# pangenome/seqrush

Hardware: AMD Instinct MI355X
Metric: aligned pairs/sec all-vs-all 64x5kb (higher is better)
Workload: dtype i16

## Files before the change

__graft_entry__.py:

```python
import os
import subprocess
import sys

ROOT = os.path.dirname(os.path.abspath(__file__))
if ROOT not in sys.path:
    sys.path.insert(0, ROOT)


def _newer(target, deps):
    if not os.path.exists(target):
        return False
    t = os.path.getmtime(target)
    return all(os.path.getmtime(d) <= t for d in deps if os.path.exists(d))


def _lib_is_current(lib):
    sys.path.insert(0, os.path.join(ROOT, "scripts"))
    import src_digest
    try:
        have, want = open(lib + ".digest").read().strip(), src_digest.digest(ROOT)
    except OSError as e:
        print(f"[build] no digest beside {os.path.basename(lib)} ({e}): building", file=sys.stderr)
        return False
    if not os.path.exists(lib) or have != want:
        print(f"[build] library digest {have} != source digest {want}: building", file=sys.stderr)
        return False
    return True


def build() -> None:
    csrc = os.path.join(ROOT, "seqrush_amd", "csrc")
    lib = os.path.join(ROOT, "seqrush_amd", "libseqrush_amd.so")
    bounds_lib = os.path.join(ROOT, "seqrush_amd", "libseqrush_amd_bounds.so")
    if not _lib_is_current(lib) or not os.path.exists(bounds_lib):
        subprocess.check_call(["make", "-C", csrc, "-s", "-j8"], stdout=subprocess.DEVNULL)
    odir = os.path.join(ROOT, "oracle")
    olib = os.path.join(odir, "liboracle.so")
    odeps = [os.path.join(odir, f) for f in ("uf.c", "wfa.c", "seqrush.c", "compact.c", "sr_oracle.h")]
    if not _newer(olib, odeps):
        subprocess.check_call(["make", "-C", odir, "-s", "-B"])
    ref_script = os.path.join(odir, "build_ref.sh")
    if os.path.isdir("/root/reference") and os.path.exists(ref_script):
        subprocess.call(["bash", ref_script])
    cli = os.path.join(ROOT, "seqrush_amd", "seqrush_mi355x")
    if not os.path.exists(cli):
        subprocess.check_call(["make", "-C", csrc, "-s"])
    import seqrush_amd
    from seqrush_amd import _lib
    L = _lib.load()
    missing = [s for s in _lib.EXPORTS if not hasattr(L, s)]
    if missing:
        raise RuntimeError(f"libseqrush_amd.so lacks symbols: {missing}")


def smoke() -> None:
    build()
    sys.path.insert(0, os.path.join(ROOT, "tests"))
    import numpy as np
    import oracle_binding as ob
    from seqrush_amd import synth
    from seqrush_amd.seqrush import SeqSet, Params, Context, build_gfa

    recs = synth.config_c1()
    ss = SeqSet(recs)
    ctx = Context(0)
    ctx.load(ss, Params())
    ctx.align(); ctx.unite(); ctx.sync()
    al = ctx.alignments()
    labels = ctx.download_labels()
    ctx.sync()
    o = ob.OracleSeqRush(records=recs)
    op = ob.default_params(); op.threads = 4
    for i in range(al.n):
        oa = o.align_pair(op, int(al.query_idx[i]), int(al.target_idx[i]))
        assert al.raw_cigar_bytes(i) == oa["cigar"], f"CIGAR mismatch on pair {i}"
        assert bool(al.is_reverse[i]) == oa["is_reverse"]
        assert int(al.score[i]) == oa["score"]
    o.align_and_unite(op)
    assert np.array_equal(o.canonical_labels(), labels), "UF partition differs from oracle"
    g_gpu, n_gpu, e_gpu = build_gfa(ss, labels)
    g_cpu, n_cpu, e_cpu = o.gfa(canonical=True)

    def canon(g):
        lines = g.strip().split("\n")
        return [x for x in lines if x[0] != "L"], sorted(x for x in lines if x[0] == "L")
    assert canon(g_gpu) == canon(g_cpu), "GFA differs from oracle"
    print(f"smoke ok: {al.n} pairs, {n_gpu} nodes, {e_gpu} edges, "
          f"align {ctx.kernel_ms(0):.2f} ms, unite {ctx.kernel_ms(1):.2f} ms")
    al.close(); ctx.close()


if __name__ == "__main__":
    build()
    if len(sys.argv) > 1 and sys.argv[1] == "smoke":
        smoke()
```

include/seqrush_amd.h:

```cpp
#ifndef SEQRUSH_AMD_H
#define SEQRUSH_AMD_H
#include <stddef.h>
#include <stdint.h>

#ifdef __cplusplus
extern "C" {
#endif

#define SR_ABI_VERSION 2

typedef enum {
    SR_OK = 0,
    SR_ERR_INVALID = -1,
    SR_ERR_NO_DEVICE = -2,
    SR_ERR_HIP = -3,
    SR_ERR_ALPHABET = -4,
    SR_ERR_EMPTY_SEQ = -5,
    SR_ERR_UNSUPPORTED = -6,
    SR_ERR_DEVICE_FAULT = -7,
    SR_ERR_IO = -8,
    SR_ERR_NOMEM = -9
} sr_status;

typedef struct {
// ... 30 lines not shown
    uint32_t shard_rank, shard_count;
    uint32_t tree_k_nearest, tree_k_farthest;
    double tree_rand_frac;
    uint32_t tree_kmer;
} sr_params;

void sr_default_params(sr_params *p);
int sr_parse_scores(const char *s, sr_params *p);
int sr_parse_orientation_scores(const char *s, sr_params *p);
int sr_parse_sparsification(const char *s, sr_params *p);

int sr_pair_list(uint32_t n, const sr_params *p, uint32_t **q_out, uint32_t **t_out,
                 uint64_t *count);

typedef struct {
    uint64_t n;
    uint32_t *query_idx, *target_idx;
    uint8_t *is_reverse;
    int32_t *score;
    uint64_t *query_start, *query_end, *target_start, *target_end;
    uint64_t *cigar_off;
    uint32_t *cigar_ops;
} sr_alignments;

int sr_align_all(const sr_seqset *seqs, const sr_params *p, sr_alignments **out);
void sr_alignments_free(sr_alignments *a);
size_t sr_alignment_cigar(const sr_alignments *a, uint64_t i, char *buf, size_t cap);

int sr_align_and_unite(const sr_seqset *seqs, const sr_params *p, uint64_t *parent_out);

uint64_t sr_uf_find(const uint64_t *nodes, uint64_t n, uint64_t x);
int sr_uf_same(const uint64_t *nodes, uint64_t n, uint64_t x, uint64_t y);
int sr_uf_init_host(uint64_t *nodes, uint64_t n, uint64_t total_len);
int sr_uf_unite_host(uint64_t *nodes, uint64_t n, uint64_t x, uint64_t y);
int sr_uf_merge_labels_host(uint64_t *nodes, uint64_t n, const uint64_t *labels, uint32_t count);
int sr_uf_canonical_labels_host(const uint64_t *nodes, uint64_t n, uint64_t *labels_out);

int sr_write_paf(const sr_alignments *a, const sr_seqset *seqs, const char *path);

typedef struct sr_ctx sr_ctx;
int sr_ctx_create(int device, sr_ctx **out);
void sr_ctx_destroy(sr_ctx *c);
int sr_ctx_set_stream(sr_ctx *c, void *hip_stream);
int sr_ctx_load(sr_ctx *c, const sr_seqset *seqs, const sr_params *p);
int sr_ctx_load_pairs(sr_ctx *c, const sr_seqset *seqs, const sr_params *p, const uint32_t *query_idx,
                      const uint32_t *target_idx, uint64_t count);
int sr_ctx_pairs(const sr_ctx *c, uint32_t **q_out, uint32_t **t_out, uint64_t *count);
uint32_t sr_ctx_num_batches(const sr_ctx *c);
const char *sr_ctx_workspace_report(const sr_ctx *c);
int sr_ctx_reset_uf(sr_ctx *c);
int sr_ctx_align(sr_ctx *c);
int sr_ctx_unite(sr_ctx *c);
int sr_ctx_run(sr_ctx *c);
int sr_ctx_align_all(sr_ctx *c, int unite, sr_alignments **out);
int sr_ctx_pair_results(sr_ctx *c, int32_t *score, uint8_t *is_reverse, uint32_t *cigar_ops);
int sr_ctx_sync(sr_ctx *c);
int sr_ctx_alignments(sr_ctx *c, sr_alignments **out);
int sr_ctx_download_uf(sr_ctx *c, uint64_t *parent_out);
uint64_t sr_ctx_uf_size(const sr_ctx *c);
uint64_t sr_ctx_num_pairs(const sr_ctx *c);
uint64_t sr_ctx_dp_cells(const sr_ctx *c);
int sr_ctx_labels_device(sr_ctx *c, uint64_t *dev_labels);
int sr_ctx_merge_labels(sr_ctx *c, const uint64_t *dev_labels, uint32_t count);
int sr_ctx_labels_device_u32(sr_ctx *c, uint32_t *dev_labels);
int sr_ctx_merge_labels_u32(sr_ctx *c, const uint32_t *dev_labels, uint32_t count);
int sr_ctx_download_labels(sr_ctx *c, uint64_t *labels_out);
int sr_ctx_merge_labels_host(sr_ctx *c, const uint64_t *labels, uint32_t count);
int sr_ctx_load_paf(sr_ctx *c, const sr_seqset *seqs, const sr_params *p, const char *paf_path);
int sr_unite_paf(const sr_seqset *seqs, const sr_params *p, const char *paf_path, uint64_t *parent_out);
int sr_ctx_build_gfa(sr_ctx *c, const sr_seqset *seqs, char **gfa, uint64_t *n_nodes, uint64_t *n_edges);
int sr_ctx_kernel_ms(sr_ctx *c, int which, float *ms);
const char *sr_ctx_align_kernel(const sr_ctx *c);
int sr_ctx_counters(sr_ctx *c, uint64_t out[16]);
int sr_ctx_counters_ext(sr_ctx *c, uint64_t out[32]);
int sr_ctx_counters_all(sr_ctx *c, uint64_t *out, uint32_t cap);
const char *sr_knobs_doc(void);
int sr_ctx_tail_deferred(sr_ctx *c, uint64_t *out);
int sr_ctx_tail_timeline(sr_ctx *c, uint64_t *out, uint32_t cap_wg);
int sr_ctx_prio_timeline(sr_ctx *c, uint64_t *out, uint32_t cap_wg);
int sr_tile_prio_role_host(uint32_t rank, uint32_t epoch, uint32_t wg_per_cu);
int sr_tile_prio_epoch_shift(void);
int sr_tail_shape(int impl, int block_levels, int wave_build, int off16, int ring_u16, int symbol_bits, int two_piece,
                  int main_threads, uint32_t max_words, int forced);

typedef struct {
    uint64_t tree_entries;
    uint64_t random_entries;
    uint64_t random_processed;
    uint64_t random_aligned;
    uint64_t checks;
    uint64_t windows;
    uint64_t post_tree;
    uint64_t final_components;
    int32_t stabilized;
    int32_t tree_defaulted;
    uint32_t tree_k_nearest, tree_k_farthest;
    double tree_rand_frac;
    uint32_t tree_kmer;
    uint32_t reserved;
} sr_iter_stats;
int sr_ctx_load_iterative(sr_ctx *c, const sr_seqset *seqs, const sr_params *p, int keep_alignments);
int sr_ctx_run_iterative(sr_ctx *c);
int sr_ctx_iterative_stats(sr_ctx *c, sr_iter_stats *out, uint64_t *check_counts, uint64_t cap);
int sr_ctx_iterative_alignments(sr_ctx *c, sr_alignments **out);
int sr_uf_count_components_host(const uint64_t *nodes, uint64_t n, uint64_t total_len, uint64_t *count);
int sr_iterative_stop_host(const uint64_t *counts, uint64_t nchecks, uint64_t post_tree, uint64_t *stop_check);
int sr_iterative_pair_lists(uint32_t n, const uint8_t *sel, const sr_params *p, uint32_t **tree_i, uint32_t **tree_j,
                            uint64_t *tree_count, uint32_t **rand_i, uint32_t **rand_j, uint64_t *rand_count);
int sr_base_cone_reach(int e1, int e2, int two, int levels_left);
int sr_mirror_map(const uint32_t *query_idx, const uint32_t *target_idx, uint64_t count, const uint32_t *batch_first,
                  uint32_t nbatch, uint32_t workgroups, uint32_t *mirror_out, uint64_t *partners_out);
int sr_ctx_orientation_scores(sr_ctx *c, int32_t *fwd, int32_t *rev);
int sr_mirror_bt_pick(const int *off, int transposed);
int sr_mirror_bt_rank_transposed(int tag);
int sr_mirror_bt_tie_host(const int *off);
int sr_mirror_bp_pick_host(const int *val, const int *dist, const int *comp, const int *diag, int n, int value_bias,
                           int *pick_out, int *pick_t_out);
int sr_replay_record_ints(void);
void sr_replay_transpose_host(const int *rec, int *out);
int sr_replay_match_host(const int *recs, int nrec, const int *segs, int nseg, int level, int *match_out);

typedef struct {
    uint64_t min_size;
    int32_t keep_alignments;
    uint32_t join_below;
} sr_inv_params;
typedef struct {
    uint64_t scanned;
    uint64_t sites;
    uint64_t candidates;
    uint64_t accepted;
    uint64_t rejected_score;
    uint64_t rejected_divergence;
    uint64_t united_bases;
    uint64_t patch_batches;
    double scan_ms, patch_align_ms;
} sr_inv_stats;
typedef struct {
    uint64_t pair;
    uint32_t query_idx, target_idx;
    uint64_t query_start, query_end;
    uint64_t target_start, target_end;
    int32_t main_score, patch_score;
    uint8_t is_reverse;
    uint8_t accepted;
    uint8_t reserved[2];
    int32_t site_cost;
} sr_inv_job;
int sr_ctx_enable_inversions(sr_ctx *c, const sr_inv_params *p);
int sr_ctx_inversion_stats(sr_ctx *c, sr_inv_stats *out);
int sr_ctx_inversion_join_stats(sr_ctx *c, uint64_t out[4]);
int sr_ctx_inversion_jobs(sr_ctx *c, sr_inv_job **jobs, uint64_t *count);
int sr_ctx_inversion_alignments(sr_ctx *c, sr_alignments **out);
int sr_append_paf_tagged(const sr_alignments *a, const sr_seqset *seqs, const char *path, const char *tag);
#define SR_INV_SITE_DIVERGENT 1
#define SR_INV_SITE_QUERY_ONLY 2
#define SR_INV_SITE_TARGET_ONLY 3
typedef struct {
    uint64_t query_start, query_end, target_start, target_end;
    int32_t kind;
    int32_t candidate;
} sr_inv_site;
int sr_inversion_sites_host(const uint32_t *ops, uint64_t n_ops, uint64_t min_size, sr_inv_site **sites, uint64_t *count);
int sr_inversion_candidate(uint64_t qgap, uint64_t tgap, uint64_t min_size);
int sr_inversion_accept(int32_t patch_score, int32_t main_score);
int sr_inversion_sites_host_join(const uint32_t *ops, uint64_t n_ops, uint64_t min_size, uint32_t join_below, const sr_params *pen,
// ... 183 lines not shown
```

seqrush_amd/_lib.py:

```python
import ctypes as C
import os

_HERE = os.path.dirname(os.path.abspath(__file__))
LIB_PATH = os.environ.get("SEQRUSH_AMD_LIB") or os.path.join(_HERE, "libseqrush_amd.so")

EXPORTS = [
    "sr_default_params", "sr_parse_scores", "sr_parse_orientation_scores",
    "sr_parse_sparsification", "sr_align_all", "sr_alignments_free", "sr_alignment_cigar",
    "sr_align_and_unite", "sr_uf_find", "sr_uf_same", "sr_write_paf", "sr_ctx_create",
    "sr_ctx_destroy", "sr_ctx_set_stream", "sr_ctx_load", "sr_ctx_reset_uf", "sr_ctx_align",
    "sr_ctx_unite", "sr_ctx_sync", "sr_ctx_alignments", "sr_ctx_download_uf", "sr_ctx_uf_size",
    "sr_ctx_num_pairs", "sr_ctx_dp_cells", "sr_ctx_labels_device", "sr_ctx_merge_labels",
    "sr_ctx_download_labels", "sr_ctx_kernel_ms", "sr_ctx_counters", "sr_build_gfa", "sr_free",
    "sr_last_error", "sr_abi_version", "sr_device_count", "sr_pair_list", "sr_ctx_align_kernel",
    "sr_ctx_load_paf", "sr_unite_paf", "sr_ctx_build_gfa", "sr_ctx_load_pairs", "sr_ctx_pairs",
    "sr_ctx_num_batches", "sr_ctx_workspace_report", "sr_ctx_run", "sr_ctx_align_all", "sr_ctx_pair_results",
    "sr_ctx_labels_device_u32", "sr_ctx_merge_labels_u32", "sr_ctx_counters_ext",
    "sr_build_gfa_opts", "sr_ctx_build_gfa_opts", "sr_ctx_merge_labels_host",
    "sr_uf_init_host", "sr_uf_unite_host", "sr_uf_merge_labels_host", "sr_uf_canonical_labels_host",
    "sr_build_gfa_from_nodes", "sr_ctx_counters_all", "sr_knobs_doc",
    "sr_sort_params_default", "sr_ctx_build_gfa_sorted", "sr_sort_gfa", "sr_sgd_layout", "sr_sgd_tables", "sr_sort_stats",
    "sr_ctx_load_iterative", "sr_ctx_run_iterative", "sr_ctx_iterative_stats", "sr_ctx_iterative_alignments",
    "sr_uf_count_components_host", "sr_iterative_stop_host", "sr_iterative_pair_lists", "sr_base_cone_reach",
    "sr_ctx_enable_inversions", "sr_ctx_inversion_stats", "sr_ctx_inversion_jobs", "sr_ctx_inversion_alignments",
    "sr_append_paf_tagged", "sr_inversion_sites_host", "sr_inversion_candidate", "sr_inversion_accept",
    "sr_inversion_scan_device",
    "sr_ctx_inversion_join_stats", "sr_inversion_sites_host_join", "sr_inversion_accept_site", "sr_inversion_scan_device_join",
    "sr_compact_gfa", "sr_compact_stats",
    "sr_sketch_device", "sr_knn_select_device",
    "sr_graph_stats_gfa", "sr_graph_stats_free", "sr_graph_stats_report", "sr_stats_sq_sums_host",
    "sr_mirror_map", "sr_mirror_bt_pick", "sr_mirror_bt_rank_transposed", "sr_mirror_bt_tie_host", "sr_mirror_bp_pick_host",
    "sr_ctx_orientation_scores",
    "sr_layout_params_default", "sr_layout_gfa", "sr_layout_tsv", "sr_layout_svg", "sr_layout_quality", "sr_layout_stats",
    "sr_layout_resolve", "sr_layout_select_host",
    "sr_path_bins_gfa", "sr_path_bins_free", "sr_path_bins_tsv", "sr_viz_params_default", "sr_path_bins_rgb", "sr_path_bins_png",
    "sr_growth_params_default", "sr_growth_gfa", "sr_growth_free", "sr_growth_groups", "sr_growth_expected", "sr_growth_fit",
    "sr_growth_report",
    "sr_variant_params_default", "sr_variants_gfa", "sr_variants_free", "sr_variants_vcf",
    "sr_ctx_tail_deferred", "sr_ctx_tail_timeline", "sr_tail_shape",
    "sr_replay_record_ints", "sr_replay_transpose_host", "sr_replay_match_host",
    "sr_ctx_prio_timeline", "sr_tile_prio_role_host", "sr_tile_prio_epoch_shift",
]


class SeqSetC(C.Structure):
    _fields_ = [("n", C.c_uint32), ("bases", C.c_char_p), ("offsets", C.POINTER(C.c_uint64)),
                ("names", C.POINTER(C.c_char_p))]


class ParamsC(C.Structure):
    _fields_ = [
        ("match_score", C.c_int32), ("mismatch_penalty", C.c_int32),
        ("gap_open1", C.c_int32), ("gap_ext1", C.c_int32),
        ("gap_open2", C.c_int32), ("gap_ext2", C.c_int32),
        ("ori_match", C.c_int32), ("ori_mismatch", C.c_int32),
        ("ori_gap_open", C.c_int32), ("ori_gap_ext", C.c_int32),
        ("min_match_len", C.c_uint64), ("max_divergence", C.c_double),
        ("exclude_self", C.c_int32), ("memory_mode", C.c_int32),
        ("sparsify_kind", C.c_int32), ("sparsify_factor", C.c_double),
        ("sparsify_seed", C.c_uint64), ("canonical_labels", C.c_int32), ("device", C.c_int32),
        ("shard_rank", C.c_uint32), ("shard_count", C.c_uint32),
        ("tree_k_nearest", C.c_uint32), ("tree_k_farthest", C.c_uint32), ("tree_rand_frac", C.c_double),
        ("tree_kmer", C.c_uint32),
    ]


class SortParamsC(C.Structure):
    _fields_ = [
        ("seed", C.c_uint64), ("iter_max", C.c_uint64), ("theta", C.c_double), ("eps", C.c_double),
        ("eta_max", C.c_double), ("cooling_start", C.c_double), ("space", C.c_uint64), ("space_max", C.c_uint64),
        ("space_quant", C.c_uint64), ("min_term_updates", C.c_uint64), ("terms_per_round", C.c_uint64),
        ("skip_sgd", C.c_int32), ("skip_groom", C.c_int32), ("skip_topo", C.c_int32), ("device", C.c_int32),
    ]


class LayoutParamsC(C.Structure):
    _fields_ = [
        ("seed", C.c_uint64), ("iter_max", C.c_uint64), ("theta", C.c_double), ("eps", C.c_double),
        ("eta_max", C.c_double), ("cooling_start", C.c_double), ("space", C.c_uint64), ("space_max", C.c_uint64),
        ("space_quant", C.c_uint64), ("min_term_updates", C.c_uint64), ("terms_per_round", C.c_uint64),
        ("device", C.c_int32), ("reserved", C.c_int32),
    ]


class IterStatsC(C.Structure):
    _fields_ = [
        ("tree_entries", C.c_uint64), ("random_entries", C.c_uint64), ("random_processed", C.c_uint64),
        ("random_aligned", C.c_uint64), ("checks", C.c_uint64), ("windows", C.c_uint64), ("post_tree", C.c_uint64),
        ("final_components", C.c_uint64), ("stabilized", C.c_int32), ("tree_defaulted", C.c_int32),
        ("tree_k_nearest", C.c_uint32), ("tree_k_farthest", C.c_uint32), ("tree_rand_frac", C.c_double),
        ("tree_kmer", C.c_uint32), ("reserved", C.c_uint32),
    ]


class InvParamsC(C.Structure):
    _fields_ = [("min_size", C.c_uint64), ("keep_alignments", C.c_int32), ("join_below", C.c_uint32)]


class InvStatsC(C.Structure):
    _fields_ = [("scanned", C.c_uint64), ("sites", C.c_uint64), ("candidates", C.c_uint64), ("accepted", C.c_uint64),
                ("rejected_score", C.c_uint64), ("rejected_divergence", C.c_uint64), ("united_bases", C.c_uint64),
                ("patch_batches", C.c_uint64), ("scan_ms", C.c_double), ("patch_align_ms", C.c_double)]


class InvJobC(C.Structure):
    _fields_ = [("pair", C.c_uint64), ("query_idx", C.c_uint32), ("target_idx", C.c_uint32),
                ("query_start", C.c_uint64), ("query_end", C.c_uint64), ("target_start", C.c_uint64),
                ("target_end", C.c_uint64), ("main_score", C.c_int32), ("patch_score", C.c_int32),
                ("is_reverse", C.c_uint8), ("accepted", C.c_uint8), ("reserved", C.c_uint8 * 2), ("site_cost", C.c_int32)]


class InvSiteC(C.Structure):
    _fields_ = [("query_start", C.c_uint64), ("query_end", C.c_uint64), ("target_start", C.c_uint64),
                ("target_end", C.c_uint64), ("kind", C.c_int32), ("candidate", C.c_int32)]


class GraphStatsC(C.Structure):
    _fields_ = [("length", C.c_uint64), ("nodes", C.c_uint64), ("edges", C.c_uint64), ("paths", C.c_uint64), ("steps", C.c_uint64),
                ("rev_steps", C.c_uint64), ("depth_bp", C.c_uint64),
                ("self_loops", C.c_uint64), ("tips", C.c_uint64), ("components", C.c_uint64),
                ("depth", C.POINTER(C.c_uint32)), ("paths_on", C.POINTER(C.c_uint32)),
                ("bp_by_paths", C.POINTER(C.c_uint64)), ("nodes_by_paths", C.POINTER(C.c_uint64)),
                ("shared", C.POINTER(C.c_uint64)),
                ("path_pairs", C.POINTER(C.c_uint64)), ("path_abs", C.POINTER(C.c_uint64)), ("path_len", C.POINTER(C.c_uint64)),
# ... 233 lines not shown
```

seqrush_amd/csrc/sr_align_blk.hip:

```cpp
#include "sr_dev_common.h"
#include "sr_uf_dev.h"
#define SR_BLK_TU 1
#undef SR_BFS_MAXACT
#ifdef SR_BLK_WAVE
#define SR_BFS_MAXACT 4
#define K_P2 4
#define SR_BLK_SUB wave1
#else
#define SR_BFS_MAXACT 16
#define K_P2 16
#define SR_BLK_SUB wg4
#endif
#define BFS_MAK_SLOTS SR_BLK_MAK_SLOTS
#define SR_BT_ATTR __forceinline__
namespace SR_NS { namespace SR_BLK_SUB {
#include "sr_align_bfs.inc"
#include "sr_align_blk.inc"
} }
using namespace SR_NS::SR_BLK_SUB;

template <typename OT, int NT, bool TWO, bool PROF = false>
static int launch_blk3(const SrAlignArgs *a, int nwg, size_t lds_bytes, hipStream_t st) {
    if (lds_bytes > 16 * 1024) {
        hipError_t e = hipFuncSetAttribute((const void *)sr_align_blk_kernel<OT, NT, TWO, 5, 2, 1, PROF>,
                                           hipFuncAttributeMaxDynamicSharedMemorySize, (int)lds_bytes);
        if (e != hipSuccess) return (int)e;
    }
    hipLaunchKernelGGL((sr_align_blk_kernel<OT, NT, TWO, 5, 2, 1, PROF>), dim3(nwg), dim3(NT), lds_bytes, st, *a);
    return (int)hipGetLastError();
}
template <typename OT, int NT, bool TWO, bool PROF = false, typename RT = OT>
static int launch_blk10(const SrAlignArgs *a, int nwg, size_t lds_bytes, hipStream_t st) {
    if (lds_bytes > 16 * 1024) {
        hipError_t e = hipFuncSetAttribute((const void *)sr_align_blk_kernel<OT, NT, TWO, 10, 2, 1, PROF, 5, 10, RT>,
                                           hipFuncAttributeMaxDynamicSharedMemorySize, (int)lds_bytes);
        if (e != hipSuccess) return (int)e;
    }
    hipLaunchKernelGGL((sr_align_blk_kernel<OT, NT, TWO, 10, 2, 1, PROF, 5, 10, RT>), dim3(nwg), dim3(NT), lds_bytes, st, *a);
    return (int)hipGetLastError();
}
#if SR_SYMBITS == 2 && !defined(SR_BLK_WAVE)
extern "C" int srk_align_blk_max_levels(void) { return KB_MAX; }
#ifndef SR_BUILD_TAG
#define SR_BUILD_TAG "default"
#endif
extern "C" const char *srk_align_blk_build_tag(void) { return SR_BUILD_TAG; }
extern "C" int srk_align_blk_supports(const SrPen *pen, const SrPen *ori) {
    if (ori->two || ori->e1 != 1 || ori->scope + 2 > BFS_MAK_SLOTS) return 0;
    if (pen->e1 != 2 || (pen->two && pen->e2 != 1)) return 0;
    if (pen->x == 5 && pen->o1 + pen->e1 == 10 && (!pen->two || (pen->o2 + pen->e2 >= 10 && (pen->o2 + pen->e2) % 5 == 0)) &&
        (2 * pen->scope + 2 * 10 + 2 + 9) / 10 * 10 <= BFS_MAK_SLOTS) return 10;
    const int B = 5;
    if (pen->x < B || pen->o1 + pen->e1 < B) return 0;
    if (pen->two && pen->o2 + pen->e2 < B) return 0;
    if (pen->scope + B + 1 > BFS_MAK_SLOTS) return 0;
    return B;
}
#endif
#ifdef SR_BLK_WAVE
extern "C" int SRK_NAME(srk_align_blkw)(const SrAlignArgs *a, int nwg, size_t lds_bytes, int off16, int nthreads, void *stream) {
    hipStream_t st = (hipStream_t)stream;
    const bool two = a->pen.two != 0;
    if (a->kblock == 10 && nthreads == 128 && off16)
        return two ? launch_blk10<int16_t, 128, true>(a, nwg, lds_bytes, st) : launch_blk10<int16_t, 128, false>(a, nwg, lds_bytes, st);
    if (a->kblock == 10) {
        if (off16) return two ? launch_blk10<int16_t, 64, true>(a, nwg, lds_bytes, st) : launch_blk10<int16_t, 64, false>(a, nwg, lds_bytes, st);
        return two ? launch_blk10<int32_t, 64, true>(a, nwg, lds_bytes, st) : launch_blk10<int32_t, 64, false>(a, nwg, lds_bytes, st);
    }
    if (off16) return two ? launch_blk3<int16_t, 64, true>(a, nwg, lds_bytes, st) : launch_blk3<int16_t, 64, false>(a, nwg, lds_bytes, st);
    return two ? launch_blk3<int32_t, 64, true>(a, nwg, lds_bytes, st) : launch_blk3<int32_t, 64, false>(a, nwg, lds_bytes, st);
}
#else
extern "C" int SRK_NAME(srk_align_blk)(const SrAlignArgs *a, int nwg, size_t lds_bytes, int off16, int nthreads, void *stream) {
    hipStream_t st = (hipStream_t)stream;
    const bool two = a->pen.two != 0;
    if (a->kblock == 10) {
        if (off16) {
#if SR_SYMBITS == 2
            if (nthreads == 1024 && two) return launch_blk10<int16_t, 1024, true>(a, nwg, lds_bytes, st);
#endif
            if (nthreads >= 512) return two ? launch_blk10<int16_t, 512, true>(a, nwg, lds_bytes, st) : launch_blk10<int16_t, 512, false>(a, nwg, lds_bytes, st);
#if SR_SYMBITS == 2
            if (a->profile_ticks && two) return launch_blk10<int16_t, 256, true, true>(a, nwg, lds_bytes, st);
#endif
            return two ? launch_blk10<int16_t, 256, true>(a, nwg, lds_bytes, st) : launch_blk10<int16_t, 256, false>(a, nwg, lds_bytes, st);
        }
        if (a->ring_u16 && nthreads == 512) return two ? launch_blk10<int32_t, 512, true, false, uint16_t>(a, nwg, lds_bytes, st)
                                                       : launch_blk10<int32_t, 512, false, false, uint16_t>(a, nwg, lds_bytes, st);
        if (a->ring_u16) return two ? launch_blk10<int32_t, 256, true, false, uint16_t>(a, nwg, lds_bytes, st)
                                    : launch_blk10<int32_t, 256, false, false, uint16_t>(a, nwg, lds_bytes, st);
        return two ? launch_blk10<int32_t, 256, true>(a, nwg, lds_bytes, st) : launch_blk10<int32_t, 256, false>(a, nwg, lds_bytes, st);
    }
    if (off16) {
        if (nthreads == 128) return two ? launch_blk3<int16_t, 128, true>(a, nwg, lds_bytes, st) : launch_blk3<int16_t, 128, false>(a, nwg, lds_bytes, st);
        if (nthreads == 512) return two ? launch_blk3<int16_t, 512, true>(a, nwg, lds_bytes, st) : launch_blk3<int16_t, 512, false>(a, nwg, lds_bytes, st);
        return two ? launch_blk3<int16_t, 256, true>(a, nwg, lds_bytes, st) : launch_blk3<int16_t, 256, false>(a, nwg, lds_bytes, st);
    }
    return two ? launch_blk3<int32_t, 256, true>(a, nwg, lds_bytes, st) : launch_blk3<int32_t, 256, false>(a, nwg, lds_bytes, st);
}
#endif
```

seqrush_amd/csrc/sr_align_blk.inc:

```
#include "sr_blk_rows.inc"
#include "sr_blk_tile.inc"
#include "sr_blk_pass.inc"
#include "sr_blk_phase2.inc"
#include "sr_blk_orient.inc"

#define K_SHIFT0 29
#define K_WIDTH0 64
struct KSeqs { int poff_f, poff_r, toff_f, toff_r, plen_all, tlen_all; };
__device__ __forceinline__ void kjob_set(int jid, int base, int pb, int pe, int tb, int te, int rev, int begin, int chk,
                                         int seg, const KSeqs &q) {
    bjob_set(jid, base, pb, pe, tb, te, 0, begin, chk, seg, rev ? q.poff_r : q.poff_f);
    BJob &b = b_sh.job[jid];
    b.shift = (pe - pb) + K_SHIFT0;
    b.pad0 = rev ? q.toff_r : q.toff_f;
    b.pad2 = 1;
    if (rev) { b.p0 = q.plen_all - pe; b.t0 = q.tlen_all - te; }
}
__device__ __forceinline__ int kjob_width(int plen, int tlen) { return (plen + tlen + K_WIDTH0) & ~3; }

#define SR_BLK_MIN_WAVES 4
template <typename OT, int NT, bool TWO, int B, int E1, int E2, bool PROF = false, int X = 0, int OE1 = 0, typename RT = OT>
__global__ void __launch_bounds__(NT, SR_BLK_MIN_WAVES) sr_align_blk_kernel(SrAlignArgs a) {
    const int tid = threadIdx.x;
    if (a.tail_mode == SR_TAIL_RUN && *a.tail_count == 0u) return;
    GP<RT> bring = (GP<RT>)(RT *)a.bring + (size_t)blockIdx.x * a.bring_wg_stride;
    GP<OT> bhist = (GP<OT>)(OT *)a.bhist + (size_t)blockIdx.x * a.bhist_wg_stride;
    GP<int> lists = (GP<int>)a.bseg + (size_t)blockIdx.x * 2 * SR_BFS_MAXSEG * SR_BFS_SEGREC;
    GP<uint32_t> btbuf = (GP<uint32_t>)a.bbt + (size_t)blockIdx.x * a.bbase_jobs * SR_BFS_BTCAP;
    GP<uint32_t> clist = (GP<uint32_t>)a.bcl + (size_t)blockIdx.x * a.bcl_wg_stride;
    GP<int> gmak = (GP<int>)a.bmak + (size_t)blockIdx.x * (BJ_MAX * BFS_MAK_SLOTS);
    unsigned long long t_ori = 0, t_bp = 0, t_base = 0, t_all = 0, tb_bt = 0, tb_emit = 0;
    unsigned long long tq_pass = 0, tq_bar = 0, tq_ctl = 0, tq_ph2 = 0, tq_tail = 0, tq_rec = 0;
    unsigned row_ld = 0, row_st = 0;
    unsigned long long tl_first = 0, tl_last = 0, tl_n = 0, tl_mir = 0, tl_end1 = 0;
    const int depth = a.kdepth;
    const int depth2 = a.kdepth2;
    const unsigned nrows = (unsigned)depth + 4u * (unsigned)depth2 + (unsigned)SR_NULL_ROWS + 2u;
    KRows<OT, RT> RR;
    KRows<OT, OT> RH;
    RR.base = bring; RR.cM = (unsigned)depth * 256u; RR.cst2 = (unsigned)depth2 * 256u; RR.sstr = 256u; RR.chs = nrows * 256u;
    RR.depth = depth; RR.depth2 = depth2; RR.perjob = false; RR.extent = (unsigned)a.bring_wg_stride;
    RR.nuloff = ((unsigned)depth + 4u * (unsigned)depth2) * 256u; RR.urow = RR.nuloff + (unsigned)SR_NULL_ROWS * 256u; RR.trash = RR.urow + 256u;
    const unsigned urow = RR.urow;
    const unsigned hw = a.hist_nul_w;
    RH.base = bhist; RH.cM = 0; RH.cst2 = 0; RH.sstr = 0; RH.chs = 256u; RH.depth = 0x3fff; RH.depth2 = 0x3fff; RH.urow = 0; RH.perjob = true; RH.extent = (unsigned)a.bhist_wg_stride;
    RH.nuloff = (unsigned)a.hist_cap; RH.trash = RH.nuloff + hw;
    if (tid < 64) k_sh.cells_l[tid] = 0ull;
    if (tid < 64) k_sh.row_w[tid >> 4][tid & 15] = 0ull;
    {
        for (int r = 0; r < SR_NULL_ROWS; r++)
            for (int i = tid; i < a.brow; i += NT) rput(RR, RR.nuloff + (unsigned)r * 256u, (unsigned)i, NULLV);
        for (int i = tid; i < (int)hw; i += NT) RH.base[RH.nuloff + (unsigned)i] = (OT)NULLV;
        if (tid == 0) {
            b_sh.pen[0] = a.pen; b_sh.pen[1] = a.ori; b_sh.cells = 0; k_sh.t_setup = 0; k_sh.t_p2a = k_sh.t_p2f = k_sh.t_p2e = k_sh.t_p2w = 0; k_sh.t_c1 = k_sh.t_c2 = 0;
            k_sh.dg_f = k_sh.dg_c = k_sh.dg_e = k_sh.dg_r = 0; k_sh.dg_redo = 0;
#ifdef SR_BOUNDS
            k_sh.bnd_flag = 0; k_sh.bnd_off = k_sh.bnd_ext = k_sh.bnd_what = 0; k_sh.lds_seq_bytes = 16u * a.max_words + 16u;
#endif
            k_sh.dg_steps = k_sh.dg_nbase = k_sh.dg_nbp = k_sh.dg_npass = 0; k_sh.base_tiles = k_sh.base_cells = 0;
            k_sh.mir_next = -1; k_sh.mir_pairs = k_sh.mir_ties = 0;
            k_sh.rp_record = k_sh.rp_on = k_sh.rp_ready = 0; k_sh.rp_nrec = 0;
            k_sh.rp_replays = k_sh.rp_cached = k_sh.rp_tie_top = k_sh.rp_tie_base = 0;
            b_sh.geom.brow = a.brow; b_sh.geom.ring_scope = a.ring_scope; b_sh.geom.ring_hot = a.ring_hot;
            b_sh.geom.bbase_jobs = a.bbase_jobs; b_sh.geom.hist_w = a.hist_w; b_sh.geom.hist_levels = a.hist_levels;
            b_sh.geom.urow = urow;
            unsigned p_rank = 0, p_idx = 0, p_arr = 0;
            if (a.cu_arrivals) {
                const unsigned xcc = (unsigned)__builtin_amdgcn_s_getreg(20 | (0 << 6) | (3 << 11));
                const unsigned cu = (unsigned)__builtin_amdgcn_s_getreg(4 | (8 << 6) | (7 << 11));
                p_idx = sr_prio_table_index(xcc, cu);
                p_arr = atomicAdd(&a.cu_arrivals[p_idx], 1u);
                p_rank = p_arr % (unsigned)max(a.prio_wg, 1);
                atomicAdd(&a.counters[52], 1ull);
                atomicMax(&a.counters[53], (unsigned long long)p_arr + 1ull);
            }
            k_sh.prio_rank = (int)p_rank; k_sh.prio_role = 0;
            k_sh.prio_wg = (a.tile_prio && a.cu_arrivals && a.prio_wg > 1) ? a.prio_wg : 0;
            if (PROF && a.prio_timeline) {
                unsigned long long *tp = a.prio_timeline + 4ull * blockIdx.x;
                tp[0] = 0ull; tp[1] = p_rank; tp[2] = p_idx; tp[3] = p_arr;
            }
        }
        __syncthreads();
    }
    const SrPen pen = a.pen;
    const SrPen ori = a.ori;
    constexpr bool KTIGHT = KTIGHT_OF(OT, RT, B, X);
    const int scope = pen.scope;
    const int gap_opening = TWO ? max(pen.o1, pen.o2) : pen.o1;
    for (;;) {
        if (tid < 64) {
            unsigned long long cl = k_sh.cells_l[tid];
            k_sh.cells_l[tid] = 0ull;
            for (int o = 32; o > 0; o >>= 1) cl += __shfl_xor(cl, o, 64);
            if (tid == 0) b_sh.cells += cl;
        }
        if (tid == 0) {
            int pr = k_sh.mir_next;
            k_sh.mir_next = -1;
            const bool from_mir = pr >= 0;
            if (a.tail_mode == SR_TAIL_RUN) {
                const uint32_t i = atomicAdd(a.tail_head, 1u);
                pr = i < *a.tail_count ? (int)a.tail_list[i] : (int)a.npairs;
            } else while (pr < 0) {
                pr = (int)atomicAdd(a.queue_head, 1u);
                if (pr >= (int)a.npairs) { pr = (int)a.npairs; break; }
                if (a.order) pr = (int)a.order[pr];
                if (a.mirror && a.mirror[pr] != SR_MIRROR_NONE && (a.mirror[pr] & SR_MIRROR_SECONDARY)) pr = -1;
            }
            if (PROF) {
                const unsigned long long now = KTICK();
                if (tl_n == 0) tl_first = now;
                if (tl_n == 1 && tl_end1 == 0) tl_end1 = now;
                if (pr < (int)a.npairs) { tl_last = now; tl_n++; tl_mir = from_mir ? 1ull : 0ull; }
            }
            k_sh.rp_on = (from_mir && k_sh.rp_ready) ? 1 : 0;
            k_sh.rp_ready = 0; k_sh.rp_record = 0;
            if (a.brec && !from_mir && a.tail_mode != SR_TAIL_RUN && a.mirror && pr < (int)a.npairs) {
                const uint32_t m = a.mirror[pr];
                if (m != SR_MIRROR_NONE && !(m & SR_MIRROR_SECONDARY)) { k_sh.rp_record = 1; k_sh.rp_nrec = 0; }
            }
            k_sh.rp_level = 0; k_sh.rp_rd = 0; k_sh.rp_top_tie = 0; k_sh.rp_seg_tie = 0;
            b_sh.pair = pr;
            b_sh.err = 0; b_sh.cig_cnt = 0; b_sh.score_acc = 0; k_sh.pend_op = -1; k_sh.pend_len = 0;
            k_sh.mir_tie = 0;
            k_sh.mir_snap[0] = b_sh.cells; k_sh.mir_snap[1] = k_sh.dg_steps; k_sh.mir_snap[2] = k_sh.dg_nbase; k_sh.mir_snap[3] = k_sh.dg_nbp;
        }
        __syncthreads();
        const int pair = RFL(b_sh.pair);
        if (pair >= (int)a.npairs) break;
        const uint32_t q = a.pair_q[pair], t = a.pair_t[pair];
        const int plen = (int)a.seqlen[q], tlen = (int)a.seqlen[t];
        const int pw = SR_SEQ_WORDS(plen), tw = SR_SEQ_WORDS(tlen);
        load_seq_lds<NT>(lds_seq, (GP<const uint32_t>)a.seqwords + a.word_off_fwd[q] - 1, pw);
        load_seq_lds<NT>(lds_seq + a.max_words, (GP<const uint32_t>)a.seqwords + a.word_off_rc[q] - 1, pw);
        load_seq_lds<NT>(lds_seq + 2 * (size_t)a.max_words, (GP<const uint32_t>)a.seqwords + a.word_off_fwd[t] - 1, tw);
        load_seq_lds<NT>(lds_seq + 3 * (size_t)a.max_words, (GP<const uint32_t>)a.seqwords + a.word_off_rev[t] - 1, tw);
        const int oPf = 1, oPr = (int)a.max_words + 1, oTf = 2 * (int)a.max_words + 1, oTr = 3 * (int)a.max_words + 1;
        GP<uint32_t> ops = (GP<uint32_t>)a.cigar_ops + a.cigar_base[pair];
        const uint32_t cap = (uint32_t)(a.cigar_base[pair + 1] - a.cigar_base[pair]);
        const unsigned long long tk0 = KTICK();
        int fwd = -1, rev = INT_MAX, is_rev = 0;
        if (a.pre_oriented) {
// ... 52 lines not shown
                if (s > smax) { if (tid == 0) b_sh.err |= SR_DEV_ERR_SCORE_BOUND; break; }
            }
        }
        }
        if (a.word_off_rev != a.word_off_rc) {
            __syncthreads();
            load_seq_lds<NT>(lds_seq + (is_rev ? 0 : (size_t)a.max_words),
                             (GP<const uint32_t>)a.seqwords + (is_rev ? a.word_off_cmp[q] : a.word_off_rev[q]) - 1, pw);
            __syncthreads();
        }
        const KSeqs ks = {is_rev ? oPr : oPf, is_rev ? oPf : oPr, oTf, oTr, plen, tlen};
        const unsigned long long tk1 = KTICK();
        t_ori += tk1 - tk0;
        GP<int> cur = lists, nxt = lists + (size_t)SR_BFS_MAXSEG * SR_BFS_SEGREC;
        if (tid == 0) {
            cur[SL_PB] = 0; cur[SL_PE] = plen; cur[SL_TB] = 0; cur[SL_TE] = tlen; cur[SL_CB] = SR_C_M; cur[SL_CE] = SR_C_M;
            const int rem = (a.mem_mode == 3) ? INT_MAX : -1;
            cur[SL_REM] = rem; cur[SL_KIND] = seg_kind(plen, tlen, rem);
            b_sh.list_n = 1;
            if (is_rev) k_sh.rp_on = 0;
            if (k_sh.rp_on) k_sh.rp_replays += 1ull;
        }
        __syncthreads();
        for (;;) {
            const int n_cur = RFL(b_sh.list_n);
            bool any_bp = false;
            int pos = 0;
            if (RFL(k_sh.rp_on) != 0 && tid == 0) {
                GP<int> recs = (GP<int>)a.brec + (size_t)blockIdx.x * (SR_BPREC_MAX * SR_BPREC_INTS);
                const int nrec = min(k_sh.rp_nrec, SR_BPREC_MAX), lvl = k_sh.rp_level;
                int rd = k_sh.rp_rd;
                unsigned long long cells = 0ull, cached = 0ull;
                while (rd < nrec && recs[rd * SR_BPREC_INTS + SR_BR_LEVEL] < lvl) rd++;
                for (int p = 0; p < n_cur; p++) {
                    GP<int> e = cur + (size_t)p * SR_BFS_SEGREC;
                    if (e[SL_KIND] != SK_BP) continue;
                    int solved = 0;
                    while (rd < nrec) {
                        GP<int> r = recs + rd * SR_BPREC_INTS;
                        if (r[SR_BR_LEVEL] != lvl) break;
                        const int c = sr_replay_cmp(r, e);
                        if (c > 0) break;
                        rd++;
                        if (c < 0) continue;
                        if (r[SR_BR_TIE] == 0 && sr_replay_same(r, e)) {
                            e[SL_BV] = sr_bprec_t(r, SR_BR_BV); e[SL_BH] = sr_bprec_t(r, SR_BR_BH); e[SL_BCOMP] = sr_bprec_t(r, SR_BR_BCOMP);
                            e[SL_BSF] = r[SR_BR_BSF]; e[SL_BSR] = r[SR_BR_BSR]; e[SL_PASSES] = r[SR_BR_PASSES];
                            cells += ((unsigned long long)(unsigned)r[SR_BR_CELLS_HI] << 32) | (unsigned long long)(unsigned)r[SR_BR_CELLS_LO];
                            cached += 1ull; solved = 1;
                        }
                        break;
                    }
                    e[SL_SOLVED] = solved;
                }
                k_sh.rp_rd = rd; b_sh.cells += cells; k_sh.rp_cached += cached;
            }
            while (pos < n_cur && RFL(b_sh.err) == 0) {
                __syncthreads();
                if (tid == 0) {
                    int na = 0, p = pos, base = 0, ntot = 0, maxp = 0;
                    const bool rp_on = k_sh.rp_on != 0, rp_rec = k_sh.rp_record != 0;
                    for (; p < n_cur && ntot < SR_BFS_MAXACT; p++) {
                        GP<int> e = cur + (size_t)p * SR_BFS_SEGREC;
                        if (e[SL_KIND] != SK_BP) continue;
                        ntot++;
                        if (rp_on && e[SL_SOLVED] != 0) { maxp = max(maxp, e[SL_PASSES]); continue; }
                        k_sh.sg_tie[na] = 0; k_sh.sg_sur[na] = 0; k_sh.sg_done[na] = 0;
                        if (rp_rec) {
                            b_sh.cells += k_sh.cells_l[2 * na] + k_sh.cells_l[2 * na + 1];
                            k_sh.cells_l[2 * na] = 0ull; k_sh.cells_l[2 * na + 1] = 0ull;
                        }
                        BSeg &sg = b_sh.seg[na];
                        sg.pb = e[SL_PB]; sg.pe = e[SL_PE]; sg.tb = e[SL_TB]; sg.te = e[SL_TE]; sg.cb = e[SL_CB]; sg.ce = e[SL_CE];
                        sg.score_f = sg.score_r = 0; sg.last_fwd = 0; sg.f_ak = sg.r_ak = 0; sg.phase = 1;
                        const int sp = sg.pe - sg.pb, st = sg.te - sg.tb;
                        sg.max_ad = sp + st - 1; sg.bp_score = INT_MAX; sg.list_pos = p;
                        const int w = kjob_width(sp, st);
                        kjob_set(2 * na, base, sg.pb, sg.pe, sg.tb, sg.te, 0, sg.cb, -1, na, ks); base += w;
                        kjob_set(2 * na + 1, base, sg.pb, sg.pe, sg.tb, sg.te, 1, sg.ce, -1, na, ks); base += w;
                        if (a.lazy_id) { b_sh.job[2 * na].pad2 = 0; b_sh.job[2 * na + 1].pad2 = 0; }
                        na++;
                    }
                    b_sh.nact = na; b_sh.next_pos = p; b_sh.njobs = 2 * na; b_sh.nrunning = na;
                    k_sh.rp_ntot = ntot; k_sh.rp_maxp = maxp; k_sh.rp_npass0 = k_sh.dg_npass;
                }
                __syncthreads();
                const int nact = RFL(b_sh.nact);
                pos = RFL(b_sh.next_pos);
                if (RFL(k_sh.rp_ntot) == 0) break;
                any_bp = true;
                if (tid == 0) k_sh.dg_nbp += (unsigned long long)k_sh.rp_ntot;
                if (nact == 0) {
                    if (tid == 0) k_sh.dg_steps += 2ull * (unsigned long long)k_sh.rp_ntot * B * (unsigned long long)k_sh.rp_maxp;
                    continue;
                }
                const unsigned long long tb0 = KTICK();
                const int njobs = 2 * nact;
                for (int s0i = 0; RFL(b_sh.nrunning) > 0; s0i += B) {
                    const int s0 = kopaque_s(s0i);
                    const unsigned long long q0 = KTICK();
                    blk_pass<OT, TWO, NT, B, E1, E2, PROF, X, OE1, RT, true>(RR, s0, pen, njobs, row_ld, row_st, s0 == 0);
                    const unsigned long long q1 = KTICK();
                    __syncthreads();
                    const unsigned long long q2 = KTICK();
                    tq_pass += q1 - q0; tq_bar += q2 - q1;
                    if (tid == 0) k_sh.dg_steps += (unsigned long long)njobs * B;
                    const int avail = s0 + B - 1;
                    const int tid_o = tid;
                    if (tid < 64) {
                        const int tid = (int)kopaque_v((unsigned)tid_o);
                        KPRIO_HI();
                        if (tid < njobs) {
#pragma unroll
                            for (int j = 0; j < B; j++) gmak[tid * BFS_MAK_SLOTS + (s0 + j) % depth] = k_sh.jak[j][tid];
                        }
                        const unsigned long long qc1 = KTICK();
                        int ph = 0, ph0 = 0;
                        if (tid < nact) {
                            BSeg &sg = b_sh.seg[tid];
                            ph = sg.phase; ph0 = ph;
                            const long long smax = 2LL * ((long long)pen.o1 * 2 + (long long)pen.e1 * (sg.max_ad + 1)) + 1024;
                            if (ph == 1) {
                                int score_f = sg.score_f, score_r = sg.score_r, last_fwd = sg.last_fwd, f_ak = sg.f_ak, r_ak = sg.r_ak;
                                const int max_ad = sg.max_ad;
                                for (int j = 0; j < B && ph == 1; j++) {
                                    const int s = s0 + j;
                                    const int akf = k_sh.jak[j][2 * tid], akr = k_sh.jak[j][2 * tid + 1];
                                    if (s == 0) {
                                        f_ak = akf; r_ak = akr;
                                        if (f_ak + r_ak >= max_ad) ph = 2;
                                    } else {
                                        score_f = s; f_ak = akf; last_fwd = 1;
                                        if (f_ak + r_ak >= max_ad) ph = 2;
                                        else {
                                            score_r = s; r_ak = akr; last_fwd = 0;
                                            if ((long long)score_f + score_r > smax) ph = 4;
                                            else if (f_ak + r_ak >= max_ad) ph = 2;
                                        }
                                    }
                                }
                                sg.score_f = score_f; sg.score_r = score_r; sg.last_fwd = last_fwd; sg.f_ak = f_ak; sg.r_ak = r_ak;
                                sg.phase = ph;
                            }
                        }
                        const unsigned long long qc2 = KTICK();
                        if (PROF && tid == 0) { k_sh.t_c1 += qc1 - q2; k_sh.t_c2 += qc2 - qc1; }
                        const unsigned long long m2 = __ballot(ph == 2);
                        const unsigned long long mnew = __ballot(ph == 2 && ph0 == 1);
                        if (tid == 0) k_sh.newmask = (unsigned)mnew;
                        if (tid == 0) { k_sh.p2mask_lo = (unsigned)m2; k_sh.p2mask_hi = (unsigned)(m2 >> 32); }
                        if (m2 == 0ull) {
                            const unsigned long long run = __ballot(ph == 1);
                            if (tid < nact && ph != 1) { b_sh.job[2 * tid].active = 0; b_sh.job[2 * tid + 1].active = 0; }
                            if (tid == 0) b_sh.nrunning = __popcll(run);
                            if (run != 0ull) blk_setup<TWO, NT, B, E1, E2, KTIGHT>(s0 + B, pen, njobs);
                        }
                        KPRIO_LO();
                    }
                    __syncthreads();
                    const unsigned long long q3 = KTICK();
                    tq_ctl += q3 - q2;
                    bool p2_or_rec = (RFL(k_sh.p2mask_lo) | RFL(k_sh.p2mask_hi)) != 0u;
                    if (a.lazy_id) {
                        if (RFL(k_sh.newmask) != 0u) p2_or_rec = true;
                        for (unsigned nm = RFL(k_sh.newmask); nm != 0u; nm &= nm - 1u) {
                            const int sa = __ffs((int)nm) - 1;
                            blk_recompute<OT, TWO, NT, B, E1, E2, X, OE1>(RR, pen, sa, RFL(b_sh.seg[sa].score_f), s0, row_ld, row_st);
                        }
                    }
                    tq_rec += KTICK() - q3;
                    if ((RFL(k_sh.p2mask_lo) | RFL(k_sh.p2mask_hi)) != 0u) {
                        blk_phase2<OT, TWO, NT, B, E1, E2, RT, PROF>(RR, clist, gmak, pen, s0, nact, gap_opening);
                        if (tid < 64) {
                            KPRIO_HI();
                            const int ph = (tid < nact) ? b_sh.seg[tid].phase : 0;
                            const unsigned long long run = __ballot(ph == 1 || ph == 2);
                            if (tid < nact && ph != 1 && ph != 2) { b_sh.job[2 * tid].active = 0; b_sh.job[2 * tid + 1].active = 0; }
                            if (tid == 0) b_sh.nrunning = __popcll(run);
                            if (run != 0ull) blk_setup<TWO, NT, B, E1, E2, KTIGHT>(s0 + B, pen, njobs);
                            KPRIO_LO();
                        }
                    }
                    const unsigned long long q4 = KTICK();
                    if (p2_or_rec) __syncthreads();
                    tq_ph2 += q4 - q3; tq_tail += KTICK() - q4;
                    if (tid == 0) k_sh.dg_npass += 1ull;
                }
                if (tid < nact) {
                    BSeg &sg = b_sh.seg[tid];
                    GP<int> e = cur + (size_t)sg.list_pos * SR_BFS_SEGREC;
                    const int sp = sg.pe - sg.pb, st = sg.te - sg.tb;
                    const int bh = sg.bp_off_f, bv = sg.bp_off_f - sg.bp_k_f;
                    if (sg.phase != 3 || sg.bp_score == INT_MAX) atomicOr(&b_sh.err, SR_DEV_ERR_SCORE_BOUND);
                    else if (bv < 0 || bv > sp || bh < 0 || bh > st) atomicOr(&b_sh.err, SR_DEV_ERR_BREAKPOINT);
                    else {
                        e[SL_BV] = bv; e[SL_BH] = bh; e[SL_BCOMP] = sg.bp_comp; e[SL_BSF] = sg.bp_score_f; e[SL_BSR] = sg.bp_score_r;
                        const int ri = k_sh.rp_nrec + tid;
// ... 228 lines not shown
                if (atomicCAS(&a.counters[40], 0ull, (unsigned long long)pair + 1ull) == 0ull) {
                    a.counters[41] = k_sh.bnd_what; a.counters[42] = k_sh.bnd_off; a.counters[43] = k_sh.bnd_ext;
                }
            }
#endif
        }
        __syncthreads();
        const uint32_t mir = a.mirror ? a.mirror[pair] : SR_MIRROR_NONE;
        bool mir_emit = false;
        if (mir != SR_MIRROR_NONE && !(mir & SR_MIRROR_SECONDARY)) {
            mir_emit = p_err == 0 && !is_rev && p_tie == 0 && !(a.pre_oriented && a.is_reverse[mir] != 0);
            if (mir_emit) {
                GP<uint32_t> ops2 = (GP<uint32_t>)a.cigar_ops + a.cigar_base[mir];
                for (uint32_t i = tid; i < cnt; i += NT) { const uint32_t v = ops[i]; ops2[i] = v ^ ((v & 2u) >> 1); }
                if (tid < 64) {
                    unsigned long long cl = k_sh.cells_l[tid];
                    k_sh.cells_l[tid] = 0ull;
                    for (int o = 32; o > 0; o >>= 1) cl += __shfl_xor(cl, o, 64);
                    if (tid == 0) {
                        b_sh.cells += cl;
                        b_sh.cells += b_sh.cells - k_sh.mir_snap[0]; k_sh.dg_steps += k_sh.dg_steps - k_sh.mir_snap[1];
                        k_sh.dg_nbase += k_sh.dg_nbase - k_sh.mir_snap[2]; k_sh.dg_nbp += k_sh.dg_nbp - k_sh.mir_snap[3];
                        k_sh.mir_pairs += 1ull;
                        a.score[mir] = p_score; a.cigar_cnt[mir] = cnt;
                        if (!a.pre_oriented) { a.is_reverse[mir] = 0; a.ori_fwd[mir] = fwd; a.ori_rev[mir] = rev; }
                    }
                }
            } else if (tid == 0) {
                k_sh.mir_ties += 1ull;
                if (p_tie != 0) {
                    if (k_sh.rp_top_tie != 0) k_sh.rp_tie_top += 1ull;
                    else if (k_sh.rp_seg_tie == 0) k_sh.rp_tie_base += 1ull;
                }
                const bool replay = k_sh.rp_record != 0 && p_err == 0 && !is_rev && k_sh.rp_top_tie == 0 &&
                                    !(a.pre_oriented && a.is_reverse[mir] != 0) && a.tail_mode != SR_TAIL_DEFER_ALL;
                bool defer = false;
                if (!replay && a.tail_list && a.tail_mode != SR_TAIL_RUN)
                    defer = a.tail_mode == SR_TAIL_DEFER_ALL ||
                            __hip_atomic_load(a.queue_head, __ATOMIC_RELAXED, __HIP_MEMORY_SCOPE_AGENT) >= a.npairs;
                if (defer) { a.tail_list[atomicAdd(a.tail_count, 1u)] = mir; atomicAdd(a.tail_deferred, 1u); }
                else { k_sh.mir_next = (int)mir; k_sh.rp_ready = replay ? 1 : 0; }
            }
        }
        if (a.fuse_unite) {
            const int sc = p_err ? -1 : p_score;
            if (sc >= 0 && sc <= a.max_score[pair]) {
                unsigned long long united = 0, runs = 0;
                int uerr = 0;
                uf_unite_cigar<NT>((const uint32_t *)a.cigar_ops + a.cigar_base[pair], cnt, a.seq_goff[q], a.seq_goff[t],
                                   (unsigned long long)plen, is_rev != 0, 0ull, 0ull, a.min_match_len, a.uf_nodes, united, runs, uerr);
                for (int o = 32; o > 0; o >>= 1) { united += __shfl_xor(united, o, 64); runs += __shfl_xor(runs, o, 64); }
                if ((tid & 63) == 0) {
                    if (united) atomicAdd(&a.counters[4], mir_emit ? 2ull * united : united);
                    if (runs) atomicAdd(&a.counters[5], mir_emit ? 2ull * runs : runs);
                }
                if (uerr) atomicOr(a.error_flag, uerr);
            }
        }
        t_all += KTICK() - tk0;
        if ((tid & 63) == 0) {
            k_sh.row_w[0][(tid >> 6) & 15] += row_ld; k_sh.row_w[1][(tid >> 6) & 15] += row_st;
            k_sh.row_w[2][(tid >> 6) & 15] += row_ld; k_sh.row_w[3][(tid >> 6) & 15] += row_st;
        }
        row_ld = 0; row_st = 0;
    }
    if (tid < 64 && k_sh.cells_l[tid]) atomicAdd(&a.counters[0], k_sh.cells_l[tid]);
    if ((tid & 63) == 0) {
        const unsigned long long lane_bytes = 8ull;
        const unsigned long long row_ld_acc = k_sh.row_w[0][(tid >> 6) & 15], row_st_acc = k_sh.row_w[1][(tid >> 6) & 15];
        if (row_ld_acc) atomicAdd(&a.counters[16], row_ld_acc * lane_bytes);
        if (row_st_acc) atomicAdd(&a.counters[17], row_st_acc * lane_bytes);
        const unsigned long long hist_ld_acc = k_sh.row_w[2][(tid >> 6) & 15], hist_st_acc = k_sh.row_w[3][(tid >> 6) & 15];
        if (hist_ld_acc) atomicAdd(&a.counters[44], hist_ld_acc * lane_bytes);
        if (hist_st_acc) atomicAdd(&a.counters[45], hist_st_acc * lane_bytes);
    }
    if (tid == 0) {
        atomicAdd(&a.counters[0], b_sh.cells);
        atomicAdd(&a.counters[1], k_sh.dg_steps);
        atomicAdd(&a.counters[2], k_sh.dg_nbase);
        atomicAdd(&a.counters[3], k_sh.dg_nbp);
        atomicAdd(&a.counters[9], k_sh.dg_npass);
        atomicAdd(&a.counters[19], k_sh.dg_f); atomicAdd(&a.counters[20], k_sh.dg_c);
        atomicAdd(&a.counters[21], k_sh.dg_e); atomicAdd(&a.counters[22], k_sh.dg_r);
        if (k_sh.dg_redo) atomicAdd(&a.counters[37], k_sh.dg_redo);
        if (k_sh.mir_pairs) atomicAdd(&a.counters[38], k_sh.mir_pairs);
        if (k_sh.mir_ties) atomicAdd(&a.counters[39], k_sh.mir_ties);
        if (k_sh.rp_tie_top) atomicAdd(&a.counters[48], k_sh.rp_tie_top);
        if (k_sh.rp_tie_base) atomicAdd(&a.counters[49], k_sh.rp_tie_base);
        if (k_sh.rp_replays) atomicAdd(&a.counters[50], k_sh.rp_replays);
        if (k_sh.rp_cached) atomicAdd(&a.counters[51], k_sh.rp_cached);
        atomicAdd(&a.counters[46], k_sh.base_tiles); atomicAdd(&a.counters[47], k_sh.base_cells);
        if (PROF && a.timeline) {
            unsigned long long *tl = a.timeline + 4ull * blockIdx.x;
            tl[0] = tl_first; tl[1] = tl_last; tl[2] = KTICK(); tl[3] = tl_n | (tl_mir << 32);
        }
        if (PROF && a.prio_timeline) a.prio_timeline[4ull * blockIdx.x] = tl_end1;
        if (PROF) {
            if (!a.pre_oriented) atomicAdd(&a.counters[6], t_ori);
            atomicAdd(&a.counters[7], t_bp);
            atomicAdd(&a.counters[8], t_base);
            atomicAdd(&a.counters[10], t_all);
            atomicAdd(&a.counters[11], tq_pass);
            atomicAdd(&a.counters[12], tq_bar);
            atomicAdd(&a.counters[13], k_sh.t_setup);
            atomicAdd(&a.counters[25], tq_ctl); atomicAdd(&a.counters[26], k_sh.t_c1); atomicAdd(&a.counters[27], k_sh.t_c2);
            atomicAdd(&a.counters[28], k_sh.t_p2a); atomicAdd(&a.counters[29], k_sh.t_p2f); atomicAdd(&a.counters[30], k_sh.t_p2e); atomicAdd(&a.counters[31], k_sh.t_p2w);
            atomicAdd(&a.counters[14], tq_ph2);
            atomicAdd(&a.counters[18], tq_rec);
            atomicAdd(&a.counters[23], tb_bt); atomicAdd(&a.counters[24], tb_emit);
            atomicAdd(&a.counters[15], tq_tail);
        }
    }
#undef KTICK
}
```

seqrush_amd/csrc/sr_blk_pass.inc:

```
#include "sr_base_cone.h"
#include "sr_prio_rule.h"
template <bool TWO, int E1, int E2>
__device__ __forceinline__ int kreach(const SrPen &p, int s, int begin) {
    int r;
    if (begin == SR_C_M) {
        r = (s >= p.o1 + E1) ? (s - p.o1) / E1 : 0;
        if (TWO && s >= p.o2 + E2) r = max(r, (s - p.o2) / E2);
    } else {
        r = s / E1;
        if (TWO) r = max(r, s / E2);
    }
    return r;
}

template <bool TWO, int B, int E1, int E2, bool TIGHT>
__device__ __forceinline__ void kwindow(const SrPen &pen, const BJob &b, int s0, int &glo, int &ghi) {
    const int Rw = kreach<TWO, E1, E2>(pen, s0 + B - 1, b.begin);
    const int mg = TIGHT ? 1 : pen.scope + 1;
    const int wlo = max(-b.plen - 1, -Rw - mg), whi = min(b.tlen + 1, Rw + mg);
    glo = (wlo + b.shift) >> 2; ghi = (whi + b.shift) >> 2;
}

#define KTICK() (PROF ? __builtin_amdgcn_s_memrealtime() : 0ull)
__device__ __forceinline__ void kprio_role() {
    switch (RFL(k_sh.prio_role)) {
    case 1: __builtin_amdgcn_s_setprio(1); break;
    case 2: __builtin_amdgcn_s_setprio(2); break;
    case 3: __builtin_amdgcn_s_setprio(3); break;
    default: __builtin_amdgcn_s_setprio(0); break;
    }
}
__device__ __forceinline__ void kprio_epoch() {
    const int wg = RFL(k_sh.prio_wg);
    if (wg > 1) {
        const unsigned epoch = (unsigned)(__builtin_amdgcn_s_memrealtime() >> SR_PRIO_EPOCH_SHIFT);
        if (threadIdx.x == 0) k_sh.prio_role = sr_tile_prio_role((unsigned)k_sh.prio_rank, epoch, (unsigned)wg);
    }
}
#define KPRIO_HI() __builtin_amdgcn_s_setprio(3)
#define KPRIO_LO() kprio_role()
#ifndef SR_BASE_CONE
#define SR_BASE_CONE 1
#endif
template <bool TWO, int NT, int B, int E1, int E2, bool TIGHT = false, bool BASE = false>
__device__ __forceinline__ void blk_setup(int s0, const SrPen &pen, int njobs) {
    const int tid = threadIdx.x;
    constexpr bool CONE = BASE && SR_BASE_CONE;
    int nt = 0, glo = 0, ghi = -1, cells = 0, ccells = 0;
    const bool act = tid < njobs && b_sh.job[tid].active;
    const int pglo = (tid < BJ_MAX) ? k_sh.jglo[tid] : 0, pghi = (tid < BJ_MAX) ? k_sh.jghi[tid] : -1;
    if (act) {
        const BJob &b = b_sh.job[tid];
        int Rw = 0, clo0 = 0, chi0 = 0;
#pragma unroll
        for (int j = 0; j < B; j++) {
            Rw = kreach<TWO, E1, E2>(pen, s0 + j, b.begin);
            int klo = max(-b.plen, -Rw), khi = min(b.tlen, Rw);
            cells += (khi >= klo) ? khi - klo + 1 : 0;
            if (CONE) {
                const int rb = sr_cone_reach(E1, E2, TWO, b.pad1 - 1 - (s0 + j));
                klo = max(klo, b.kend - rb); khi = min(khi, b.kend + rb);
                if (j == 0) { clo0 = b.kend - rb; chi0 = b.kend + rb; }
            }
            k_sh.jklo[j][tid] = klo; k_sh.jkhi[j][tid] = khi;
            ccells += (khi >= klo) ? khi - klo + 1 : 0;
        }
        (void)Rw;
        kwindow<TWO, B, E1, E2, TIGHT>(pen, b, s0, glo, ghi);
        if (CONE) {
            const int mg = TIGHT ? 1 : pen.scope + 1;
            const int wlo = max(max(-b.plen - 1, -Rw - mg), clo0 - 1), whi = min(min(b.tlen + 1, Rw + mg), chi0 + 1);
            glo = (wlo + b.shift) >> 2; ghi = (whi >= wlo) ? (whi + b.shift) >> 2 : glo - 1;
        }
        nt = max(0, (ghi - glo + KGeo<B>::OWN) / KGeo<B>::OWN);
        if (BASE && ccells) atomicAdd(&k_sh.base_cells, (unsigned long long)ccells);
    }
    int incl = nt, hincl = 0;
#pragma unroll
    for (int o = 1; o < 64; o <<= 1) {
        const int v = __shfl_up(incl, o, 64), h = __shfl_up(hincl, o, 64);
        if (tid >= o) { incl += v; hincl += h; }
    }
    if (tid < BJ_MAX) {
        k_sh.jglo[tid] = glo; k_sh.jghi[tid] = ghi;
        k_sh.jgplo[tid] = pglo; k_sh.jgphi[tid] = pghi;
        k_sh.jtstart[tid + 1] = incl;
        k_sh.jmerge[tid] = 0;
        k_sh.jband[tid] = INT_MAX / 2;
#pragma unroll
        for (int j = 0; j < B; j++) { k_sh.jak[j][tid] = 0; k_sh.jreach[j][tid] = 0; }
    }
    if (tid == 0) k_sh.jtstart[0] = 0;
    if (tid == 63) { k_sh.nband = hincl; k_sh.total_tiles = incl + hincl; k_sh.next_tile = NT / 64; if (BASE) k_sh.base_tiles += (unsigned long long)incl; }
    k_sh.cells_l[tid] += (unsigned long long)cells;
    kprio_epoch();
}

template <typename OT, bool TWO, int NT, int B, int E1, int E2, bool PROF, int X = 0, int OE1 = 0, typename ST = OT, bool RING = false, bool BASE = false>
__device__ __forceinline__ void blk_pass(const KRows<OT, ST> &R, int s0, const SrPen &pen, int njobs,
                                         unsigned &row_ld, unsigned &row_st, const bool setup = true) {
    const int tid = threadIdx.x;
    if (setup) {
        const unsigned long long tsu0 = KTICK();
        if (tid < 64) blk_setup<TWO, NT, B, E1, E2, RING && KTIGHT_OF(OT, ST, B, X), BASE>(s0, pen, njobs);
        __syncthreads();
        if (PROF && threadIdx.x == 0) k_sh.t_setup += KTICK() - tsu0;
    }
    kprio_role();
    const int total = RFL(k_sh.total_tiles);
    const int slot0 = kslots(R, s0);
    const int nband = RFL(k_sh.nband);
    for (int t = (tid >> 6); t < total;) {
        int lo, ti;
        if (t < nband) { lo = RFL(k_sh.jbandown[t]); ti = RFL(k_sh.jband[lo]); }
        else {
            const int r = t - nband;
            int hi = njobs; lo = 0;
            while (hi - lo > 1) { const int mid = (lo + hi) >> 1; if (RFL(k_sh.jtstart[mid]) <= r) lo = mid; else hi = mid; }
            ti = r - RFL(k_sh.jtstart[lo]);
            ti += (ti >= RFL(k_sh.jband[lo])) ? 1 : 0;
        }
        blk_tile_any<OT, TWO, B, E1, E2, false, X, OE1, ST, RING>(R, s0, slot0, pen, lo, ti, lo, row_ld, row_st);
        int nx = 0;
        if ((tid & 63) == 0) nx = atomicAdd(&k_sh.next_tile, 1);
        t = RFL(nx);
    }
}

template <typename OT, bool TWO, int NT, int B, int E1, int E2, int X = 0, int OE1 = 0, typename ST = OT>
__device__ __forceinline__ void blk_recompute(const KRows<OT, ST> &R, const SrPen &pen, int sa, int entry_level, int s0_now,
                                              unsigned &row_ld, unsigned &row_st) {
    const int tid = threadIdx.x;
    const int wlo = max(0, entry_level - pen.scope);
    for (int blk = (wlo / B) * B; blk <= s0_now; blk += B) {
        __syncthreads();
        if (tid < 2) {
            const BJob &b = b_sh.job[2 * sa + tid];
            int Rw = 0;
#pragma unroll
            for (int j = 0; j < B; j++) {
                Rw = kreach<TWO, E1, E2>(pen, blk + j, b.begin);
                k_sh.jklo[j][BJ_MAX + tid] = max(-b.plen, -Rw); k_sh.jkhi[j][BJ_MAX + tid] = min(b.tlen, Rw);
            }
            (void)Rw;
            int glo, ghi;
            kwindow<TWO, B, E1, E2, KTIGHT_OF(OT, ST, B, X)>(pen, b, blk, glo, ghi);
            const bool first = blk == (wlo / B) * B;
            k_sh.jgplo[BJ_MAX + tid] = first ? 1 : k_sh.jglo[BJ_MAX + tid];
            k_sh.jgphi[BJ_MAX + tid] = first ? 0 : k_sh.jghi[BJ_MAX + tid];
            k_sh.jglo[BJ_MAX + tid] = glo; k_sh.jghi[BJ_MAX + tid] = ghi;
            const int nt = (ghi - glo + KGeo<B>::OWN) / KGeo<B>::OWN;
            const int n0 = __shfl(nt, 0, 64), n1 = __shfl(nt, 1, 64);
            if (tid == 0) { k_sh.rt_n0 = n0; k_sh.rt_total = n0 + n1; }
        }
        __syncthreads();
        const int n0 = RFL(k_sh.rt_n0), total = RFL(k_sh.rt_total);
        const int slot0 = kslots(R, blk);
        for (int t = (tid >> 6); t < total; t += NT / 64) {
            const int side = (t >= n0) ? 1 : 0;
            blk_tile_any<OT, TWO, B, E1, E2, true, X, OE1, ST, true>(R, blk, slot0, pen, 2 * sa + side, t - (side ? n0 : 0), BJ_MAX + side, row_ld, row_st);
        }
    }
    __syncthreads();
    if (tid < 2) b_sh.job[2 * sa + tid].pad2 = 1;
}

__device__ __forceinline__ long long blk_surplus(const SrPen &pen, int jid, int l0, int l1) {
    const BJob &b = b_sh.job[jid];
    long long c = 0;
    for (int l = l0 + 1; l <= l1; l++) {
        const int Rw = reach(pen, l, b.begin);
        const int klo = max(-b.plen, -Rw), khi = min(b.tlen, Rw);
        c += (khi >= klo) ? khi - klo + 1 : 0;
    }
    return c;
}
```

seqrush_amd/csrc/sr_blk_rows.inc:

```
#define SR_ORI_B 16
#define SR_KB_MAX 10
#define KB_LV (SR_ORI_B > SR_KB_MAX ? SR_ORI_B : SR_KB_MAX)
#define KB_MAX SR_KB_MAX
#define KPK_U16_OF(OT, ST, B, X) (sizeof(OT) == 4 && sizeof(ST) == 2 && (X) > 0 && (B) % 10 == 0)
#define KTIGHT_OF(OT, ST, B, X) ((X) > 0 && (B) % 10 == 0 && (sizeof(OT) == 2 || KPK_U16_OF(OT, ST, B, X)))

struct KShared {
    int jklo[KB_LV][BJ_MAX + 2], jkhi[KB_LV][BJ_MAX + 2];
    int jak[KB_MAX][BJ_MAX], jreach[KB_LV][BJ_MAX];
    int jtstart[BJ_MAX + 1], jglo[BJ_MAX + 2], jghi[BJ_MAX + 2];
    int jmerge[BJ_MAX];
    int jband[BJ_MAX], jbandown[BJ_MAX], nband;
    unsigned newmask;
    int rt_n0, rt_total;
    int jgplo[BJ_MAX + 2], jgphi[BJ_MAX + 2];
    int total_tiles;
    int next_tile;
    int prio_role, prio_rank, prio_wg;
    int p2n, p2seg[K_P2];
    unsigned p2mask_lo, p2mask_hi;
    int pc_n[K_P2], pc_s1[K_P2][2 * KB_MAX];
    unsigned char pc_side[K_P2][2 * KB_MAX];
    signed char pc_idx[K_P2][2][KB_MAX];
    unsigned long long pc_best[K_P2][2 * KB_MAX];
    unsigned long long pc_best_t[K_P2][2 * KB_MAX];
    int pu_start[2 * K_P2 + 1], pu_glo[2 * K_P2];
    int pu_kmin[2 * K_P2], pu_kmax[2 * K_P2];
    int cl_n;
#ifdef SR_BOUNDS
    unsigned lds_seq_bytes;
    int bnd_flag; unsigned bnd_off, bnd_ext, bnd_what;
#endif
    int mir_tie, mir_next;
    unsigned long long mir_snap[4];
    unsigned long long mir_pairs, mir_ties;
    int sg_tie[SR_BFS_MAXACT], sg_sur[SR_BFS_MAXACT], sg_done[SR_BFS_MAXACT];
    int rp_record, rp_on, rp_ready;
    int rp_level, rp_nrec, rp_rd;
    int rp_top_tie, rp_seg_tie;
    int rp_ntot, rp_maxp;
    unsigned long long rp_npass0;
    unsigned long long rp_replays, rp_cached, rp_tie_top, rp_tie_base;
    int redo_from;
    int pend_op, pend_len;
    unsigned long long row_w[4][16];
    unsigned long long base_tiles, base_cells;
    unsigned long long cells_l[64];
    unsigned long long t_c1, t_c2;
    unsigned long long t_setup, t_p2a, t_p2f, t_p2e, t_p2w;
    unsigned long long dg_steps, dg_nbase, dg_nbp, dg_npass;
    unsigned long long dg_f, dg_c, dg_e, dg_r;
    unsigned long long dg_redo;
};
__shared__ KShared k_sh;

template <typename OT, typename ST = OT>
struct KRows {
    GP<ST> base;
    unsigned cM, cst2, sstr, chs;
    unsigned urow, nuloff, trash;
    int depth, depth2;
    bool perjob;
    unsigned extent;
};
#ifdef SR_BOUNDS
__device__ __forceinline__ void kbnd_fail(unsigned what, unsigned off, unsigned ext) {
    atomicOr(&b_sh.err, SR_DEV_ERR_ADDRESS);
    if (atomicCAS(&k_sh.bnd_flag, 0, 1) == 0) { k_sh.bnd_off = off; k_sh.bnd_ext = ext; k_sh.bnd_what = what; }
}
#define SR_BND_OK(R, CELL, WHAT) (((CELL) + 3u < (R).extent) ? true : (kbnd_fail((WHAT), (CELL), (R).extent), false))
#else
#define SR_BND_OK(R, CELL, WHAT) true
#endif
struct KAdr { unsigned hb, cM, cst2, sst; int slotM, slotD, depth, depth2; };
template <typename OT, typename ST>
__device__ __forceinline__ KAdr kadr(const KRows<OT, ST> &R, const BJob &jb, int slots) {
    KAdr A;
    if (R.perjob) { const unsigned hw = RFL(jb.hw); A.hb = RFL(jb.hbase); A.cM = hw; A.cst2 = hw; A.sst = 5u * hw; }
    else { A.hb = 0u; A.cM = R.cM; A.cst2 = R.cst2; A.sst = R.sstr; }
    A.slotM = slots & 0xffff; A.slotD = (int)((unsigned)slots >> 16); A.depth = R.depth; A.depth2 = R.depth2;
    return A;
}
template <typename OT, typename ST>
__device__ __forceinline__ int kslots(const KRows<OT, ST> &R, int s) { return (s % R.depth) | ((s % R.depth2) << 16); }
#define SR_RING_BIAS 24576
typedef short __attribute__((ext_vector_type(4))) S4;
template <typename OT, typename ST> __device__ __forceinline__ V4<OT> kcvt_in(V4<ST> v) {
    if constexpr (sizeof(ST) == sizeof(OT)) return v;
    else { const V4<OT> b = {SR_RING_BIAS, SR_RING_BIAS, SR_RING_BIAS, SR_RING_BIAS}; return __builtin_convertvector((S4)v, V4<OT>) + b; }
}
template <typename OT, typename ST> __device__ __forceinline__ V4<ST> kcvt_out(V4<OT> v) {
    if constexpr (sizeof(ST) == sizeof(OT)) return v;
    else { const V4<OT> b = {SR_RING_BIAS, SR_RING_BIAS, SR_RING_BIAS, SR_RING_BIAS}; return (V4<ST>)__builtin_convertvector(v - b, S4); }
}
// ... 111 lines not shown
```

seqrush_amd/csrc/sr_blk_tile.inc:

```
template <typename OT, bool TWO, int B, int E1, int E2, bool IDONLY = false, int X = 0, int OE1 = 0, typename ST = OT>
__device__ __forceinline__ void blk_tile(const KRows<OT, ST> &R, const int s0, const int slot0, const SrPen &pen,
                                         const int jid, const int ti, const int tix, unsigned &row_ld, unsigned &row_st) {
    constexpr int N1 = E1 < B ? E1 : B, N2 = E2 < B ? E2 : B;
    constexpr bool XK = X > 0;
    static_assert(!XK || (B == OE1 && X <= B), "exact-penalty instance: block depth == o1 + e1 >= x");
    constexpr int HL = KGeo<B>::HL, OWN = KGeo<B>::OWN;
    constexpr int PF = XK ? 3 : B;
    const int lane = threadIdx.x & 63;
    const BJob &jb = b_sh.job[jid];
    const int base = RFL(jb.base), shift = RFL(jb.shift), plen = RFL(jb.plen), tlen = RFL(jb.tlen);
    const int p0 = RFL(jb.p0), t0 = RFL(jb.t0), begin = RFL(jb.begin);
    const int chk = RFL(jb.chk), kend = RFL(jb.kend), poff = RFL(jb.poff), toff = RFL(jb.pad0);
    const bool rec = IDONLY || RFL(jb.pad2) != 0;
    const int glo = RFL(k_sh.jglo[tix]), ghi = RFL(k_sh.jghi[tix]);
    const int g = glo + ti * OWN + lane - HL;
    const bool owned = (lane >= HL) && (lane < 64 - HL) && (g <= ghi);
    const int k0 = (g << 2) - shift;
    const unsigned idx0 = klane(R, (unsigned)(base + (g << 2)));
    const LP P = (LP)(lds_seq + poff), T = (LP)(lds_seq + toff);
    const int cp0 = p0 - k0 + (int)(((uint32_t)(uintptr_t)P >> 2) << SR_WIN_LOG);
    const int ct0 = t0 + (int)(((uint32_t)(uintptr_t)T >> 2) << SR_WIN_LOG);
    const KAdr A = kadr(R, jb, slot0);
#define KROW(LVL, C) krow_rel(R, A, s0, (LVL), (C))
    V4<OT> Lmx[XK ? 1 : B], Lmo1[B], Lmo2[B], Li1[N1], Ld1[N1], Li2[N2], Ld2[N2];
// ... 272 lines not shown
            "v_pk_ashrrev_i16 %1, 15, %5 op_sel_hi:[0,1]\n\t"
            "v_bfi_b32 %2, %0, %6, %4\n\t"
            "v_bfi_b32 %3, %1, %6, %5"
            : "=&v"(ta), "=&v"(tb), "=&v"(ra), "=&v"(rb)
            : "v"(h2_u(v.a)), "v"(h2_u(v.b)), "s"(nul));
    } else {
        const uint32_t bias2 = ((uint32_t)BIAS & 0xffffu) | ((uint32_t)BIAS << 16);
        asm("v_pk_add_i16 %0, %4, %7 clamp\n\t"
            "v_pk_add_i16 %1, %5, %7 clamp\n\t"
            "v_pk_ashrrev_i16 %0, 15, %0 op_sel_hi:[0,1]\n\t"
            "v_pk_ashrrev_i16 %1, 15, %1 op_sel_hi:[0,1]\n\t"
            "v_bfi_b32 %2, %0, %6, %4\n\t"
            "v_bfi_b32 %3, %1, %6, %5"
            : "=&v"(ta), "=&v"(tb), "=&v"(ra), "=&v"(rb)
            : "v"(h2_u(v.a)), "v"(h2_u(v.b)), "s"(nul), "v"(bias2));
    }
    Q4 r; r.a = h2_bits(ra); r.b = h2_bits(rb);
    return r;
}
#define SR_DEEP_INT16 3000
#define SR_DEEP_RING16 1500
__device__ __forceinline__ int q4_get(Q4 x, int q) {
    return (q == 0) ? (int)x.a.x : (q == 1) ? (int)x.a.y : (q == 2) ? (int)x.b.x : (int)x.b.y;
}

template <bool TWO, int B, int E1, int E2, bool IDONLY = false, int X = 0, int OE1 = 0, bool RING = false, typename KR = KRows<short>, int BIAS = 0>
__device__ __forceinline__ void blk_tile16(const KR &R, const int s0, const int slot0, const SrPen &pen,
                                           const int jid, const int ti, const int tix, unsigned &row_ld, unsigned &row_st) {
    typedef short OT;
    typedef short ST;
    static_assert(BIAS == 0 || (RING && X > 0 && B % 10 == 0), "the biased tile exists for ring rows with immediate addressing only");
    constexpr uint32_t NUL = BIAS ? 0x80008000u : NULL16;
    constexpr int NULC = BIAS ? -32768 : -16384;
    const Q4 nulq = {h2_bits(NUL), h2_bits(NUL)};
    constexpr int N1 = E1 < B ? E1 : B, N2 = E2 < B ? E2 : B;
    constexpr bool XK = X > 0;
    static_assert(!XK || (B == OE1 && X <= B), "exact-penalty instance: block depth == o1 + e1 >= x");
    constexpr int HL = KGeo<B>::HL, OWN = KGeo<B>::OWN;
    constexpr int PF = XK ? 3 : B;
    const int lane = threadIdx.x & 63;
    const BJob &jb = b_sh.job[jid];
    const int base = RFL(jb.base), p0 = RFL(jb.p0), t0 = RFL(jb.t0), poff = RFL(jb.poff), toff = RFL(jb.pad0);
    const int shift = RFL(jb.shift), plen = RFL(jb.plen), tlen = RFL(jb.tlen), begin = RFL(jb.begin);
    const int chk = RFL(jb.chk), kend = RFL(jb.kend);
    const bool rec = IDONLY || RFL(jb.pad2) != 0;
    const int glo = RFL(k_sh.jglo[tix]), ghi = RFL(k_sh.jghi[tix]);
    const int g = glo + ti * OWN + lane - HL;
    const bool owned = (lane >= HL) && (lane < 64 - HL) && (g <= ghi);
    const int k0 = (g << 2) - shift;
    const unsigned idx0 = klane(R, (unsigned)(base + (g << 2)));
    const LP P = (LP)(lds_seq + poff), T = (LP)(lds_seq + toff);
    const KAdr A = kadr(R, jb, slot0);
#define KROW(LVL, C) krow_rel(R, A, s0, (LVL), (C))
#define LDQ(LVL, C) q4_from(rld<OT>(R, KROW((LVL), (C)), idx0))
#define LDQ_NT(LVL, C) q4_from(rld_nt<OT>(R, KROW((LVL), (C)), idx0))
    constexpr bool IMMR = RING && XK && (B % 10 == 0);
    const unsigned lane_b = idx0 * (unsigned)sizeof(ST);
    GPB bM1 = nullptr, bM2a = nullptr, bM2b = nullptr, bI1 = nullptr, bD1 = nullptr, bI2 = nullptr, bD2 = nullptr;
    GPB sM = nullptr, sI1 = nullptr, sD1 = nullptr, sI2 = nullptr, sD2 = nullptr;
    if constexpr (IMMR) {
        const int oe2 = pen.o2 + E2;
        bM1 = kbase(R, s0 - B < 0 ? R.nuloff + KBLK_C * 256u : KROW(s0 - B + KBLK_C, SR_C_M));
        bM2a = kbase(R, KROW(s0 - oe2, SR_C_M)); bM2b = kbase(R, KROW(s0 - oe2 + 5, SR_C_M));
        bI1 = kbase(R, KROW(s0 - E1, SR_C_I1)); bD1 = kbase(R, KROW(s0 - E1, SR_C_D1));
        bI2 = kbase(R, KROW(s0 - E2, SR_C_I2)); bD2 = kbase(R, KROW(s0 - E2, SR_C_D2));
        sM = kbase(R, KROW(s0 + KBLK_C, SR_C_M));
        sI1 = kbase(R, KROW(s0 + KBLK_C, SR_C_I1)); sD1 = kbase(R, KROW(s0 + KBLK_C, SR_C_D1));
        sI2 = kbase(R, KROW(s0 + KBLK_C, SR_C_I2)); sD2 = kbase(R, KROW(s0 + KBLK_C, SR_C_D2));
    }
    constexpr bool TIGHT = IMMR && (BIAS ? true : (bool)KTIGHT_OF(short, short, B, X));
    bool msk = false, in10 = true, in2a = true, in2b = true;
    if constexpr (TIGHT) {
        const int oe2 = TWO ? pen.o2 + E2 : B;
        const int l2a = s0 - oe2, l2b = s0 - oe2 + 5;
        const int b2a = l2a >= 0 ? (l2a / B) * B : -1, b2b = l2b >= 0 ? (l2b / B) * B : -1;
        int lo10 = INT_MIN / 2, hi10 = INT_MAX / 2, lo2a = lo10, hi2a = hi10, lo2b = lo10, hi2b = hi10;
        if (s0 - B >= 0) kwindow<TWO, B, E1, E2, true>(pen, jb, s0 - B, lo10, hi10);
        if (TWO && b2a >= 0) kwindow<TWO, B, E1, E2, true>(pen, jb, b2a, lo2a, hi2a);
        if (TWO && b2b >= 0) kwindow<TWO, B, E1, E2, true>(pen, jb, b2b, lo2b, hi2b);
        lo10 = RFL(lo10); hi10 = RFL(hi10); lo2a = RFL(lo2a); hi2a = RFL(hi2a); lo2b = RFL(lo2b); hi2b = RFL(hi2b);
        in10 = g >= lo10 && g <= hi10; in2a = g >= lo2a && g <= hi2a; in2b = g >= lo2b && g <= hi2b;
        msk = __builtin_amdgcn_ballot_w64(!(in10 && in2a && in2b)) != 0ull;
    }
    Q4 Lmx[XK ? 1 : B], Lmo1[B], Lmo2[B], Li1[N1], Ld1[N1], Li2[N2], Ld2[N2];
    unsigned ld_lanes10 = 64u, ld_lanes2 = 64u;
    if (TIGHT && msk) {
#pragma unroll
        for (int j = 0; j < B; j++) { Lmo1[j] = nulq; Lmo2[j] = nulq; }
#pragma unroll
        for (int j = 0; j < N1; j++) { Li1[j] = nulq; Ld1[j] = nulq; }
#pragma unroll
        for (int j = 0; j < N2; j++) { Li2[j] = nulq; Ld2[j] = nulq; }
        if constexpr (IMMR) {
            if (in10) {
#pragma unroll
                for (int j = 0; j < B; j++) Lmo1[j] = q4_from(ild<OT, ST>(R, bM1, lane_b, j - KBLK_C));
#pragma unroll
                for (int j = 0; j < N1; j++) { Li1[j] = q4_from(ild_nt<OT, ST>(R, bI1, lane_b, j)); Ld1[j] = q4_from(ild_nt<OT, ST>(R, bD1, lane_b, j)); }
                if (TWO) {
#pragma unroll
                    for (int j = 0; j < N2; j++) { Li2[j] = q4_from(ild_nt<OT, ST>(R, bI2, lane_b, j)); Ld2[j] = q4_from(ild_nt<OT, ST>(R, bD2, lane_b, j)); }
                }
            }
            if (TWO && in2a) {
#pragma unroll
                for (int j = 0; j < PF && j < 5; j++) Lmo2[j] = q4_from(ild_nt<OT, ST>(R, bM2a, lane_b, j));
            }
        }
        ld_lanes10 = (unsigned)__popcll(__builtin_amdgcn_ballot_w64(in10)); ld_lanes2 = (unsigned)__popcll(__builtin_amdgcn_ballot_w64(in2a));
    } else {
#pragma unroll
    for (int j = 0; j < B; j++) {
        if constexpr (!IDONLY && !XK) Lmx[XK ? 0 : j] = LDQ(s0 + j - pen.x, SR_C_M);
        if constexpr (IMMR) {
            Lmo1[j] = q4_from(ild<OT, ST>(R, bM1, lane_b, j - KBLK_C));
            if (TWO && j < PF) Lmo2[j] = q4_from(ild_nt<OT, ST>(R, j < 5 ? bM2a : bM2b, lane_b, j < 5 ? j : j - 5));
        } else {
            Lmo1[j] = LDQ(s0 + j - pen.o1 - E1, SR_C_M);
            if (TWO && j < PF) Lmo2[j] = LDQ_NT(s0 + j - pen.o2 - E2, SR_C_M);
        }
    }
#pragma unroll
    for (int j = 0; j < N1; j++) {
        if constexpr (IMMR) {
            Li1[j] = q4_from(ild_nt<OT, ST>(R, bI1, lane_b, j)); Ld1[j] = q4_from(ild_nt<OT, ST>(R, bD1, lane_b, j));
        } else {
            Li1[j] = LDQ_NT(s0 + j - E1, SR_C_I1);
            Ld1[j] = LDQ_NT(s0 + j - E1, SR_C_D1);
        }
    }
    if (TWO) {
#pragma unroll
        for (int j = 0; j < N2; j++) {
            if constexpr (IMMR) {
                Li2[j] = q4_from(ild_nt<OT, ST>(R, bI2, lane_b, j)); Ld2[j] = q4_from(ild_nt<OT, ST>(R, bD2, lane_b, j));
            } else {
                Li2[j] = LDQ_NT(s0 + j - E2, SR_C_I2);
                Ld2[j] = LDQ_NT(s0 + j - E2, SR_C_D2);
            }
        }
    }
    }
    const bool with_u = (chk < 0) && (R.urow != 0u) && rec;
    {
        const int nown = min(OWN, max(0, ghi - (glo + ti * OWN) + 1));
        const int n10 = ((!IDONLY && !XK) ? B : 0) + B + 2 * N1 + (TWO ? 2 * N2 : 0);
        const int n2f = TWO ? (PF < B ? PF : B) : 0, n2p = TWO ? B - n2f : 0;
        int nst = (IDONLY ? 0 : B) + (with_u ? 1 : 0);
#pragma unroll
        for (int j = 0; j < B; j++) {
            nst += (j + E1 >= B || rec) ? 2 : 0;
            if (TWO) nst += (j + E2 >= B || rec) ? 2 : 0;
        }
        row_ld += ld_lanes10 * (unsigned)n10 + ld_lanes2 * (unsigned)n2f + 64u * (unsigned)(n2p + (IDONLY ? B : 0) + ((with_u && s0 > 0) ? 1 : 0));
        row_st += (unsigned)nown * (unsigned)nst;
    }
    Q4 uacc = nulq;
    Q4 Lown[IDONLY ? B : 1];
    if (IDONLY) {
#pragma unroll
        for (int j = 0; j < B; j++) {
            if constexpr (IMMR) Lown[IDONLY ? j : 0] = q4_from(ild<OT, ST>(R, sM, lane_b, j - KBLK_C));
            else Lown[IDONLY ? j : 0] = LDQ(s0 + j, SR_C_M);
        }
    }
    if (with_u) {
        const int gplo = RFL(k_sh.jgplo[tix]), gphi = RFL(k_sh.jgphi[tix]);
        if (s0 > 0 && g >= gplo && g <= gphi) uacc = q4_from(rld_raw16(R, R.urow, idx0));
    }
    const bool deep = s0 >= (BIAS ? SR_DEEP_RING16 : SR_DEEP_INT16);
    if (deep) {
#pragma unroll
        for (int j = 0; j < B; j++) {
            if (XK) { if (j + OE1 - X < B && j + OE1 - X >= 0 && j < X) Lmo1[(XK && j + OE1 - X < B) ? j + OE1 - X : 0] = q4_renull<NUL, BIAS>(Lmo1[(XK && j + OE1 - X < B) ? j + OE1 - X : 0]); }
            else if (!IDONLY) Lmx[XK ? 0 : j] = q4_renull<NUL, BIAS>(Lmx[XK ? 0 : j]);
        }
#pragma unroll
        for (int j = 0; j < N1; j++) { Li1[j] = q4_renull<NUL, BIAS>(Li1[j]); Ld1[j] = q4_renull<NUL, BIAS>(Ld1[j]); }
        if (TWO) {
#pragma unroll
            for (int j = 0; j < N2; j++) { Li2[j] = q4_renull<NUL, BIAS>(Li2[j]); Ld2[j] = q4_renull<NUL, BIAS>(Ld2[j]); }
        }
    }
    Q4 Lb;
    {
        int l[4];
#pragma unroll
        for (int q = 0; q < 4; q++) l[q] = max(min(tlen, plen + k0 + q), -1) - BIAS;
        Lb.a = h2_pack(l[0], l[1]); Lb.b = h2_pack(l[2], l[3]);
    }
    const int cp0 = p0 - k0 + BIAS + (int)(((uint32_t)(uintptr_t)P >> 2) << SR_WIN_LOG);
    const int ct0 = t0 + BIAS + (int)(((uint32_t)(uintptr_t)T >> 2) << SR_WIN_LOG);
    const int cpb0 = cp0 << SR_SYM_LOG, cpb1 = (cp0 - 1) << SR_SYM_LOG, cpb2 = (cp0 - 2) << SR_SYM_LOG, cpb3 = (cp0 - 3) << SR_SYM_LOG;
    const int ctb = ct0 << SR_SYM_LOG;
    const unsigned long long ownb = __builtin_amdgcn_ballot_w64(owned);
    Q4 kk;
    kk.a = h2_pack(k0, k0 + 1); kk.b = h2_pack(k0 + 2, k0 + 3);
    int klo0 = RFL(k_sh.jklo[0][tix]), khi0 = RFL(k_sh.jkhi[0][tix]);
    if constexpr (!RING) { klo0 = max(klo0, RFL(k_sh.jklo[B - 1][tix])); khi0 = min(khi0, RFL(k_sh.jkhi[B - 1][tix])); }
    const bool inside = __builtin_amdgcn_ballot_w64(!(k0 >= klo0 && k0 + 3 <= khi0)) == 0ull;
    Q4 hI1[B], hD1[B], hI2[B], hD2[B], mvh[XK ? B : 1];
#pragma unroll
    for (int j = 0; j < B; j++) {
        const int s = s0 + j;
        int klo = 0, khi = 0;
        if (!inside || chk >= 0 || (j == 0 && s0 == 0)) { klo = RFL(k_sh.jklo[j][tix]); khi = RFL(k_sh.jkhi[j][tix]); }
        if (TWO && XK && j + PF < B) {
            if constexpr (IMMR) Lmo2[j + PF < B ? j + PF : 0] = q4_from(ild_nt<OT, ST>(R, j + PF < 5 ? bM2a : bM2b, kopaque_v(lane_b), j + PF < 5 ? j + PF : j + PF - 5));
            else Lmo2[j + PF < B ? j + PF : 0] = LDQ_NT(s0 + j + PF - pen.o2 - E2, SR_C_M);
        }
        if (TIGHT && TWO && msk && j >= PF) {
            const bool in_ = j < 5 ? in2a : in2b;
            const Q4 nq = nulq;
            Lmo2[j].a = in_ ? Lmo2[j].a : nq.a; Lmo2[j].b = in_ ? Lmo2[j].b : nq.b;
        }
        const unsigned lane_j = IMMR ? kopaque_v(lane_b) : 0u;
        Q4 Lj = Lb;
        if (!inside) {
            int l[4];
#pragma unroll
            for (int q = 0; q < 4; q++) { const int k = k0 + q; l[q] = (k >= klo && k <= khi) ? q4_get(Lb, q) : -32768; }
            Lj.a = h2_pack(l[0], l[1]); Lj.b = h2_pack(l[2], l[3]);
        }
        Q4 mx, mo1 = Lmo1[j], si1, sd1, mo2 = nulq, si2 = nulq, sd2 = nulq;
        if (IDONLY) mx = nulq;
        else if (!XK) mx = Lmx[XK ? 0 : j];
        else if (j >= X) mx = mvh[(XK && j >= X) ? j - X : 0];
        else mx = Lmo1[(XK && j + OE1 - X < B) ? j + OE1 - X : 0];
        if (j < N1) { si1 = Li1[j < N1 ? j : 0]; sd1 = Ld1[j < N1 ? j : 0]; }
        else { si1 = hI1[j >= E1 ? j - E1 : 0]; sd1 = hD1[j >= E1 ? j - E1 : 0]; }
        if (TWO) {
            mo2 = Lmo2[j];
            if (j < N2) { si2 = Li2[j < N2 ? j : 0]; sd2 = Ld2[j < N2 ? j : 0]; }
            else { si2 = hI2[j >= E2 ? j - E2 : 0]; sd2 = hD2[j >= E2 ? j - E2 : 0]; }
        }
        Q4 i1 = q4_bound<NUL>(q4_inc(q4_from_left(q4_max(mo1, si1))), Lj);
        Q4 d1 = q4_bound<NUL>(q4_from_right(q4_max(mo1, sd1)), Lj);
// ... 28 lines not shown
                bp[0] = bit_index<0>(mwa, cpb0); bp[1] = bit_index<1>(mwa, cpb1); bp[2] = bit_index<0>(mwb, cpb2); bp[3] = bit_index<1>(mwb, cpb3);
                bt[0] = bit_index_u<0>(mwa, ctb); bt[1] = bit_index_u<1>(mwa, ctb); bt[2] = bit_index_u<0>(mwb, ctb); bt[3] = bit_index_u<1>(mwb, ctb);
#ifdef SR_BOUNDS
                {
                    const unsigned lo_ = (unsigned)(uintptr_t)lds_seq;
                    const unsigned seq_hi = lo_ + RFL(k_sh.lds_seq_bytes);
#pragma unroll
                    for (int q = 0; q < 4; q++) {
                        const int mvq = q4_get(m, q);
                        if (owned && mvq >= -BIAS && mvq <= q4_get(Lb, q)) {
                            const unsigned ap = ((unsigned)bp[q] >> 3) & ~3u, at = ((unsigned)bt[q] >> 3) & ~3u;
                            if (ap < lo_ || ap + 8u > seq_hi) kbnd_fail(3u, ap, seq_hi);
                            if (at < lo_ || at + 8u > seq_hi) kbnd_fail(3u, at, seq_hi);
                        }
                    }
                }
#endif
#pragma unroll
                for (int q = 0; q < 4; q++) { win_words_bit(bp[q], pl[q], ph[q]); win_words_bit(bt[q], tl[q], th[q]); }
                asm volatile("; 8 windows in flight" : "+v"(pl[0]), "+v"(ph[0]), "+v"(pl[1]), "+v"(ph[1]), "+v"(pl[2]), "+v"(ph[2]), "+v"(pl[3]), "+v"(ph[3]),
                                                        "+v"(tl[0]), "+v"(th[0]), "+v"(tl[1]), "+v"(th[1]), "+v"(tl[2]), "+v"(th[2]), "+v"(tl[3]), "+v"(th[3]));
#pragma unroll
                for (int q = 0; q < 4; q++) {
                    const int nn = q4_get(Lb, q) - mv[q];
                    const uint32_t xw = __builtin_amdgcn_alignbit(ph[q], pl[q], (uint32_t)bp[q]) ^
                                        __builtin_amdgcn_alignbit(th[q], tl[q], (uint32_t)bt[q]);
                    const int ext_ = (int)min3u(ffs_sym(xw), (unsigned)SR_WIN, (unsigned)nn);
                    mv[q] += ext_;
                    pend[q] = __builtin_amdgcn_ballot_w64(ext_ == SR_WIN) & __builtin_amdgcn_ballot_w64(mv[q] >= -BIAS) & ownb;
                }
            }
            while ((pend[0] | pend[1] | pend[2] | pend[3]) != 0ull) {
#pragma unroll
                for (int q = 0; q < 4; q++) {
                    if (pend[q] == 0ull) continue;
                    const int nn = lanes_or_zero(pend[q], q4_get(Lb, q) - mv[q]);
                    const uint32_t xw = win_sym(mv[q] + cp0 - q) ^ win_sym(mv[q] + ct0);
                    mv[q] += (int)min3u(ffs_sym(xw), (unsigned)SR_WIN, (unsigned)nn);
                    pend[q] = __builtin_amdgcn_ballot_w64(xw == 0u && nn > SR_WIN);
                }
            }
            m.a = h2_pack_perm(mv[0], mv[1]); m.b = h2_pack_perm(mv[2], mv[3]);
            if (XK) mvh[XK ? j : 0] = m;
            int ak;
            if constexpr (BIAS == 0) {
                typedef unsigned short __attribute__((ext_vector_type(2))) U2;
                const uint32_t va = ~h2_u(m.a >> (H2){15, 15}), vb = ~h2_u(m.b >> (H2){15, 15});
                const uint32_t aa = h2_u(m.a + m.a - kk.a) & va, ab = h2_u(m.b + m.b - kk.b) & vb;
                const uint32_t mx2 = __builtin_bit_cast(uint32_t, __builtin_elementwise_max(__builtin_bit_cast(U2, aa), __builtin_bit_cast(U2, ab)));
                ak = owned ? (int)max(mx2 >> 16, mx2 & 0xffffu) : 0;
            } else {
                ak = 0;
#pragma unroll
                for (int q = 0; q < 4; q++) ak = max(ak, mv[q] >= -BIAS ? 2 * (mv[q] + BIAS) - (k0 + q) : 0);
                ak = owned ? ak : 0;
            }
            uacc = q4_max(uacc, m);
            if (j == 0 && s0 == 0) uacc = TWO ? q4_max(uacc, q4_max(q4_max(i1, i2), q4_max(d1, d2))) : q4_max(uacc, q4_max(i1, d1));
            if (chk >= 0) {
                const int qe = kend - k0;
                if (owned && qe >= 0 && qe < 4 && kend >= klo && kend <= khi) {
                    const uint32_t wa = (chk == SR_C_I1) ? h2_u(i1.a) : (chk == SR_C_I2) ? h2_u(i2.a) : (chk == SR_C_D1) ? h2_u(d1.a)
                                      : (chk == SR_C_D2) ? h2_u(d2.a) : h2_u(m.a);
                    const uint32_t wb = (chk == SR_C_I1) ? h2_u(i1.b) : (chk == SR_C_I2) ? h2_u(i2.b) : (chk == SR_C_D1) ? h2_u(d1.b)
                                      : (chk == SR_C_D2) ? h2_u(d2.b) : h2_u(m.b);
                    const uint32_t w = (qe & 2) ? wb : wa;
                    const int val = (int)(short)((qe & 1) ? (w >> 16) : (w & 0xffffu));
                    if (val + BIAS >= tlen) k_sh.jreach[j][jid] = 1;
                }
            }
            ak = row16_max_nn(ak);
            if ((lane & 15) == 15 && ak > 0) atomicMax(&k_sh.jak[j][jid], ak);
        } else {
            uacc = q4_max(uacc, Lown[IDONLY ? j : 0]);
            if (j == 0 && s0 == 0) uacc = TWO ? q4_max(uacc, q4_max(q4_max(i1, i2), q4_max(d1, d2))) : q4_max(uacc, q4_max(i1, d1));
        }
        if (owned) {
            if constexpr (IMMR) {
                const int im = j - KBLK_C;
                const bool l1 = j + E1 >= B, l2 = j + E2 >= B;
                if (!IDONLY) ist<OT, ST>(R, sM, lane_j, im, q4_vec(m));
                if (l1) { ist<OT, ST>(R, sI1, lane_j, im, q4_vec(i1)); ist<OT, ST>(R, sD1, lane_j, im, q4_vec(d1)); }
                if (TWO && l2) { ist<OT, ST>(R, sI2, lane_j, im, q4_vec(i2)); ist<OT, ST>(R, sD2, lane_j, im, q4_vec(d2)); }
                if (rec && (!l1 || (TWO && !l2))) {
                    const unsigned lane_r = kopaque_v(lane_b);
                    if (!l1) { ist_nt<OT, ST>(R, sI1, lane_r, im, q4_vec(i1)); ist_nt<OT, ST>(R, sD1, lane_r, im, q4_vec(d1)); }
                    if (TWO && !l2) { ist_nt<OT, ST>(R, sI2, lane_r, im, q4_vec(i2)); ist_nt<OT, ST>(R, sD2, lane_r, im, q4_vec(d2)); }
                }
            } else {
            if (!IDONLY) rst<OT>(R, KROW(s, SR_C_M), idx0, q4_vec(m));
            if (j + E1 < B) { if (rec) { rst_nt<OT>(R, KROW(s, SR_C_I1), idx0, q4_vec(i1)); rst_nt<OT>(R, KROW(s, SR_C_D1), idx0, q4_vec(d1)); } }
            else { rst<OT>(R, KROW(s, SR_C_I1), idx0, q4_vec(i1)); rst<OT>(R, KROW(s, SR_C_D1), idx0, q4_vec(d1)); }
            if (TWO) {
                if (j + E2 < B) { if (rec) { rst_nt<OT>(R, KROW(s, SR_C_I2), idx0, q4_vec(i2)); rst_nt<OT>(R, KROW(s, SR_C_D2), idx0, q4_vec(d2)); } }
                else { rst<OT>(R, KROW(s, SR_C_I2), idx0, q4_vec(i2)); rst<OT>(R, KROW(s, SR_C_D2), idx0, q4_vec(d2)); }
            }
            }
        }
    }
    if (with_u && owned) rst_raw16(R, R.urow, idx0, q4_vec(uacc));
#undef KROW
#undef LDQ
#undef LDQ_NT
}

template <typename OT, bool TWO, int B, int E1, int E2, bool IDONLY, int X, int OE1, typename ST = OT, bool RING = false>
__device__ __forceinline__ void blk_tile_any(const KRows<OT, ST> &R, const int s0, const int slot0, const SrPen &pen,
                                             const int jid, const int ti, const int tix, unsigned &row_ld, unsigned &row_st) {
    if constexpr (sizeof(OT) == 2 && (X > 0 || B >= 5)) blk_tile16<TWO, B, E1, E2, IDONLY, X, OE1, RING>(R, s0, slot0, pen, jid, ti, tix, row_ld, row_st);
    else if constexpr (KPK_U16_OF(OT, ST, B, X) && RING) blk_tile16<TWO, B, E1, E2, IDONLY, X, OE1, true, KRows<OT, ST>, SR_RING_BIAS>(R, s0, slot0, pen, jid, ti, tix, row_ld, row_st);
    else blk_tile<OT, TWO, B, E1, E2, IDONLY, X, OE1>(R, s0, slot0, pen, jid, ti, tix, row_ld, row_st);
}
```

seqrush_amd/csrc/sr_host.cpp:

```cpp
#include <hip/hip_runtime_api.h>
#include <algorithm>
#include <chrono>
#include <climits>
#include <functional>
#include <queue>
#include <cmath>
#include <cstdio>
#include <cstdlib>
#include <cstring>
#include <string>
#include <unordered_map>
#include <unordered_set>
#include <vector>
#include "../../include/seqrush_amd.h"
#include "sr_internal.h"
#include "sr_graph.h"
#include "sr_sort.h"
#include "sr_compact.h"
#include "sr_iter_rule.h"
#include "sr_inv_rule.h"
#include "sr_base_cone.h"
#include "sr_mirror_rule.h"
#include "sr_prio_rule.h"

static thread_local std::string g_err;
static int fail(int code, const std::string &msg) { g_err = msg; return code; }
int sr_fail(int code, const std::string &msg) { return fail(code, msg); }
extern "C" const char *sr_last_error(void) { return g_err.c_str(); }

struct SrKnob { const char *name, *unset, *doc; };
static const SrKnob SR_KNOBS[] = {
    {"SR_ALIGN_IMPL", "2 when the penalties have a blocked instance", "1 = level-per-pass kernel (sr_align_bfs_kernel), 2 = score-blocked kernel"},
    {"SR_BLK_LEVELS", "10 for x=5, o1+e1=10", "5 = generic 5-level blocked instance instead of the exact 10-level one"},
    {"SR_ALIGN_THREADS", "by pairs per CU", "threads per workgroup: 64 | 128 | 256 | 512 | 1024"},
    {"SR_WG_PER_CU", "4", "workgroups per CU the launch is sized for"},
    {"SR_NWG", "CUs x workgroups per CU", "cap on workgroups (several pairs per workgroup on small inputs)"},
    {"SR_RING_U16", "1 below 57 k", "0 = 32-bit searches keep 32-bit ring rows"},
    {"SR_LAZY_ID", "1", "0 = searches store their I/D rows from the first level (no recompute pass)"},
    {"SR_HIST_JOBS", "4", "worst-case base cases the per-workgroup history holds (1..16)"},
    {"SR_BFS_BASE_JOBS", "16 (lean builds 4 / 8)", "base cases per batch"},
    {"SR_CIGAR_ARENA_OPS", "25 % of free memory", "CIGAR arena in ops (tests: force batches)"},
    {"SR_POISON_ROWS", "off", "fill the row workspaces with this offset before the run (stale-row tests)"},
    {"SR_PREORIENT", "by pairs per CU and LDS", "1 / 0 = orientation as its own kernel / inside the alignment kernel"},
    {"SR_NO_REORDER", "off", "keep list order instead of the cost-sorted dequeue order"},
    {"SR_ORIENT_LEVELS", "off", "orientation level by level even for the default penalties"},
    {"SR_NO_KBITS", "off", "no q-gram bound in the orientation kernel"},
    {"SR_NO_MIRROR", "off", "1 = no pair has a mirror partner: (q, t) and (t, q) are both aligned (A/B runs, tests)"},
    {"SR_MIRROR_REPLAY", "on", "0 = a tied secondary is aligned in full: its primary keeps no breakpoint records and none is matched (A/B runs, tests)"},
    {"SR_NO_FUSED_UNITE", "off", "sr_ctx_run launches sr_unite_kernel per batch instead of uniting inside the blocked alignment kernel"},
    {"SR_PROFILE_TICKS", "0", "1 = launch the instrumented instance (100 MHz tick counters, per-workgroup timeline)"},
    {"SR_TAIL", "on", "0 = no tail launch: a tied secondary is always aligned by its primary's workgroup (A/B runs); all = every such secondary is deferred to the tail launch (tests)"},
    {"SR_TAIL_THREADS", "widest instance wider than the main launch", "threads per workgroup of the tail launch among the existing instances: 256 | 512 | 1024 (tests)"},
    {"SR_TILE_PRIO", "1", "0 = no rotating tile priority among the workgroups of a CU: all tile code at priority 0, no clock read (A/B runs, tests)"},
    {"SR_TAIL_ROUNDS", "8", "a batch defers only when its alignments are at most this many times the launch's workgroups"},
    {"SR_FORCE_INT32", "off", "tests: 32-bit offsets (and the 16-bit ring of 32-bit searches) whatever the sequence length"},
    {"SR_TEST_BASE_LEVELS", "off", "tests: cap on the levels a base case is given at first (forces the re-queue path)"},
    {"SR_BOUNDS_DETAIL", "off", "1 = (bounds-checked build) keep the first offending access in counters[40..43]"},
};
static const char *knob(const char *name) {
    for (const SrKnob &k : SR_KNOBS)
        if (!strcmp(k.name, name)) return getenv(name);
    fprintf(stderr, "seqrush_amd: internal error: environment knob %s is not in SR_KNOBS\n", name);
    abort();
}
static std::string knobs_json() {
    std::string out = "{";
    for (const SrKnob &k : SR_KNOBS)
        if (const char *v = getenv(k.name)) {
            if (out.size() > 1) out += ", ";
            out += std::string("\"") + k.name + "\": \"";
            for (const char *q = v; *q; q++) if (*q != '"' && *q != '\\' && (unsigned char)*q >= 32) out += *q;
            out += "\"";
        }
    return out + "}";
}
extern "C" const char *sr_knobs_doc(void) {
    static std::string doc;
    if (doc.empty())
        for (const SrKnob &k : SR_KNOBS) doc += std::string(k.name) + "\t" + k.unset + "\t" + k.doc + "\n";
    return doc.c_str();
}
extern "C" int sr_abi_version(void) { return SR_ABI_VERSION; }
extern "C" void sr_free(void *p) { free(p); }
extern "C" int sr_device_count(void) {
    int n = 0;
    if (hipGetDeviceCount(&n) != hipSuccess) return 0;
    return n;
}

#define HIPCHK(expr)                                                                     \
    do {                                                                                 \
        hipError_t _e = (expr);                                                          \
        if (_e != hipSuccess)                                                            \
            return fail(SR_ERR_HIP, std::string(#expr) + ": " + hipGetErrorString(_e));  \
    } while (0)

extern "C" void sr_default_params(sr_params *p) {
    memset(p, 0, sizeof(*p));
    p->match_score = 0; p->mismatch_penalty = 5; p->gap_open1 = 8; p->gap_ext1 = 2;
    p->gap_open2 = 24; p->gap_ext2 = 1;
    p->ori_match = 0; p->ori_mismatch = 1; p->ori_gap_open = 1; p->ori_gap_ext = 1;
    p->min_match_len = 0; p->max_divergence = -1.0; p->exclude_self = 0;
    p->memory_mode = SR_MEM_ULTRALOW; p->sparsify_kind = SR_SPARSE_NONE; p->sparsify_factor = 1.0;
    p->sparsify_seed = 42; p->canonical_labels = 0; p->device = 0;
    p->shard_rank = 0; p->shard_count = 1;
    p->tree_k_nearest = 0; p->tree_k_farthest = 0; p->tree_rand_frac = 0.0; p->tree_kmer = 16;
}

static bool parse_i32(const std::string &s, int32_t *out) {
    if (s.empty() || s.size() > 15) return false;
    size_t i = (s[0] == '+' || s[0] == '-') ? 1 : 0;
    if (i == s.size()) return false;
    for (size_t j = i; j < s.size(); j++) if (s[j] < '0' || s[j] > '9') return false;
    long long v = atoll(s.c_str());
    if (v > INT32_MAX || v < INT32_MIN) return false;
    *out = (int32_t)v;
    return true;
}
static std::vector<std::string> split(const std::string &s, char c) {
    std::vector<std::string> out;
    size_t st = 0;
    for (;;) {
        size_t p = s.find(c, st);
        if (p == std::string::npos) { out.push_back(s.substr(st)); break; }
        out.push_back(s.substr(st, p - st));
        st = p + 1;
    }
    return out;
}

extern "C" int sr_parse_scores(const char *s, sr_params *p) {
    auto parts = split(s, ',');
    if (parts.size() < 4)
        return fail(SR_ERR_INVALID, "Scores must have at least 4 values: match,mismatch,gap1_open,gap1_extend");
    if (parts.size() > 6) return fail(SR_ERR_INVALID, "Too many score values provided (max 6)");
    int32_t v[6] = {0, 0, 0, 0, -1, -1};
// ... 29 lines not shown
    *out = v;
    return true;
}

extern "C" int sr_parse_sparsification(const char *cs, sr_params *p) {
    std::string s(cs);
    if (s == "none" || s == "1.0") { p->sparsify_kind = SR_SPARSE_NONE; return SR_OK; }
    if (s == "auto") { p->sparsify_kind = SR_SPARSE_AUTO; return SR_OK; }
    double f;
    if (s.rfind("random:", 0) == 0) {
        if (!parse_f64(s.substr(7), &f)) return fail(SR_ERR_INVALID, "Invalid random factor: " + s);
        if (f > 0.0 && f <= 1.0) { p->sparsify_kind = SR_SPARSE_RANDOM; p->sparsify_factor = f; return SR_OK; }
        return fail(SR_ERR_INVALID, "Random factor must be in (0.0, 1.0]");
    }
    if (s.rfind("connectivity:", 0) == 0) {
        if (!parse_f64(s.substr(13), &f)) return fail(SR_ERR_INVALID, "Invalid connectivity probability: " + s);
        if (f > 0.0 && f <= 1.0) { p->sparsify_kind = SR_SPARSE_CONNECTIVITY; p->sparsify_factor = f; return SR_OK; }
        return fail(SR_ERR_INVALID, "Connectivity probability must be in (0.0, 1.0]");
    }
    if (s.rfind("tree:", 0) == 0) {
        auto parts = split(s.substr(5), ',');
        if (parts.empty() || parts.size() > 4)
            return fail(SR_ERR_INVALID, "Tree sampling requires 1-4 values: tree:neighbor[,stranger[,random[,k-mer]]], got " + s);
        auto parse_usize = [](const std::string &t, uint64_t *v) {
            size_t i = (!t.empty() && t[0] == '+') ? 1 : 0;
            if (i >= t.size()) return false;
            *v = 0;
            for (; i < t.size(); i++) {
                if (t[i] < '0' || t[i] > '9') return false;
                const uint64_t dgt = (uint64_t)(t[i] - '0');
                if (*v > (0xffffffffffffffffULL - dgt) / 10) return false;
                *v = *v * 10 + dgt;
            }
            return true;
        };
        uint64_t kn = 0, kf = 0, km = 16;
        double rf = 0.0;
        if (!parse_usize(parts[0], &kn)) return fail(SR_ERR_INVALID, "Invalid neighbor count: " + parts[0]);
        if (parts.size() >= 2 && !parse_usize(parts[1], &kf)) return fail(SR_ERR_INVALID, "Invalid stranger count: " + parts[1]);
        if (parts.size() >= 3) {
            if (!parse_f64(parts[2], &rf)) return fail(SR_ERR_INVALID, "Invalid random fraction: " + parts[2]);
            if (rf < 0.0 || rf > 1.0) return fail(SR_ERR_INVALID, "Random fraction must be in [0.0, 1.0], got " + parts[2]);
        }
        if (parts.size() >= 4) {
            if (!parse_usize(parts[3], &km)) return fail(SR_ERR_INVALID, "Invalid k-mer size: " + parts[3]);
            if (km == 0) return fail(SR_ERR_INVALID, "K-mer size must be > 0");
        }
        p->sparsify_kind = SR_SPARSE_TREE;
        p->tree_k_nearest = (uint32_t)std::min<uint64_t>(kn, 0xffffffffULL);
        p->tree_k_farthest = (uint32_t)std::min<uint64_t>(kf, 0xffffffffULL);
        p->tree_rand_frac = rf; p->tree_kmer = (uint32_t)std::min<uint64_t>(km, 0xffffffffULL);
        return SR_OK;
    }
    if (parse_f64(s, &f) && f > 0.0 && f <= 1.0) { p->sparsify_kind = SR_SPARSE_RANDOM; p->sparsify_factor = f; return SR_OK; }
    return fail(SR_ERR_INVALID, "Invalid sparsification: '" + s + "'");
}

static int32_t max_score_for_divergence(const sr_params &p, uint64_t seq_len, double d) {
    int32_t max_mismatches = (int32_t)std::ceil((double)seq_len * d);
    int32_t max_gaps = (int32_t)std::ceil((double)seq_len * d * 0.5);
    int32_t mismatch_score = max_mismatches * p.mismatch_penalty;
    int32_t gap_score = max_gaps > 0 ? p.gap_open1 + (max_gaps - 1) * p.gap_ext1 : 0;
    return std::max(mismatch_score + gap_score, p.mismatch_penalty * 2);
}

#define SR_TAIL_ROUNDS_DEFAULT 8

struct sr_ctx {
    int device = 0;
    hipStream_t stream = nullptr;
    bool own_stream = false;
    sr_params prm;
    uint32_t n = 0;
    std::vector<uint32_t> len;
    std::vector<uint64_t> goff;
    uint64_t total_len = 0, uf_size = 0;
    std::vector<uint32_t> pair_q, pair_t;
    std::vector<uint64_t> cigar_base;
    std::vector<uint32_t> batch_first;
    uint64_t total_pairs_all_ranks = 0;
    uint64_t dp_cells = 0;
    int off16 = 1, nwg = 0, nthreads = 256, symbits = 2;
    size_t lds_bytes = 0;
    SrAlignArgs aa{};
    SrUniteArgs ua{};
    std::vector<void *> dev_allocs;
    unsigned long long *d_nodes = nullptr, *d_minarr = nullptr, *d_labels = nullptr;
    unsigned long long *d_counters = nullptr;
    int *d_error = nullptr;
    uint32_t *d_queue = nullptr, *d_oqueue = nullptr, *d_order = nullptr;
    uint64_t *d_okeys = nullptr, *d_okeys2 = nullptr;
    uint32_t *d_ovals = nullptr; void *d_otemp = nullptr; size_t otemp_bytes = 0;
    uint64_t *d_cbase = nullptr;
    uint8_t *d_bases = nullptr;
    int onwg = 0;
    size_t olds_bytes = 0;
    int32_t *d_max_score = nullptr;
    uint32_t *d_mirror = nullptr;
    uint64_t mirror_partners = 0;
    int tail_threads = 0, tail_wg_per_cu = 1, tail_rounds = SR_TAIL_ROUNDS_DEFAULT, tail_cus = 0;
    bool tail_all = false;
    std::vector<uint32_t> batch_partners;
    uint32_t *d_tail_list = nullptr, *d_tail_deferred = nullptr;
    unsigned long long *d_timeline = nullptr;
    int prio_rounds = SR_TAIL_ROUNDS_DEFAULT;
    uint32_t *d_cu_arrivals = nullptr;
    unsigned long long *d_prio_timeline = nullptr;
    std::vector<std::pair<hipEvent_t, hipEvent_t>> ev[5];
    int ev_used[5] = {0, 0, 0, 0, 0};
    bool loaded = false;
    bool fuse_unite = false;
    bool from_paf = false;
    bool aligned_batch_valid = false;
    std::string workspace_report;
    bool iter_loaded = false, iter_keep = false, iter_ran = false;
    uint64_t iter_tree_pairs = 0;
    uint32_t iter_tree_batches = 0, iter_max_chunks = 0;
    sr_iter_stats iter_stats{};
    std::vector<uint64_t> iter_counts;
    SrIterState *d_iter_state = nullptr;
    unsigned long long *d_iter_counts = nullptr;
    sr_alignments *iter_al = nullptr;
    bool inv_on = false, inv_keep = false;
    uint64_t inv_m = 0;
    uint32_t *d_inv_count = nullptr, *d_inv_off = nullptr;
    unsigned long long *d_inv_stats = nullptr;
    SrInvJob *d_inv_jobs = nullptr;
    uint64_t inv_job_cap = 0;
    std::vector<SrInvJob> inv_raw;
    std::vector<sr_inv_job> inv_jobs;
    sr_inv_stats inv_stats{};
    sr_alignments *inv_al = nullptr;
    std::vector<std::pair<hipEvent_t, hipEvent_t>> inv_ev;
    uint32_t inv_join = 0;
    SrInvJobJ *d_inv_jobs_j = nullptr;
    uint64_t inv_job_cap_j = 0;
    std::vector<SrInvJobJ> inv_raw_j;
    uint64_t inv_join_stats[4] = {0, 0, 0, 0};
    std::chrono::steady_clock::time_point t_first_kernel;
    int inv_ev_used = 0;
};

static int dev_alloc(sr_ctx *c, void **p, size_t bytes) {
    hipError_t e = hipMalloc(p, bytes ? bytes : 16);
    if (e != hipSuccess) {
        char buf[160];
        snprintf(buf, sizeof(buf), "hipMalloc of %zu bytes failed: %s", bytes, hipGetErrorString(e));
        return fail(e == hipErrorOutOfMemory ? SR_ERR_NOMEM : SR_ERR_HIP, buf);
    }
    c->dev_allocs.push_back(*p);
    return SR_OK;
}
static void free_dev(sr_ctx *c) {
    for (void *p : c->dev_allocs) (void)hipFree(p);
    c->dev_allocs.clear();
    c->d_nodes = c->d_minarr = c->d_labels = c->d_counters = nullptr;
    c->d_error = nullptr; c->d_queue = nullptr; c->d_oqueue = nullptr; c->d_order = nullptr; c->d_cbase = nullptr;
    c->d_bases = nullptr; c->d_max_score = nullptr; c->d_mirror = nullptr; c->mirror_partners = 0; c->onwg = 0;
    c->tail_threads = 0; c->tail_all = false; c->batch_partners.clear(); c->d_tail_list = c->d_tail_deferred = nullptr; c->d_timeline = nullptr;
    c->d_cu_arrivals = nullptr; c->d_prio_timeline = nullptr;
    c->d_okeys = c->d_okeys2 = nullptr; c->d_ovals = nullptr; c->d_otemp = nullptr; c->otemp_bytes = 0;
    c->loaded = false; c->from_paf = false; c->aligned_batch_valid = false;
    for (int k = 0; k < 5; k++) c->ev_used[k] = 0;
    c->iter_loaded = c->iter_keep = c->iter_ran = false; c->iter_tree_pairs = 0; c->iter_tree_batches = c->iter_max_chunks = 0;
    c->iter_counts.clear(); c->d_iter_state = nullptr; c->d_iter_counts = nullptr; c->iter_stats = sr_iter_stats{};
    if (c->iter_al) { sr_alignments_free(c->iter_al); c->iter_al = nullptr; }
// ... 456 lines not shown
    for (uint32_t b = 0; b < nbatch; b++)
        if (batch_first[b] > batch_first[b + 1]) return fail(SR_ERR_INVALID, "batches do not cover the pair list");
    const uint64_t n = mirror_map(query_idx, target_idx, batch_first, nbatch, workgroups, mirror_out);
    if (partners_out) *partners_out = n;
    return SR_OK;
}
extern "C" int sr_mirror_bt_pick(const int *off, int transposed) {
    int bo = -1, bty = 0;
    for (int tag = 1; tag <= 9; tag++) {
        if (off[tag] < 0) continue;
        const int r = transposed ? sr_mirror_bt_rank_t(tag) : tag, rb = transposed ? sr_mirror_bt_rank_t(bty) : bty;
        if (off[tag] > bo || (off[tag] == bo && r > rb)) { bo = off[tag]; bty = tag; }
    }
    return bty;
}
extern "C" int sr_mirror_bt_rank_transposed(int tag) { return sr_mirror_bt_rank_t(tag); }
extern "C" int sr_mirror_bt_tie_host(const int *off) {
    int bo = -1, bty = 0, bi = -1;
    for (int tag = 1; tag <= 9; tag++) {
        if (off[tag] < 0) continue;
        if (tag <= SR_BT_I2_EXT && off[tag] > bi) bi = off[tag];
        if (off[tag] > bo || (off[tag] == bo && tag > bty)) { bo = off[tag]; bty = tag; }
    }
    return bty != 0 && sr_mirror_bt_tie(bty, bo, bi) ? 1 : 0;
}
extern "C" int sr_mirror_bp_pick_host(const int *val, const int *dist, const int *comp, const int *diag, int n, int value_bias,
                                      int *pick_out, int *pick_t_out) {
    unsigned long long best = ~0ull, best_t = ~0ull;
    *pick_out = *pick_t_out = -1;
    for (int j = 0; j < n; j++) {
        const unsigned long long k = sr_mirror_bp_key((unsigned)(val[j] + value_bias), dist[j], comp[j], diag[j]);
        const unsigned long long kt = sr_mirror_bp_key_t((unsigned)(val[j] + value_bias), dist[j], comp[j], diag[j]);
        if (k < best) { best = k; *pick_out = j; }
        if (kt < best_t) { best_t = kt; *pick_t_out = j; }
    }
    return n > 0 && sr_mirror_bp_tie(best, best_t) ? 1 : 0;
}
extern "C" int sr_replay_record_ints(void) { return SR_BPREC_INTS; }
extern "C" void sr_replay_transpose_host(const int *rec, int *out) {
    for (int f = 0; f < SR_BPREC_INTS; f++) out[f] = sr_bprec_t(rec, f);
}
extern "C" int sr_replay_match_host(const int *recs, int nrec, const int *segs, int nseg, int level, int *match_out) {
    int rd = 0, n = 0;
    while (rd < nrec && recs[rd * SR_BPREC_INTS + SR_BR_LEVEL] < level) rd++;
    for (int p = 0; p < nseg; p++) {
        const int *e = segs + 6 * p;
        match_out[p] = -1;
        while (rd < nrec) {
            const int *r = recs + rd * SR_BPREC_INTS;
            if (r[SR_BR_LEVEL] != level) break;
            const int c = sr_replay_cmp(r, e);
            if (c > 0) break;
            rd++;
            if (c < 0) continue;
            if (r[SR_BR_TIE] == 0 && sr_replay_same(r, e)) { match_out[p] = rd - 1; n++; }
            break;
        }
    }
    return n;
}

static size_t align_static_lds(bool wave_wg, int impl, int nthreads) {
    return (size_t)(wave_wg ? 6 : impl != 2 ? 28 : nthreads >= 1024 ? 34 : nthreads >= 512 ? 28 : 25) * 1024;
}
static int tail_shape(int impl, int kblock, int wave_wg, int off16, int ring_u16, int symbits, int two, int main_threads,
                      uint32_t max_words, int forced) {
    if (impl != 2 || kblock != 10 || wave_wg) return 0;
    if (!off16 && !ring_u16 && forced < 256) return 0;
    static const int shapes[3] = {1024, 512, 256};
    for (int nt : shapes) {
        if (forced > 0 ? nt > forced : nt <= main_threads) continue;
        if (nt == 1024 && !(off16 && symbits == 2 && two)) continue;
        if (nt == 512 && !(off16 || ring_u16)) continue;
        if ((size_t)max_words * 16 + 16 + align_static_lds(false, 2, nt) > 128 * 1024) continue;
        return nt;
    }
    return 0;
}
extern "C" int sr_tail_shape(int impl, int kblock, int wave_wg, int off16, int ring_u16, int symbits, int two, int main_threads,
                             uint32_t max_words, int forced) {
    return tail_shape(impl, kblock, wave_wg, off16, ring_u16, symbits, two, main_threads, max_words, forced);
}

static int plan_kernel(sr_ctx *c, const PackedSeqs &pk, const SrPen &pen, const SrPen &ori, uint64_t maxlen, uint32_t np, Plan &pl) {
    hipDeviceProp_t prop;
    HIPCHK(hipGetDeviceProperties(&prop, c->device));
    pl.cus = prop.multiProcessorCount > 0 ? prop.multiProcessorCount : 256;
    const int cus = pl.cus, bits = pk.sm.bits;
    c->off16 = maxlen <= 32000 ? 1 : 0;
    if (knob("SR_FORCE_INT32")) c->off16 = 0;
    pl.osz = c->off16 ? 2 : 4;
    pl.max_words = (uint32_t)((maxlen + pk.per_word - 1) / pk.per_word + 2);
    c->lds_bytes = (size_t)pl.max_words * 3 * 4;
    if ((long long)c->lds_bytes > (long long)srk_align_max_lds())
        return fail(SR_ERR_UNSUPPORTED, "sequences too long to stage in LDS (limit 177456 / 88728 / 44364 symbols per sequence at 2 / 4 / 8 bits per symbol)");
    pl.impl = 1;
    pl.kblock = srk_align_blk_supports(&pen, &ori);
    if (const char *e = knob("SR_BLK_LEVELS")) { if (atoi(e) == 5 && pl.kblock == 10) pl.kblock = 5; }
    if (pl.kblock > 0 && (long long)pl.max_words * 16 + 28 * 1024 <= 128 * 1024) pl.impl = 2;
    if (const char *e = knob("SR_ALIGN_IMPL")) { if (atoi(e) <= 1) pl.impl = 1; }
    int &impl = pl.impl, &kblock = pl.kblock;
    if (impl == 2) c->lds_bytes = (size_t)pl.max_words * 4 * 4 + 16;
    pl.wg_per_cu = 4;
    if (const char *e = knob("SR_WG_PER_CU")) pl.wg_per_cu = std::max(1, atoi(e));
    c->nthreads = 256;
    if (impl == 2 && (uint64_t)np <= 2ULL * (uint64_t)cus + (uint64_t)cus / 2) c->nthreads = 512;
    if (impl == 2 && (uint64_t)np <= (uint64_t)cus) c->nthreads = 1024;
    if (const char *e = knob("SR_ALIGN_THREADS")) {
        const int v = atoi(e);
        if (v == 128 || v == 256 || v == 512 || (v == 1024 && impl == 2) || (v == 64 && impl == 2 && bits == 2)) c->nthreads = v;
    }
    if (c->nthreads == 1024 && !(impl == 2 && kblock == 10 && c->off16 && bits == 2 && pen.two)) c->nthreads = 512;
    if (impl == 2 && c->nthreads == 128 && kblock == 10 && !(bits == 2 && c->off16)) kblock = 5;
    pl.wave_wg = impl == 2 && (c->nthreads == 64 || (c->nthreads == 128 && kblock == 10));
    if (pl.wave_wg) pl.wg_per_cu = c->nthreads == 64 ? 16 : 8;
    auto static_lds = [&](int nthreads) -> size_t { return align_static_lds(pl.wave_wg, impl, nthreads); };
    const size_t lds_per_wg = c->lds_bytes + static_lds(c->nthreads);
    pl.wg_per_cu = (int)std::min<size_t>((size_t)pl.wg_per_cu, std::max<size_t>(1, (160 * 1024) / lds_per_wg));
    const char *ru = knob("SR_RING_U16");
    const bool u16_ok = kblock == 10 && maxlen <= 57000 && !(ru && atoi(ru) == 0);
    if (impl == 2 && !pl.wave_wg && pl.wg_per_cu <= 2 && !knob("SR_ALIGN_THREADS") && (c->off16 || u16_ok)) c->nthreads = 512;
    pl.wg_per_cu = (int)std::min<size_t>((size_t)pl.wg_per_cu, std::max<size_t>(1, (160 * 1024) / (c->lds_bytes + static_lds(c->nthreads))));
    pl.ring_u16 = (impl == 2 && !c->off16 && u16_ok && c->nthreads >= 256) ? 1 : 0;
    if (impl == 2 && !pl.wave_wg && !c->off16 && !pl.ring_u16) c->nthreads = 256;
    pl.rsz = pl.ring_u16 ? 2 : pl.osz;
    pl.bbase_jobs = pl.wave_wg ? (c->nthreads == 64 ? 4 : 8) : 16;
    if (const char *e = knob("SR_BFS_BASE_JOBS")) pl.bbase_jobs = std::max(1, std::min(16, atoi(e)));
    const char *tl = knob("SR_TAIL"), *tt = knob("SR_TAIL_THREADS");
    pl.tail_threads = (tl && !strcmp(tl, "0")) ? 0
                      : tail_shape(impl, kblock, pl.wave_wg, c->off16, pl.ring_u16, bits, pen.two, c->nthreads, pl.max_words, tt ? std::max(1, atoi(tt)) : 0);
    return SR_OK;
}

static int plan_workspace(const sr_ctx *c, const SrPen &pen, const SrPen &ori, uint64_t maxlen, Plan &pl) {
    const int impl = pl.impl, kblock = pl.kblock;
    pl.ring_scope = std::max(pen.scope, ori.scope);
    int emax = std::max(pen.e1, ori.e1);
    if (pen.two) emax = std::max(emax, pen.e2);
    pl.ring_hot = emax + 2;
    const int gapmax = pen.two ? std::max(pen.o1, pen.o2) : pen.o1;
    auto gc = [&](int len) { int g = pen.o1 + pen.e1 * len; if (pen.two) g = std::min(g, pen.o2 + pen.e2 * len); return g; };
    const int smax_base = std::max(250 + gapmax, 2 * gc(100)) + 2 * gapmax + 4;
    pl.hist_levels = smax_base + 1 + std::max(kblock, 5);
    int rmax = smax_base / pen.e1;
    if (pen.two) rmax = std::max(rmax, smax_base / pen.e2);
    pl.hist_w = (2 * (rmax + pen.scope + 2) + 1 + 8 + 64 + 7) & ~7;
    pl.brow = (int)((4 * maxlen + 32 * 72 + 64 + 512 + 7) & ~7ULL);
    pl.kdepth = std::max(pen.scope + std::max(kblock, 1), ori.scope + 1) + 1;
    const char *lz = knob("SR_LAZY_ID");
    pl.lazy_id = (impl == 2 && !(lz && atoi(lz) == 0) && 2 * pen.scope + 2 * kblock + 2 <= SR_BLK_MAK_SLOTS) ? 1 : 0;
    pl.kdepth2 = pl.kdepth;
    if (pl.lazy_id) {
        pl.kdepth2 = std::max(pl.kdepth, pen.scope + 2 * kblock + 2);
        pl.kdepth = std::max(pl.kdepth, 2 * pen.scope + 2 * kblock + 2);
    }
    if (impl == 2 && kblock == 10) {
        pl.kdepth = (pl.kdepth + 9) / 10 * 10; pl.kdepth2 = (pl.kdepth2 + 9) / 10 * 10;
    }
    pl.bring_wg = ((uint64_t)(pl.ring_scope + 1) + 4ULL * pl.ring_hot + 4ULL * (pl.ring_scope + 1) + 2ULL) * (uint64_t)pl.brow;
    if (impl == 2) pl.bring_wg = ((uint64_t)pl.brow / 256 + 2ULL) * ((uint64_t)pl.kdepth + 4ULL * pl.kdepth2 + (uint64_t)SR_NULL_ROWS + 2ULL) * 256ULL + 1024;
    if (impl == 2 && pl.bring_wg * pl.rsz >= (1ULL << 32)) return fail(SR_ERR_UNSUPPORTED, "sequences too long for the device row workspace (4 GB per workgroup)");
    const uint64_t hist_worst = (uint64_t)pl.hist_levels * 5 * (uint64_t)pl.hist_w;
    pl.hist_cap = hist_worst * 4;
    if (const char *e = knob("SR_HIST_JOBS")) pl.hist_cap = hist_worst * (uint64_t)std::max(1, std::min(16, atoi(e)));
    pl.hist_nul_w = impl == 2 ? (uint64_t)pl.hist_w + 256 : (uint64_t)pl.bbase_jobs * (uint64_t)pl.hist_w;
    pl.bhist_wg = impl == 2 ? ((pl.hist_cap + pl.hist_nul_w + 256 + 1024 + 7) & ~7ULL)
                            : ((uint64_t)pl.hist_levels * 5 + 1) * pl.hist_nul_w + 1024;
    pl.bseg_wg = 2ULL * SR_BFS_MAXSEG * SR_BFS_SEGREC * 4;
    pl.bbt_wg = (uint64_t)pl.bbase_jobs * SR_BFS_BTCAP * 4;
    pl.brec_wg = impl == 2 ? (uint64_t)SR_BPREC_MAX * SR_BPREC_INTS * 4 : 0;
    pl.bcl_wg = 0;
    pl.per_wg_bytes = pl.bring_wg * pl.rsz + pl.bhist_wg * pl.osz + pl.bseg_wg + pl.bbt_wg + pl.bcl_wg * 4 + (impl == 2 ? 32 * SR_BLK_MAK_SLOTS * 4 : 0) +
                      pl.brec_wg;
    (void)c;
    return SR_OK;
}

static int plan_memory(sr_ctx *c, uint32_t np, Plan &pl, bool iterative = false) {
    size_t total_b = 0;
    HIPCHK(hipMemGetInfo(&pl.free_b, &total_b));
    const uint64_t fixed = 3ULL * c->uf_size * 8 + (uint64_t)np * 40 + (1ULL << 20);
    if (fixed + (64ULL << 20) > pl.free_b) return fail(SR_ERR_NOMEM, "not enough device memory for the union-find arrays");
    const uint64_t avail = pl.free_b - fixed;
    pl.arena_ops = c->cigar_base[np] + 1;
    {
        uint64_t cap = std::max<uint64_t>((uint64_t)(avail * 0.25) / 4, pl.max_reserve + 1);
        if (const char *e = knob("SR_CIGAR_ARENA_OPS")) cap = std::max<uint64_t>((uint64_t)atoll(e), pl.max_reserve + 1);
        if (iterative)
            for (uint64_t f = c->iter_tree_pairs; f < np; f += 4 * SR_ITER_CHECK_INTERVAL)
                cap = std::max<uint64_t>(cap, c->cigar_base[std::min<uint64_t>(np, f + 4 * SR_ITER_CHECK_INTERVAL)] - c->cigar_base[f] + 1);
        pl.arena_ops = std::min(pl.arena_ops, cap);
    }
    if (pl.arena_ops * 4 > avail / 2) return fail(SR_ERR_NOMEM, "not enough device memory for one pair's CIGAR");
    c->batch_first.assign(1, 0);
    const uint32_t tp = iterative ? (uint32_t)c->iter_tree_pairs : np;
    for (uint32_t i = 0; i < tp; i++)
        if (c->cigar_base[i + 1] - c->cigar_base[c->batch_first.back()] + 1 > pl.arena_ops) c->batch_first.push_back(i);
    if (iterative) {
        if (tp > 0 && tp < np) c->batch_first.push_back(tp);
        c->iter_tree_batches = tp == 0 ? 0 : (tp < np ? (uint32_t)c->batch_first.size() - 1 : (uint32_t)c->batch_first.size());
        const uint32_t CH = 4 * SR_ITER_CHECK_INTERVAL;
        uint64_t target = SR_ITER_STABILITY_THRESHOLD;
        c->iter_max_chunks = 0;
        for (uint32_t f = tp; f < np;) {
            uint32_t l = f, chunks = 0;
            while (l < np && (chunks == 0 || chunks < target)) {
                const uint32_t e = std::min(np, l + CH);
                if (chunks > 0 && c->cigar_base[e] - c->cigar_base[f] + 1 > pl.arena_ops) break;
                l = e; chunks++;
            }
            c->iter_max_chunks = std::max(c->iter_max_chunks, chunks);
            if (l < np) c->batch_first.push_back(l);
            f = l;
            target = std::min<uint64_t>(2 * target, 1ULL << 32);
        }
    } else {
        c->iter_tree_batches = 0;
    }
    c->batch_first.push_back(np);
    pl.nbatch = (uint32_t)c->batch_first.size() - 1;
    pl.max_batch_pairs = 0;
    for (uint32_t b = 0; b < pl.nbatch; b++) pl.max_batch_pairs = std::max(pl.max_batch_pairs, c->batch_first[b + 1] - c->batch_first[b]);
    pl.left = avail - pl.arena_ops * 4;
    const uint64_t budget = (uint64_t)(pl.left * 0.7);
    int nwg = pl.cus * pl.wg_per_cu;
    if (const char *e = knob("SR_NWG")) nwg = std::max(1, std::min(nwg, atoi(e)));
    if ((uint64_t)nwg > pl.max_batch_pairs) nwg = (int)pl.max_batch_pairs;
    if (nwg < 1) nwg = 1;
    while (nwg > 1 && (uint64_t)nwg * pl.per_wg_bytes > budget) nwg--;
    if ((uint64_t)nwg * pl.per_wg_bytes > budget) return fail(SR_ERR_NOMEM, "not enough device memory for one workgroup's wavefront ring");
    pl.nwg = c->nwg = nwg;
    return SR_OK;
}

static int alloc_workspace(sr_ctx *c, const sr_params *p, const PackedSeqs &pk, const SeqDev &sd, const SrPen &pen, const SrPen &ori,
                           uint64_t maxlen, const std::vector<int32_t> &max_score, Plan &pl, bool forced_strand = false) {
    int r;
    void *d;
    const uint32_t np = (uint32_t)c->pair_q.size(), nbatch = pl.nbatch;
    const int impl = pl.impl, nwg = pl.nwg;
    const size_t osz = pl.osz, rsz = pl.rsz;
    SrAlignArgs &a = c->aa;
    memset(&a, 0, sizeof(a));
    uint32_t *d_pq, *d_pt;
    std::vector<uint32_t> pq = c->pair_q, pt = c->pair_t;
    if (pq.empty()) { pq.push_back(0); pt.push_back(0); }
    DEV_UPLOAD(d_pq, uint32_t, pq);
    DEV_UPLOAD(d_pt, uint32_t, pt);
    std::vector<uint64_t> cb((size_t)np + nbatch, 0);
    for (uint32_t b = 0; b < nbatch; b++) {
        const uint32_t f = c->batch_first[b], l = c->batch_first[b + 1];
        for (uint32_t i = f; i <= l; i++) cb[(size_t)i + b] = c->cigar_base[i] - c->cigar_base[f];
    }
    DEV_UPLOAD(c->d_cbase, uint64_t, cb);
    std::vector<uint32_t> order(std::max<uint32_t>(np, 1), 0);
    for (uint32_t b = 0; b < nbatch; b++) {
        const uint32_t f = c->batch_first[b], l = c->batch_first[b + 1];
        std::vector<uint32_t> idx(l - f);
        for (uint32_t i = 0; i < l - f; i++) idx[i] = i;
        auto cost = [&](uint32_t i) { const uint32_t q = c->pair_q[f + i], t = c->pair_t[f + i];
                                      return q == t ? (uint64_t)c->len[q] : (uint64_t)c->len[q] * c->len[t]; };
        std::stable_sort(idx.begin(), idx.end(), [&](uint32_t x, uint32_t y) { return cost(x) > cost(y); });
        for (uint32_t i = 0; i < l - f; i++) order[f + i] = idx[i];
    }
    DEV_UPLOAD(c->d_order, uint32_t, order);
    DEV_UPLOAD(c->d_max_score, int32_t, max_score);
    std::vector<uint32_t> mirror;
    c->mirror_partners = 0;
    if (impl == 2 && pk.sm.bits == 2 && !forced_strand && np > 0) {
        mirror.assign(np, SR_MIRROR_NONE);
        if (!knob("SR_NO_MIRROR")) c->mirror_partners = mirror_map(c->pair_q.data(), c->pair_t.data(), c->batch_first.data(), nbatch, (uint32_t)nwg, mirror.data());
        DEV_UPLOAD(c->d_mirror, uint32_t, mirror);
    }
    c->batch_partners.assign(nbatch, 0);
    uint32_t max_partners = 0;
    for (uint32_t b = 0; b < nbatch && !mirror.empty(); b++) {
        for (uint32_t i = c->batch_first[b]; i < c->batch_first[b + 1]; i++)
            if (mirror[i] != SR_MIRROR_NONE && !(mirror[i] & SR_MIRROR_SECONDARY)) c->batch_partners[b]++;
        max_partners = std::max(max_partners, c->batch_partners[b]);
    }
    HIPCHK(hipStreamSynchronize(c->stream));
    if ((r = dev_alloc(c, &d, 4 * sizeof(uint32_t)))) return r; c->d_queue = (uint32_t *)d;
    c->tail_threads = c->mirror_partners > 0 ? pl.tail_threads : 0;
    pl.tail_threads = c->tail_threads;
    if (c->tail_threads) {
        c->tail_wg_per_cu = (int)std::max<size_t>(1, std::min<size_t>((size_t)1024 / c->tail_threads,
                                                                      (160 * 1024) / (c->lds_bytes + align_static_lds(false, 2, c->tail_threads))));
        const char *tl = knob("SR_TAIL"), *tr = knob("SR_TAIL_ROUNDS");
        c->tail_all = tl && !strcmp(tl, "all");
        c->tail_rounds = tr ? std::max(0, atoi(tr)) : SR_TAIL_ROUNDS_DEFAULT;
        c->tail_cus = pl.cus;
        if ((r = dev_alloc(c, &d, (size_t)max_partners * 4))) return r; c->d_tail_list = (uint32_t *)d;
        if ((r = dev_alloc(c, &d, sizeof(uint32_t)))) return r; c->d_tail_deferred = (uint32_t *)d;
        HIPCHK(hipMemsetAsync(c->d_tail_deferred, 0, sizeof(uint32_t), c->stream));
    }
    if (impl == 2 && knob("SR_PROFILE_TICKS") && atoi(knob("SR_PROFILE_TICKS")) != 0) {
        if ((r = dev_alloc(c, &d, (size_t)nwg * 4 * 8))) return r; c->d_timeline = (unsigned long long *)d;
        HIPCHK(hipMemsetAsync(c->d_timeline, 0, (size_t)nwg * 4 * 8, c->stream));
        if ((r = dev_alloc(c, &d, (size_t)nwg * 4 * 8))) return r; c->d_prio_timeline = (unsigned long long *)d;
        HIPCHK(hipMemsetAsync(c->d_prio_timeline, 0, (size_t)nwg * 4 * 8, c->stream));
    }
    if (impl == 2) {
        if ((r = dev_alloc(c, &d, SR_PRIO_TABLE * sizeof(uint32_t)))) return r; c->d_cu_arrivals = (uint32_t *)d;
        HIPCHK(hipMemsetAsync(c->d_cu_arrivals, 0, SR_PRIO_TABLE * sizeof(uint32_t), c->stream));
        const char *tp = knob("SR_TILE_PRIO");
        a.prio_wg = std::max(1, std::min(pl.wg_per_cu, 1024 / std::max(64, c->nthreads)));
        a.tile_prio = (a.prio_wg > 1 && !(tp && atoi(tp) == 0)) ? 1 : 0;
        const char *trk = knob("SR_TAIL_ROUNDS");
        c->prio_rounds = trk ? std::max(0, atoi(trk)) : SR_TAIL_ROUNDS_DEFAULT;
    }
    if ((r = dev_alloc(c, &d, (uint64_t)nwg * pl.bring_wg * rsz))) return r; a.bring = d;
    if ((r = dev_alloc(c, &d, (uint64_t)nwg * pl.bhist_wg * osz))) return r; a.bhist = d;
    if (const char *e = knob("SR_POISON_ROWS")) {
        const int v = atoi(e);
        if (rsz == 2) HIPCHK(hipMemsetD16Async((hipDeviceptr_t)a.bring, (unsigned short)(pl.ring_u16 ? v - 24576 : v), (size_t)nwg * pl.bring_wg, c->stream));
        else HIPCHK(hipMemsetD32Async((hipDeviceptr_t)a.bring, v, (size_t)nwg * pl.bring_wg, c->stream));
        if (osz == 2) HIPCHK(hipMemsetD16Async((hipDeviceptr_t)a.bhist, (unsigned short)v, (size_t)nwg * pl.bhist_wg, c->stream));
        else HIPCHK(hipMemsetD32Async((hipDeviceptr_t)a.bhist, v, (size_t)nwg * pl.bhist_wg, c->stream));
    }
    if ((r = dev_alloc(c, &d, (uint64_t)nwg * pl.bseg_wg))) return r; a.bseg = (int *)d;
    if ((r = dev_alloc(c, &d, (uint64_t)nwg * pl.bbt_wg))) return r; a.bbt = (uint32_t *)d;
    {
        const char *rpk = knob("SR_MIRROR_REPLAY");
        pl.brec_bytes = 0;
        if (impl == 2 && c->mirror_partners > 0 && pl.brec_wg && !(rpk && atoi(rpk) == 0)) {
            pl.brec_bytes = (uint64_t)nwg * pl.brec_wg;
            if ((r = dev_alloc(c, &d, pl.brec_bytes))) return r; a.brec = (int *)d;
        }
    }
    if (pl.bcl_wg) { if ((r = dev_alloc(c, &d, (uint64_t)nwg * pl.bcl_wg * 4))) return r; a.bcl = (uint32_t *)d; a.bcl_wg_stride = pl.bcl_wg; }
    if (impl == 2) { if ((r = dev_alloc(c, &d, (uint64_t)nwg * 32 * SR_BLK_MAK_SLOTS * 4))) return r; a.bmak = (int *)d; }
    const char *po = knob("SR_PREORIENT");
    const bool pre_auto = (uint64_t)np >= 4ULL * (uint64_t)pl.cus && (size_t)pl.max_words * 12 <= 20 * 1024;
    if (!forced_strand && impl == 2 && (po ? atoi(po) != 0 : pre_auto) && (size_t)pl.max_words * 12 <= 60 * 1024) {
        const int orow = (int)((2 * ((2 * maxlen + 32) & ~3ULL) + 512 + 7) & ~7ULL);
        const uint64_t oring_wg = ((uint64_t)(ori.scope + 1) * 3 + 1) * (uint64_t)orow + 256;
        int onwg = (int)std::min<uint64_t>(pl.max_batch_pairs, (uint64_t)pl.cus * 16);
        while (onwg > 1 && (uint64_t)onwg * oring_wg * osz > (uint64_t)(pl.left * 0.2)) onwg--;
        if (onwg >= 1 && np > 0) {
            pl.oring_bytes = (uint64_t)onwg * oring_wg * osz;
            if ((r = dev_alloc(c, &d, pl.oring_bytes))) return r; a.oring = d;
            if ((r = dev_alloc(c, &d, sizeof(uint32_t)))) return r; c->d_oqueue = (uint32_t *)d;
            a.oring_wg_stride = oring_wg; a.orow = orow; a.oqueue = c->d_oqueue; a.pre_oriented = 1;
            if (!knob("SR_NO_REORDER")) {
                c->otemp_bytes = srk_order_temp_bytes(pl.max_batch_pairs);
                if ((r = dev_alloc(c, &d, (uint64_t)pl.max_batch_pairs * 8))) return r; c->d_okeys = (uint64_t *)d;
                if ((r = dev_alloc(c, &d, (uint64_t)pl.max_batch_pairs * 8))) return r; c->d_okeys2 = (uint64_t *)d;
                if ((r = dev_alloc(c, &d, (uint64_t)pl.max_batch_pairs * 4))) return r; c->d_ovals = (uint32_t *)d;
                if ((r = dev_alloc(c, &d, std::max<size_t>(c->otemp_bytes, 16)))) return r; c->d_otemp = d;
            }
            c->onwg = onwg; c->olds_bytes = (size_t)pl.max_words * 3 * 4;
        }
    }
    if ((r = dev_alloc(c, &d, (size_t)np + 1))) return r; a.is_reverse = (uint8_t *)d;
    if ((r = dev_alloc(c, &d, ((size_t)np + 1) * 4))) return r; a.score = (int32_t *)d;
    if ((r = dev_alloc(c, &d, ((size_t)np + 1) * 4))) return r; a.ori_fwd = (int32_t *)d;
    if ((r = dev_alloc(c, &d, ((size_t)np + 1) * 4))) return r; a.ori_rev = (int32_t *)d;
    if ((r = dev_alloc(c, &d, ((size_t)np + 1) * 4))) return r; a.cigar_cnt = (uint32_t *)d;
    if ((r = dev_alloc(c, &d, (pl.arena_ops + 1) * 4))) return r; a.cigar_ops = (uint32_t *)d;
    if ((r = dev_alloc(c, &d, SR_NCOUNTERS * sizeof(unsigned long long)))) return r; c->d_counters = (unsigned long long *)d;
    if ((r = dev_alloc(c, &d, sizeof(int)))) return r; c->d_error = (int *)d;
    if ((r = dev_alloc(c, &d, c->uf_size * 8))) return r; c->d_nodes = (unsigned long long *)d;
    if ((r = dev_alloc(c, &d, c->uf_size * 8))) return r; c->d_minarr = (unsigned long long *)d;
    if ((r = dev_alloc(c, &d, c->uf_size * 8))) return r; c->d_labels = (unsigned long long *)d;
    HIPCHK(hipMemsetAsync(c->d_counters, 0, SR_NCOUNTERS * sizeof(unsigned long long), c->stream));
    HIPCHK(hipMemsetAsync(c->d_error, 0, sizeof(int), c->stream));
    HIPCHK(hipMemsetAsync(a.cigar_cnt, 0, ((size_t)np + 1) * 4, c->stream));
    HIPCHK(hipMemsetAsync(a.score, 0xff, ((size_t)np + 1) * 4, c->stream));
    if (forced_strand) {
        HIPCHK(hipMemsetAsync(a.is_reverse, 0, (size_t)np + 1, c->stream));
        HIPCHK(hipMemsetAsync(a.ori_fwd, 0, ((size_t)np + 1) * 4, c->stream));
        HIPCHK(hipMemsetAsync(a.ori_rev, 0, ((size_t)np + 1) * 4, c->stream));
    }
    a.seqwords = sd.words; a.word_off_fwd = sd.woff[0]; a.word_off_rc = sd.woff[1]; a.word_off_rev = sd.woff[2]; a.word_off_cmp = sd.woff[3];
    if (forced_strand) { if (impl == 2) a.pre_oriented = 1; else a.word_off_rc = a.word_off_fwd; }
    a.symbits = pk.sm.bits; a.order = c->d_order; a.seqlen = sd.len;
    a.max_words = pl.max_words; a.pair_q = d_pq; a.pair_t = d_pt; a.npairs = np;
    a.queue_head = c->d_queue; a.pen = pen; a.ori = ori; a.mem_mode = p->memory_mode;
    a.ring_scope = pl.ring_scope; a.ring_hot = pl.ring_hot;
    a.hist_w = pl.hist_w; a.hist_levels = pl.hist_levels;
    { const char *pt_ = knob("SR_PROFILE_TICKS"); a.profile_ticks = (pt_ && atoi(pt_) != 0) ? 1 : 0; }
    a.impl = impl; a.kdepth = pl.kdepth; a.kdepth2 = pl.kdepth2; a.kblock = pl.kblock; a.lazy_id = pl.lazy_id; a.ring_u16 = pl.ring_u16;
    a.ori_levels = knob("SR_ORIENT_LEVELS") ? 1 : 0;
    { const char *tb = knob("SR_TEST_BASE_LEVELS"); a.test_base_levels = tb ? std::max(0, atoi(tb)) : 0; }
    a.bring_wg_stride = pl.bring_wg; a.brow = pl.brow; a.bhist_wg_stride = pl.bhist_wg; a.bbase_jobs = pl.bbase_jobs;
    a.hist_cap = pl.hist_cap; a.hist_nul_w = (uint32_t)pl.hist_nul_w; a.hist_stride = (uint32_t)((uint64_t)pl.bbase_jobs * (uint64_t)pl.hist_w);
    a.cigar_base = c->d_cbase; a.counters = c->d_counters; a.error_flag = c->d_error;
    if (a.pre_oriented && pk.sm.bits == 2 && !ori.two && ori.x == 1 && ori.o1 == 1 && ori.e1 == 1 && !knob("SR_NO_KBITS") && !knob("SR_ORIENT_LEVELS")) {
        const uint64_t kb = (uint64_t)c->len.size() * 8192ull;
        if (kb > 0 && kb <= (256ull << 20) && kb <= (uint64_t)(pl.left * 0.05)) {
            if ((r = dev_alloc(c, &d, kb))) return r;
            if ((r = srk_kmer_bits(&a, (uint32_t)c->len.size(), (uint32_t *)d, c->stream))) return fail(SR_ERR_DEVICE_FAULT, "k-mer set kernel failed to launch");
            a.kbits = (const uint32_t *)d;
        }
    }
    SrUniteArgs &u = c->ua;
    memset(&u, 0, sizeof(u));
    u.pair_q = d_pq; u.pair_t = d_pt; u.npairs = np; u.seqlen = sd.len; u.seq_goff = sd.goff;
    a.fuse_unite = 0; a.uf_nodes = c->d_nodes; a.seq_goff = sd.goff; a.max_score = c->d_max_score; a.min_match_len = p->min_match_len;
    a.mirror = c->d_mirror;
    a.tail_count = c->d_queue + 1; a.tail_head = c->d_queue + 2; a.tail_deferred = c->d_tail_deferred; a.timeline = c->d_timeline;
    a.cu_arrivals = c->d_cu_arrivals; a.prio_timeline = c->d_prio_timeline;
    c->fuse_unite = impl == 2 && !knob("SR_NO_FUSED_UNITE");
    u.is_reverse = a.is_reverse; u.score = a.score; u.max_score = c->d_max_score;
    u.cigar_ops = a.cigar_ops; u.cigar_base = c->d_cbase; u.cigar_cnt = a.cigar_cnt;
    u.min_match_len = p->min_match_len; u.nodes = c->d_nodes; u.uf_size = c->uf_size;
    u.counters = c->d_counters; u.error_flag = c->d_error;
    return SR_OK;
}

static void write_report(sr_ctx *c, const PackedSeqs &pk, const SrPen &pen, const Plan &pl) {
    const uint32_t np = (uint32_t)c->pair_q.size();
    char buf[3072];
    const SrPen &ori = c->aa.ori;
    const char *oroute = c->onwg == 0 ? "in-kernel"
                         : (!ori.two && ori.x == 1 && ori.o1 == 1 && ori.e1 == 1 && !knob("SR_ORIENT_LEVELS")) ? "orient-blk" : "orient-levels";
    snprintf(buf, sizeof(buf),
             "{\"pairs\": %u, \"batches\": %u, \"symbol_bits\": %d, \"offset_bytes\": %zu, \"ring_cell_bytes\": %zu, \"kernel_impl\": %d, "
             "\"block_levels\": %d, \"two_piece\": %d, \"lazy_id_rows\": %d, \"workgroups\": %d, "
             "\"threads_per_workgroup\": %d, \"workgroups_per_cu\": %d, \"lds_dynamic_bytes\": %zu, \"ring_bytes_per_workgroup\": %llu, "
             "\"base_history_bytes_per_workgroup\": %llu, \"workspace_bytes\": %llu, \"cigar_arena_bytes\": %llu, "
             "\"orientation_ring_bytes\": %llu, \"union_find_bytes\": %llu, \"device_free_bytes_at_load\": %zu, \"kernel_build\": \"%s\", "
             "\"ring_depth_m\": %d, \"ring_depth_id\": %d, \"fused_unite\": %d, \"wave_build\": %d, \"level_kernel_wide\": %d, "
             "\"profile_ticks\": %d, \"orientation_route\": \"%s\", \"source_digest\": \"%s\", \"mirror_partners\": %llu, \"tail_threads\": %d, \"mirror_replay\": %d, \"replay_record_bytes\": %llu, \"tile_prio\": %d, \"prio_epoch_shift\": %d, \"prio_workgroups_per_cu\": %d, \"knobs\": ",
             np, pl.nbatch, pk.sm.bits, pl.osz, pl.impl == 2 ? pl.rsz : pl.osz, pl.impl, pl.impl == 2 ? pl.kblock : 1, pen.two ? 1 : 0, pl.lazy_id,
             pl.nwg, c->nthreads, pl.wg_per_cu, c->lds_bytes,
             (unsigned long long)(pl.bring_wg * pl.rsz), (unsigned long long)(pl.bhist_wg * pl.osz),
             (unsigned long long)((uint64_t)pl.nwg * pl.per_wg_bytes), (unsigned long long)(pl.arena_ops * 4), (unsigned long long)pl.oring_bytes,
             (unsigned long long)(3ULL * c->uf_size * 8), pl.free_b, srk_align_blk_build_tag(), pl.kdepth, pl.kdepth2, c->fuse_unite ? 1 : 0,
             pl.wave_wg ? 1 : 0, (pl.impl == 1 && pl.ring_scope + 1 > 32) ? 1 : 0, c->aa.profile_ticks, oroute, srk_source_digest(),
             (unsigned long long)c->mirror_partners, c->tail_threads, pl.brec_bytes ? 1 : 0, (unsigned long long)pl.brec_bytes,
             c->aa.tile_prio, SR_PRIO_EPOCH_SHIFT, c->aa.prio_wg);
    c->workspace_report = std::string(buf) + knobs_json() + "}";
}

static int load_impl(sr_ctx *c, const sr_seqset *seqs, const sr_params *p, const uint32_t *eq, const uint32_t *et,
                     uint64_t ecount, bool explicit_pairs, bool iterative = false, bool forced_strand = false) {
    if (!c || !seqs || !p) return fail(SR_ERR_INVALID, "null argument");
    if (seqs->n == 0) return fail(SR_ERR_INVALID, "no sequences");
    HIPCHK(hipSetDevice(c->device));
    HIPCHK(hipStreamSynchronize(c->stream));
    free_dev(c);
    int r;
    SrPen pen, ori;
    uint64_t maxlen = 0;
    if ((r = load_index(c, seqs, p, explicit_pairs, &pen, &ori, &maxlen))) return r;
    PackedSeqs pk;
    pack_sequences(c, seqs, pk);
    c->symbits = pk.sm.bits;
    SeqDev sd;
    if ((r = upload_sequences(c, seqs, pk, sd))) return r;
    Plan pl;
    std::vector<int32_t> max_score;
    if ((r = build_pair_list(c, p, sd, eq, et, ecount, explicit_pairs, max_score, &pl.max_reserve, iterative))) return r;
    const uint32_t np = (uint32_t)c->pair_q.size();
    if ((r = plan_kernel(c, pk, pen, ori, maxlen, np, pl))) return r;
    if ((r = plan_workspace(c, pen, ori, maxlen, pl))) return r;
    if ((r = plan_memory(c, np, pl, iterative))) return r;
    if ((r = alloc_workspace(c, p, pk, sd, pen, ori, maxlen, max_score, pl, forced_strand))) return r;
    write_report(c, pk, pen, pl);
    c->t_first_kernel = std::chrono::steady_clock::now();
    if (srk_uf_init(c->d_nodes, c->total_len, c->uf_size, c->stream)) return fail(SR_ERR_HIP, "uf init launch failed");
    HIPCHK(hipStreamSynchronize(c->stream));
    c->loaded = true;
    return SR_OK;
}
#undef DEV_UPLOAD

extern "C" int sr_ctx_load(sr_ctx *c, const sr_seqset *seqs, const sr_params *p) {
    return load_impl(c, seqs, p, nullptr, nullptr, 0, false);
}
extern "C" int sr_ctx_load_pairs(sr_ctx *c, const sr_seqset *seqs, const sr_params *p, const uint32_t *query_idx,
                                 const uint32_t *target_idx, uint64_t count) {
    if (count && (!query_idx || !target_idx)) return fail(SR_ERR_INVALID, "null pair list");
    return load_impl(c, seqs, p, query_idx, target_idx, count, true);
}

extern "C" int sr_ctx_pairs(const sr_ctx *c, uint32_t **q_out, uint32_t **t_out, uint64_t *count) {
    if (!c || !c->loaded || !q_out || !t_out || !count) return fail(SR_ERR_INVALID, "context not loaded");
    const size_t m = c->pair_q.size();
    *count = m;
    *q_out = (uint32_t *)malloc((m ? m : 1) * 4);
    *t_out = (uint32_t *)malloc((m ? m : 1) * 4);
    memcpy(*q_out, c->pair_q.data(), m * 4);
    memcpy(*t_out, c->pair_t.data(), m * 4);
    return SR_OK;
}
extern "C" int sr_ctx_orientation_scores(sr_ctx *c, int32_t *fwd, int32_t *rev) {
    if (!c || !c->loaded || c->from_paf || !c->aa.ori_fwd) return fail(SR_ERR_INVALID, "context has no alignment stage");
    const size_t np = c->pair_q.size();
    HIPCHK(hipSetDevice(c->device));
    HIPCHK(hipStreamSynchronize(c->stream));
    if (fwd && np) HIPCHK(hipMemcpy(fwd, c->aa.ori_fwd, np * 4, hipMemcpyDeviceToHost));
    if (rev && np) HIPCHK(hipMemcpy(rev, c->aa.ori_rev, np * 4, hipMemcpyDeviceToHost));
    return SR_OK;
}
extern "C" uint32_t sr_ctx_num_batches(const sr_ctx *c) { return (c && c->loaded) ? (uint32_t)c->batch_first.size() - 1 : 0; }
extern "C" const char *sr_ctx_workspace_report(const sr_ctx *c) { return c ? c->workspace_report.c_str() : ""; }

extern "C" int sr_ctx_reset_uf(sr_ctx *c) {
    if (!c || !c->loaded) return fail(SR_ERR_INVALID, "context not loaded");
    HIPCHK(hipSetDevice(c->device));
    if (srk_uf_init(c->d_nodes, c->total_len, c->uf_size, c->stream)) return fail(SR_ERR_HIP, "uf init launch failed");
    return SR_OK;
}

static void batch_args(const sr_ctx *c, uint32_t b, SrAlignArgs *a, SrUniteArgs *u) {
    const uint32_t f = c->batch_first[b], cnt = c->batch_first[b + 1] - f;
    if (a) {
        *a = c->aa;
        a->pair_q += f; a->pair_t += f; a->npairs = cnt; if (a->order) a->order += f;
        a->is_reverse += f; a->score += f; a->ori_fwd += f; a->ori_rev += f; a->cigar_cnt += f;
        if (a->max_score) a->max_score += f;
        if (a->mirror) a->mirror += f;
        a->cigar_base = c->d_cbase + f + b;
    }
    if (u) {
        *u = c->ua;
        u->pair_q += f; u->pair_t += f; u->npairs = cnt; u->is_reverse += f; u->score += f; u->max_score += f;
        u->cigar_cnt += f; u->cigar_base = c->d_cbase + f + b;
        if (u->q_start) { u->q_start += f; u->t_start += f; }
    }
}

static int enqueue_align_batch(sr_ctx *c, uint32_t b, bool fuse_unite = false) {
    SrAlignArgs a;
    batch_args(c, b, &a, nullptr);
    a.fuse_unite = fuse_unite ? 1 : 0;
    const int main_wg = std::min<int>(c->nwg, (int)a.npairs);
    const uint32_t partners = c->tail_threads && b < c->batch_partners.size() ? c->batch_partners[b] : 0;
    const bool defer = partners > 0 && (c->tail_all || (uint64_t)(a.npairs - partners) <= (uint64_t)c->tail_rounds * (uint64_t)main_wg);
    a.tail_list = defer ? c->d_tail_list : nullptr;
    a.tail_mode = defer && c->tail_all ? SR_TAIL_DEFER_ALL : SR_TAIL_MAIN;
    const uint32_t secondaries = b < c->batch_partners.size() ? std::min<uint32_t>(c->batch_partners[b], a.npairs) : 0;
    if ((uint64_t)(a.npairs - secondaries) > (uint64_t)c->prio_rounds * (uint64_t)main_wg) a.tile_prio = 0;
    HIPCHK(hipMemsetAsync(c->d_queue, 0, (c->tail_threads ? 3 : 1) * sizeof(uint32_t), c->stream));
    hipEvent_t *e0, *e1;
    int r;
    if (c->onwg > 0 && a.npairs > 0) {
        HIPCHK(hipMemsetAsync(c->d_oqueue, 0, sizeof(uint32_t), c->stream));
        if ((r = ev_get(c, 4, c->ev_used[4], &e0, &e1))) return r;
        HIPCHK(hipEventRecord(*e0, c->stream));
        r = srk_orient(&a, std::min<int>(c->onwg, (int)a.npairs), c->olds_bytes, c->off16, c->stream);
        if (r) return fail(SR_ERR_HIP, std::string("orientation kernel launch failed: ") + hipGetErrorString((hipError_t)r));
        if (c->d_okeys && a.order) {
            r = srk_order(&a, c->d_okeys, c->d_okeys2, c->d_ovals, c->d_otemp, c->otemp_bytes, (uint32_t *)a.order, c->stream);
            if (r) return fail(SR_ERR_HIP, std::string("dequeue-order sort failed: ") + hipGetErrorString((hipError_t)r));
        }
        HIPCHK(hipEventRecord(*e1, c->stream));
        c->ev_used[4]++;
    }
    if ((r = ev_get(c, 0, c->ev_used[0], &e0, &e1))) return r;
    HIPCHK(hipEventRecord(*e0, c->stream));
    if (a.npairs > 0) {
        if (a.cu_arrivals) HIPCHK(hipMemsetAsync(a.cu_arrivals, 0, SR_PRIO_TABLE * sizeof(uint32_t), c->stream));
        r = srk_align(&a, main_wg, c->lds_bytes, c->off16, c->nthreads, c->stream);
        if (r) return fail(SR_ERR_HIP, std::string("align kernel launch failed: ") + hipGetErrorString((hipError_t)r));
        if (defer) {
            const int grid = (int)std::min<uint64_t>({(uint64_t)c->tail_cus * (uint64_t)c->tail_wg_per_cu, (uint64_t)c->nwg, (uint64_t)partners});
            a.tail_mode = SR_TAIL_RUN; a.timeline = nullptr;
            a.cu_arrivals = nullptr; a.prio_timeline = nullptr; a.tile_prio = 0;
            r = srk_align(&a, grid, c->lds_bytes, c->off16, c->tail_threads, c->stream);
            if (r) return fail(SR_ERR_HIP, std::string("align kernel tail launch failed: ") + hipGetErrorString((hipError_t)r));
        }
    }
    HIPCHK(hipEventRecord(*e1, c->stream));
    c->ev_used[0]++;
    return SR_OK;
}

static int enqueue_unite_batch(sr_ctx *c, uint32_t b, bool fused = false) {
    SrUniteArgs u;
    batch_args(c, b, nullptr, &u);
    hipEvent_t *e0, *e1;
    int r;
    if ((r = ev_get(c, 1, c->ev_used[1], &e0, &e1))) return r;
    HIPCHK(hipEventRecord(*e0, c->stream));
    if (u.npairs > 0 && !fused) {
        int nwg = (int)std::min<uint64_t>(u.npairs, 4096);
        r = srk_unite(&u, nwg, c->stream);
        if (r) return fail(SR_ERR_HIP, std::string("unite kernel launch failed: ") + hipGetErrorString((hipError_t)r));
    }
    HIPCHK(hipEventRecord(*e1, c->stream));
    c->ev_used[1]++;
    return SR_OK;
}

static int begin_pass(sr_ctx *c, bool reset_counters) {
    HIPCHK(hipSetDevice(c->device));
    if (reset_counters) {
        HIPCHK(hipMemsetAsync(c->d_counters, 0, SR_NCOUNTERS * sizeof(unsigned long long), c->stream));
        if (c->d_tail_deferred) HIPCHK(hipMemsetAsync(c->d_tail_deferred, 0, sizeof(uint32_t), c->stream));
        c->ev_used[0] = c->ev_used[4] = 0;
    }
    return SR_OK;
}

extern "C" int sr_ctx_align(sr_ctx *c) {
    if (!c || !c->loaded) return fail(SR_ERR_INVALID, "context not loaded");
    if (c->from_paf) return fail(SR_ERR_INVALID, "context was loaded from a PAF file: there is no alignment stage");
    if (c->batch_first.size() > 2)
        return fail(SR_ERR_UNSUPPORTED, "the pair list runs in several batches that share one CIGAR arena: use sr_ctx_run "
                                        "(align + unite per batch) or sr_align_all");
    int r = begin_pass(c, true);
    if (r) return r;
    if ((r = enqueue_align_batch(c, 0))) return r;
    c->aligned_batch_valid = true;
    return SR_OK;
}

extern "C" int sr_ctx_unite(sr_ctx *c) {
    if (!c || !c->loaded) return fail(SR_ERR_INVALID, "context not loaded");
    if (c->batch_first.size() > 2) return fail(SR_ERR_UNSUPPORTED, "several batches: use sr_ctx_run");
    HIPCHK(hipSetDevice(c->device));
    c->ev_used[1] = 0;
    return enqueue_unite_batch(c, 0);
}

static int inv_begin_run(sr_ctx *c);
static int inv_scan_batch(sr_ctx *c, uint32_t b);
static int inv_patch_pass(sr_ctx *c);

extern "C" int sr_ctx_run(sr_ctx *c) {
    if (!c || !c->loaded) return fail(SR_ERR_INVALID, "context not loaded");
    int r = begin_pass(c, !c->from_paf);
    if (r) return r;
    c->ev_used[1] = 0;
    const uint32_t nbatch = (uint32_t)c->batch_first.size() - 1;
    const bool fuse = c->fuse_unite && !c->from_paf;
    if (c->inv_on && (r = inv_begin_run(c))) return r;
    for (uint32_t b = 0; b < nbatch; b++) {
        if (!c->from_paf && (r = enqueue_align_batch(c, b, fuse))) return r;
        if ((r = enqueue_unite_batch(c, b, fuse))) return r;
        if (c->inv_on && (r = inv_scan_batch(c, b))) return r;
    }
    c->aligned_batch_valid = nbatch == 1 && !c->from_paf;
    if (c->inv_on && (r = inv_patch_pass(c))) return r;
    return SR_OK;
}

extern "C" int sr_ctx_sync(sr_ctx *c) {
    if (!c) return fail(SR_ERR_INVALID, "null ctx");
    HIPCHK(hipSetDevice(c->device));
    HIPCHK(hipStreamSynchronize(c->stream));
    if (c->loaded) {
// ... 1473 lines not shown
```

seqrush_amd/csrc/sr_internal.h:

```cpp
#pragma once
#include <stdint.h>
#include <stddef.h>

#define SR_NULL_OFF (-8192)
#define SR_MAX_SCOPE 127
#define SR_STACK_DEPTH 64
#define SR_WG 256
#define SR_BFS_MAXSEG 4096
#define SR_BFS_SEGREC 16
#define SR_BFS_MAXACT 32
#define SR_BFS_BTCAP 1024
#define SR_NULL_ROWS 10
#define SR_BLK_MAK_SLOTS 80

enum { SR_C_M = 0, SR_C_I1 = 1, SR_C_I2 = 2, SR_C_D1 = 3, SR_C_D2 = 4 };
enum { SR_OP_M = 0, SR_OP_X = 1, SR_OP_I = 2 , SR_OP_D = 3  };

enum {
    SR_DEV_ERR_SCORE_BOUND = 1,
    SR_DEV_ERR_BASE_OVERFLOW = 2,
    SR_DEV_ERR_BACKTRACE = 4,
    SR_DEV_ERR_STACK = 8,
    SR_DEV_ERR_CIGAR_OVERFLOW = 16,
    SR_DEV_ERR_UF_SPIN = 32,
    SR_DEV_ERR_BREAKPOINT = 64,
    SR_DEV_ERR_GRAPH = 128,
    SR_DEV_ERR_ADDRESS = 256
};

struct SrPen {
    int x, o1, e1, o2, e2;
    int two;
    int scope;
};

struct SrAlignArgs {
    const uint32_t *seqwords;
    const uint64_t *word_off_fwd;
    const uint64_t *word_off_rc;
    const uint64_t *word_off_rev;
    const uint64_t *word_off_cmp;
    int symbits;
    const uint32_t *order;
    const uint32_t *seqlen;
    uint32_t max_words;
    const uint32_t *pair_q, *pair_t;
    uint32_t npairs;
    uint32_t *queue_head;
    SrPen pen, ori;
    int mem_mode;
    int ring_scope;
    int ring_hot;
    int hist_w, hist_levels;
    int impl;
    int kdepth;
    int kdepth2;
    int kblock;
    void *bring;
    uint64_t bring_wg_stride;
    int brow;
    void *bhist;
    uint64_t bhist_wg_stride;
    uint64_t hist_cap;
    uint32_t hist_stride;
    uint32_t hist_nul_w;
    int bbase_jobs;
    int *bseg;
    uint32_t *bbt;
    uint32_t *bcl;
    uint64_t bcl_wg_stride;
    void *oring;
    uint64_t oring_wg_stride;
    int orow;
    uint32_t *oqueue;
    const uint32_t *kbits;
    int pre_oriented;
    int lazy_id;
    int profile_ticks;
    int ori_levels;
    int ring_u16;
    int *bmak;
    int test_base_levels;
    int fuse_unite;
    unsigned long long *uf_nodes;
    const uint64_t *seq_goff;
    const int32_t *max_score;
    uint64_t min_match_len;
    const uint32_t *mirror;
    uint32_t *tail_list;
    uint32_t *tail_count;
    uint32_t *tail_head;
    uint32_t *tail_deferred;
    int tail_mode;
    int *brec;
    unsigned long long *timeline;
    uint32_t *cu_arrivals;
    int prio_wg;
    int tile_prio;
    unsigned long long *prio_timeline;
    uint8_t *is_reverse;
    int32_t *score;
    int32_t *ori_fwd, *ori_rev;
    uint32_t *cigar_ops;
    const uint64_t *cigar_base;
    uint32_t *cigar_cnt;
    unsigned long long *counters;
    int *error_flag;
};
#define SR_NCOUNTERS 54
enum { SR_TAIL_MAIN = 0,
       SR_TAIL_RUN = 1,
       SR_TAIL_DEFER_ALL = 2 };

struct SrUniteArgs {
    const uint32_t *pair_q, *pair_t;
    uint32_t npairs;
    const uint32_t *seqlen;
    const uint64_t *seq_goff;
    const uint32_t *q_start, *t_start;
    const uint8_t *is_reverse;
    const int32_t *score;
    const int32_t *max_score;
    const uint32_t *cigar_ops;
    const uint64_t *cigar_base;
    const uint32_t *cigar_cnt;
    uint64_t min_match_len;
    unsigned long long *nodes;
    uint64_t uf_size;
    unsigned long long *counters;
    int *error_flag;
};

struct SrInvJob;
struct SrInvJobJ;
struct SrInvScanArgs {
    const uint32_t *cigar_ops;
    const uint64_t *cigar_base;
    const uint32_t *cigar_cnt;
    const int32_t *score;
    const int32_t *max_score;
    uint32_t npairs;
    uint32_t pair0;
    unsigned long long min_size;
    uint32_t *count;
    const uint32_t *offset;
    struct SrInvJob *jobs;
    uint64_t job_cap;
    unsigned long long *stats;
    uint32_t join_below;
    struct SrInvJobJ *jobs_j;
    int32_t pen[6];
};

#ifdef __cplusplus
extern "C" {
#endif
int srk_inv_scan(const struct SrInvScanArgs *a, int emit, void *stream);
int srk_inv_offsets(const uint32_t *count, uint32_t n, uint32_t *off, void *stream);
int srk_align(const SrAlignArgs *a, int nwg, size_t lds_bytes, int off16, int nthreads, void *stream);
int srk_unite(const SrUniteArgs *a, int nwg, void *stream);
int srk_uf_init(unsigned long long *nodes, uint64_t total_len, uint64_t uf_size, void *stream);
int srk_labels(unsigned long long *nodes, uint64_t uf_size, unsigned long long *minarr,
               unsigned long long *labels, int *error_flag, void *stream);
int srk_merge(unsigned long long *nodes, uint64_t uf_size, const unsigned long long *labels,
              uint32_t count, int *error_flag, void *stream);
int srk_align_max_lds(void);
int srk_orient(const SrAlignArgs *a, int nwg, size_t lds_bytes, int off16, void *stream);
int srk_kmer_bits(const SrAlignArgs *a, uint32_t nseq, uint32_t *kbits, void *stream);
size_t srk_order_temp_bytes(uint32_t n);
int srk_order(const SrAlignArgs *a, uint64_t *keys_in, uint64_t *keys_out, uint32_t *vals_in, void *temp, size_t temp_bytes,
              uint32_t *order_out, void *stream);
int srk_graph_induce(const unsigned long long *labels, const uint8_t *bases, const uint8_t *islast,
                     uint64_t N, uint64_t uf_size, unsigned long long *first, uint32_t *flag, uint32_t *nid,
                     uint32_t *steps, uint8_t *node_base, unsigned long long *hkeys, uint32_t *hvals,
                     uint64_t hcap, uint32_t *eslot, unsigned long long *edges, uint32_t *tile_sum,
                     uint32_t *counts, int *error_flag, void *stream);
int srk_scan_u32(const uint32_t *in, uint64_t n, uint32_t *out, uint32_t *tile_sum, uint32_t *grand, void *stream);
const char *srk_source_digest(void);
const char *srk_align_blk_build_tag(void);
int srk_align_blk_max_levels(void);
int srk_align_blk_supports(const SrPen *pen, const SrPen *ori);
int srk_labels32(unsigned long long *nodes, uint64_t uf_size, unsigned long long *minarr, uint32_t *labels, int *error_flag,
                 void *stream);
int srk_merge32(unsigned long long *nodes, uint64_t uf_size, const uint32_t *labels, uint32_t count, int *error_flag, void *stream);
int srk_sketch(const uint8_t *bases, const uint64_t *goff, const uint32_t *len, uint32_t n, int k, int s_max,
               unsigned long long *scratch, uint64_t stride, const uint32_t *npad, unsigned long long *sketch, uint32_t *sk_n,
               void *stream);
int srk_jaccard(const unsigned long long *sketch, const uint32_t *sk_n, uint32_t n, int s_max, uint32_t *shared, uint32_t *denom,
                void *stream);
int srk_knn_select(const uint32_t *shared, const uint32_t *denom, uint32_t n, int kn, int kf, uint8_t *sel, void *stream);
struct SrIterState;
int srk_iter_unite(const SrUniteArgs *a, int nwg, const struct SrIterState *st, void *stream);
int srk_count_roots(const unsigned long long *nodes, uint64_t nbases, unsigned long long *count, const struct SrIterState *st,
                    void *stream);
int srk_iter_decide(struct SrIterState *st, const unsigned long long *counts, uint32_t k, uint32_t check, void *stream);
#ifdef __cplusplus
}
#endif
```

Baseline: 107,600.

## Cache gap chain-source rows in spare LDS instead of reloading from ring

Adds an LDS chain cache: the 10-level tile stores insertion/deletion gap rows into a per-aligner LDS slice, and on the next pass reads them back from there instead of from the global ring. The cache size is taken from whatever LDS the workgroups per CU leave free, and is added to the dynamic LDS request at launch. It targets ring load traffic in the tight path. In exchange it adds extra LDS stores, index bookkeeping and shared-state resets. The larger LDS footprint could lower occupancy if the budget estimate is wrong. It only applies when the SR_LDS_CHAIN_BUILD compile flag is set.

```diff
diff --git a/__graft_entry__.py b/__graft_entry__.py
--- a/__graft_entry__.py
+++ b/__graft_entry__.py
@@ -32,7 +32,8 @@
     csrc = os.path.join(ROOT, "seqrush_amd", "csrc")
     lib = os.path.join(ROOT, "seqrush_amd", "libseqrush_amd.so")
     bounds_lib = os.path.join(ROOT, "seqrush_amd", "libseqrush_amd_bounds.so")
-    if not _lib_is_current(lib) or not os.path.exists(bounds_lib):
+    chain_lib = os.path.join(ROOT, "seqrush_amd", "libseqrush_amd_chain.so")
+    if not _lib_is_current(lib) or not os.path.exists(bounds_lib) or not os.path.exists(chain_lib):
         subprocess.check_call(["make", "-C", csrc, "-s", "-j8"], stdout=subprocess.DEVNULL)
     odir = os.path.join(ROOT, "oracle")
     olib = os.path.join(odir, "liboracle.so")
diff --git a/include/seqrush_amd.h b/include/seqrush_amd.h
--- a/include/seqrush_amd.h
+++ b/include/seqrush_amd.h
@@ -136,6 +136,14 @@
 int sr_tile_prio_epoch_shift(void);
 int sr_tail_shape(int impl, int block_levels, int wave_build, int off16, int ring_u16, int symbol_bits, int two_piece,
                   int main_threads, uint32_t max_words, int forced);
+unsigned sr_chain_cache_bytes(int impl, int block_levels, int wave_build, int ring_cell_bytes, int threads, int workgroups_per_cu,
+                              uint64_t seq_lds_bytes, int e1, int e2, int two_piece, long long cap);
+int sr_chain_slice(uint32_t cap, int naligners, int words, int idx, int shift, int32_t *out);
+int sr_chain_served_host(int first, int n, int g);
+uint32_t sr_chain_word_off_host(uint32_t slice_off, int first, int n, int g, int row);
+uint32_t sr_chain_min_bytes_host(int words);
+int sr_chain_words_host(int n1, int n2, int two_piece);
+int sr_chain_tile_own(void);
 
 typedef struct {
     uint64_t tree_entries;
diff --git a/seqrush_amd/_lib.py b/seqrush_amd/_lib.py
--- a/seqrush_amd/_lib.py
+++ b/seqrush_amd/_lib.py
@@ -40,6 +40,8 @@
     "sr_ctx_tail_deferred", "sr_ctx_tail_timeline", "sr_tail_shape",
     "sr_replay_record_ints", "sr_replay_transpose_host", "sr_replay_match_host",
     "sr_ctx_prio_timeline", "sr_tile_prio_role_host", "sr_tile_prio_epoch_shift",
+    "sr_chain_cache_bytes", "sr_chain_slice", "sr_chain_served_host", "sr_chain_word_off_host", "sr_chain_min_bytes_host",
+    "sr_chain_words_host", "sr_chain_tile_own",
 ]
 
 
diff --git a/seqrush_amd/csrc/sr_align_blk.hip b/seqrush_amd/csrc/sr_align_blk.hip
--- a/seqrush_amd/csrc/sr_align_blk.hip
+++ b/seqrush_amd/csrc/sr_align_blk.hip
@@ -45,6 +45,7 @@
 #define SR_BUILD_TAG "default"
 #endif
 extern "C" const char *srk_align_blk_build_tag(void) { return SR_BUILD_TAG; }
+extern "C" int srk_align_blk_chain_build(void) { return SR_LDS_CHAIN_BUILD; }
 extern "C" int srk_align_blk_supports(const SrPen *pen, const SrPen *ori) {
     if (ori->two || ori->e1 != 1 || ori->scope + 2 > BFS_MAK_SLOTS) return 0;
     if (pen->e1 != 2 || (pen->two && pen->e2 != 1)) return 0;
diff --git a/seqrush_amd/csrc/sr_align_blk.inc b/seqrush_amd/csrc/sr_align_blk.inc
--- a/seqrush_amd/csrc/sr_align_blk.inc
+++ b/seqrush_amd/csrc/sr_align_blk.inc
@@ -14,6 +14,9 @@
     b.shift = (pe - pb) + K_SHIFT0;
     b.pad0 = rev ? q.toff_r : q.toff_f;
     b.pad2 = 1;
+#if SR_LDS_CHAIN_BUILD
+    k_sh.jchain[jid] = SR_CHAIN_NONE;
+#endif
     if (rev) { b.p0 = q.plen_all - pe; b.t0 = q.tlen_all - te; }
 }
 __device__ __forceinline__ int kjob_width(int plen, int tlen) { return (plen + tlen + K_WIDTH0) & ~3; }
@@ -59,6 +62,10 @@
 #endif
             k_sh.dg_steps = k_sh.dg_nbase = k_sh.dg_nbp = k_sh.dg_npass = 0; k_sh.base_tiles = k_sh.base_cells = 0;
             k_sh.mir_next = -1; k_sh.mir_pairs = k_sh.mir_ties = 0;
+#if SR_LDS_CHAIN_BUILD
+            k_sh.chain_n = 0; k_sh.chain_lanes = 0ull;
+            k_sh.chain_base = (unsigned)(uintptr_t)lds_seq + 16u * a.max_words + 16u;
+#endif
             k_sh.rp_record = k_sh.rp_on = k_sh.rp_ready = 0; k_sh.rp_nrec = 0;
             k_sh.rp_replays = k_sh.rp_cached = k_sh.rp_tie_top = k_sh.rp_tie_base = 0;
             b_sh.geom.brow = a.brow; b_sh.geom.ring_scope = a.ring_scope; b_sh.geom.ring_hot = a.ring_hot;
@@ -277,6 +284,13 @@
                         na++;
                     }
                     b_sh.nact = na; b_sh.next_pos = p; b_sh.njobs = 2 * na; b_sh.nrunning = na;
+#if SR_LDS_CHAIN_BUILD
+                    {
+                        const int cn = KTIGHT ? sr_chain_slice_groups(a.lds_chain_bytes, 2 * na, sr_chain_words(E1 < B ? E1 : B, E2 < B ? E2 : B, TWO)) : 0;
+                        k_sh.chain_n = cn;
+                        for (int j = 0; j < 2 * na && cn > 0; j++) k_sh.jclo[j] = sr_chain_slice_first(cn, b_sh.job[j].shift);
+                    }
+#endif
                     k_sh.rp_ntot = ntot; k_sh.rp_maxp = maxp; k_sh.rp_npass0 = k_sh.dg_npass;
                 }
                 __syncthreads();
@@ -308,6 +322,9 @@
                         if (tid < njobs) {
 #pragma unroll
                             for (int j = 0; j < B; j++) gmak[tid * BFS_MAK_SLOTS + (s0 + j) % depth] = k_sh.jak[j][tid];
+#if SR_LDS_CHAIN_BUILD
+                            k_sh.jchain[tid] = s0;
+#endif
                         }
                         const unsigned long long qc1 = KTICK();
                         int ph = 0, ph0 = 0;
@@ -702,6 +719,9 @@
         atomicAdd(&a.counters[9], k_sh.dg_npass);
         atomicAdd(&a.counters[19], k_sh.dg_f); atomicAdd(&a.counters[20], k_sh.dg_c);
         atomicAdd(&a.counters[21], k_sh.dg_e); atomicAdd(&a.counters[22], k_sh.dg_r);
+#if SR_LDS_CHAIN_BUILD
+        if (k_sh.chain_lanes) atomicAdd(&a.counters[36], k_sh.chain_lanes * 8ull);
+#endif
         if (k_sh.dg_redo) atomicAdd(&a.counters[37], k_sh.dg_redo);
         if (k_sh.mir_pairs) atomicAdd(&a.counters[38], k_sh.mir_pairs);
         if (k_sh.mir_ties) atomicAdd(&a.counters[39], k_sh.mir_ties);
diff --git a/seqrush_amd/csrc/sr_blk_pass.inc b/seqrush_amd/csrc/sr_blk_pass.inc
--- a/seqrush_amd/csrc/sr_blk_pass.inc
+++ b/seqrush_amd/csrc/sr_blk_pass.inc
@@ -85,7 +85,9 @@
         k_sh.jglo[tid] = glo; k_sh.jghi[tid] = ghi;
         k_sh.jgplo[tid] = pglo; k_sh.jgphi[tid] = pghi;
         k_sh.jtstart[tid + 1] = incl;
+#if !SR_LDS_CHAIN_BUILD
         k_sh.jmerge[tid] = 0;
+#endif
         k_sh.jband[tid] = INT_MAX / 2;
 #pragma unroll
         for (int j = 0; j < B; j++) { k_sh.jak[j][tid] = 0; k_sh.jreach[j][tid] = 0; }
@@ -162,7 +164,12 @@
         }
     }
     __syncthreads();
-    if (tid < 2) b_sh.job[2 * sa + tid].pad2 = 1;
+    if (tid < 2) {
+        b_sh.job[2 * sa + tid].pad2 = 1;
+#if SR_LDS_CHAIN_BUILD
+        k_sh.jchain[2 * sa + tid] = SR_CHAIN_NONE;
+#endif
+    }
 }
 
 __device__ __forceinline__ long long blk_surplus(const SrPen &pen, int jid, int l0, int l1) {
diff --git a/seqrush_amd/csrc/sr_blk_rows.inc b/seqrush_amd/csrc/sr_blk_rows.inc
--- a/seqrush_amd/csrc/sr_blk_rows.inc
+++ b/seqrush_amd/csrc/sr_blk_rows.inc
@@ -1,3 +1,7 @@
+#include "sr_chain_rule.h"
+#ifndef SR_LDS_CHAIN_BUILD
+#define SR_LDS_CHAIN_BUILD 0
+#endif
 #define SR_ORI_B 16
 #define SR_KB_MAX 10
 #define KB_LV (SR_ORI_B > SR_KB_MAX ? SR_ORI_B : SR_KB_MAX)
@@ -9,7 +13,13 @@
     int jklo[KB_LV][BJ_MAX + 2], jkhi[KB_LV][BJ_MAX + 2];
     int jak[KB_MAX][BJ_MAX], jreach[KB_LV][BJ_MAX];
     int jtstart[BJ_MAX + 1], jglo[BJ_MAX + 2], jghi[BJ_MAX + 2];
+#if SR_LDS_CHAIN_BUILD
+    int jchain[BJ_MAX], jclo[BJ_MAX], chain_n;
+    unsigned chain_base;
+    unsigned long long chain_lanes;
+#else
     int jmerge[BJ_MAX];
+#endif
     int jband[BJ_MAX], jbandown[BJ_MAX], nband;
     unsigned newmask;
     int rt_n0, rt_total;
diff --git a/seqrush_amd/csrc/sr_blk_tile.inc b/seqrush_amd/csrc/sr_blk_tile.inc
--- a/seqrush_amd/csrc/sr_blk_tile.inc
+++ b/seqrush_amd/csrc/sr_blk_tile.inc
@@ -378,6 +378,21 @@
         in10 = g >= lo10 && g <= hi10; in2a = g >= lo2a && g <= hi2a; in2b = g >= lo2b && g <= hi2b;
         msk = __builtin_amdgcn_ballot_w64(!(in10 && in2a && in2b)) != 0ull;
     }
+    constexpr bool CHAIN = SR_LDS_CHAIN_BUILD && IMMR && !IDONLY;
+    constexpr int CHW = 2 * N1 + (TWO ? 2 * N2 : 0);
+    static_assert(!CHAIN || KGeo<B>::OWN == SR_CHAIN_TILE_OWN, "sr_chain_rule.h: owned groups of the 10-level tile");
+    unsigned chw = ~0u, chrs = 0u;
+    bool cuse = false;
+#if SR_LDS_CHAIN_BUILD
+    if constexpr (CHAIN) {
+        const int cn = RFL(k_sh.chain_n), clo = RFL(k_sh.jclo[jid]);
+        chrs = (unsigned)cn * SR_CHAIN_WORD_BYTES;
+        if (owned && sr_chain_served(clo, cn, g)) chw = RFL(k_sh.chain_base) + sr_chain_word_off(sr_chain_slice_off(cn, jid, CHW), clo, cn, g, 0);
+        cuse = chw != ~0u && in10 && RFL(k_sh.jchain[jid]) == s0 - B;
+    }
+#endif
+#define CH_LD(ROW) q4_from(*(const V4<short> __attribute__((address_space(3))) *)(uintptr_t)(chw + (unsigned)(ROW) * chrs))
+#define CH_ST(ROW, V) (*(V4<short> __attribute__((address_space(3))) *)(uintptr_t)(chw + (unsigned)(ROW) * chrs) = q4_vec(V))
     Q4 Lmx[XK ? 1 : B], Lmo1[B], Lmo2[B], Li1[N1], Ld1[N1], Li2[N2], Ld2[N2];
     unsigned ld_lanes10 = 64u, ld_lanes2 = 64u;
     if (TIGHT && msk) {
@@ -391,6 +406,8 @@
             if (in10) {
 #pragma unroll
                 for (int j = 0; j < B; j++) Lmo1[j] = q4_from(ild<OT, ST>(R, bM1, lane_b, j - KBLK_C));
+            }
+            if (in10 && !cuse) {
 #pragma unroll
                 for (int j = 0; j < N1; j++) { Li1[j] = q4_from(ild_nt<OT, ST>(R, bI1, lane_b, j)); Ld1[j] = q4_from(ild_nt<OT, ST>(R, bD1, lane_b, j)); }
                 if (TWO) {
@@ -416,6 +433,7 @@
             if (TWO && j < PF) Lmo2[j] = LDQ_NT(s0 + j - pen.o2 - E2, SR_C_M);
         }
     }
+    if (!cuse) {
 #pragma unroll
     for (int j = 0; j < N1; j++) {
         if constexpr (IMMR) {
@@ -437,6 +455,22 @@
         }
     }
     }
+    }
+    unsigned ch_lanes = 0u;
+    if constexpr (CHAIN) {
+        if (cuse) {
+#pragma unroll
+            for (int j = 0; j < N1; j++) { Li1[j] = CH_LD(j); Ld1[j] = CH_LD(N1 + j); }
+            if (TWO) {
+#pragma unroll
+                for (int j = 0; j < N2; j++) { Li2[j] = CH_LD(2 * N1 + j); Ld2[j] = CH_LD(2 * N1 + N2 + j); }
+            }
+        }
+        ch_lanes = (unsigned)__popcll(__builtin_amdgcn_ballot_w64(cuse));
+#if SR_LDS_CHAIN_BUILD
+        if (lane == 0 && ch_lanes) atomicAdd(&k_sh.chain_lanes, (unsigned long long)(ch_lanes * (unsigned)CHW));
+#endif
+    }
     const bool with_u = (chk < 0) && (R.urow != 0u) && rec;
     {
         const int nown = min(OWN, max(0, ghi - (glo + ti * OWN) + 1));
@@ -448,7 +482,7 @@
             nst += (j + E1 >= B || rec) ? 2 : 0;
             if (TWO) nst += (j + E2 >= B || rec) ? 2 : 0;
         }
-        row_ld += ld_lanes10 * (unsigned)n10 + ld_lanes2 * (unsigned)n2f + 64u * (unsigned)(n2p + (IDONLY ? B : 0) + ((with_u && s0 > 0) ? 1 : 0));
+        row_ld += ld_lanes10 * (unsigned)n10 - ch_lanes * (unsigned)CHW + ld_lanes2 * (unsigned)n2f + 64u * (unsigned)(n2p + (IDONLY ? B : 0) + ((with_u && s0 > 0) ? 1 : 0));
         row_st += (unsigned)nown * (unsigned)nst;
     }
     Q4 uacc = nulq;
@@ -643,6 +677,12 @@
                 if (!IDONLY) ist<OT, ST>(R, sM, lane_j, im, q4_vec(m));
                 if (l1) { ist<OT, ST>(R, sI1, lane_j, im, q4_vec(i1)); ist<OT, ST>(R, sD1, lane_j, im, q4_vec(d1)); }
                 if (TWO && l2) { ist<OT, ST>(R, sI2, lane_j, im, q4_vec(i2)); ist<OT, ST>(R, sD2, lane_j, im, q4_vec(d2)); }
+                if constexpr (CHAIN) {
+                    if ((l1 || (TWO && l2)) && chw != ~0u) {
+                        if (l1) { CH_ST(j - (B - N1), i1); CH_ST(N1 + j - (B - N1), d1); }
+                        if (TWO && l2) { CH_ST(2 * N1 + j - (B - N2), i2); CH_ST(2 * N1 + N2 + j - (B - N2), d2); }
+                    }
+                }
                 if (rec && (!l1 || (TWO && !l2))) {
                     const unsigned lane_r = kopaque_v(lane_b);
                     if (!l1) { ist_nt<OT, ST>(R, sI1, lane_r, im, q4_vec(i1)); ist_nt<OT, ST>(R, sD1, lane_r, im, q4_vec(d1)); }
@@ -663,6 +703,8 @@
 #undef KROW
 #undef LDQ
 #undef LDQ_NT
+#undef CH_LD
+#undef CH_ST
 }
 
 template <typename OT, bool TWO, int B, int E1, int E2, bool IDONLY, int X, int OE1, typename ST = OT, bool RING = false>
diff --git a/seqrush_amd/csrc/sr_chain_rule.h b/seqrush_amd/csrc/sr_chain_rule.h
--- /dev/null
+++ b/seqrush_amd/csrc/sr_chain_rule.h
@@ -0,0 +1,25 @@
+#pragma once
+
+#if defined(__HIPCC__) || defined(__CUDACC__)
+#define SR_CHAIN_HD __host__ __device__
+#else
+#define SR_CHAIN_HD
+#endif
+
+#define SR_CHAIN_TILE_OWN 58
+#define SR_CHAIN_WORD_BYTES 8
+#define SR_CHAIN_MAX_BYTES 65536
+#define SR_CHAIN_NONE (-1)
+
+SR_CHAIN_HD inline int sr_chain_words(int n1, int n2, int two) { return 2 * n1 + (two ? 2 * n2 : 0); }
+SR_CHAIN_HD inline unsigned sr_chain_min_bytes(int words) { return (unsigned)SR_CHAIN_TILE_OWN * (unsigned)words * SR_CHAIN_WORD_BYTES; }
+SR_CHAIN_HD inline int sr_chain_slice_groups(unsigned cap, int naligners, int words) {
+    if (naligners <= 0 || words <= 0 || cap < sr_chain_min_bytes(words)) return 0;
+    return (int)(cap / ((unsigned)naligners * (unsigned)words * SR_CHAIN_WORD_BYTES));
+}
+SR_CHAIN_HD inline int sr_chain_slice_first(int n, int shift) { return (shift >> 2) - (n >> 1); }
+SR_CHAIN_HD inline unsigned sr_chain_slice_off(int n, int idx, int words) { return (unsigned)idx * (unsigned)n * (unsigned)words * SR_CHAIN_WORD_BYTES; }
+SR_CHAIN_HD inline bool sr_chain_served(int first, int n, int g) { return (unsigned)(g - first) < (unsigned)n; }
+SR_CHAIN_HD inline unsigned sr_chain_word_off(unsigned slice_off, int first, int n, int g, int row) {
+    return slice_off + ((unsigned)row * (unsigned)n + (unsigned)(g - first)) * SR_CHAIN_WORD_BYTES;
+}
diff --git a/seqrush_amd/csrc/sr_host.cpp b/seqrush_amd/csrc/sr_host.cpp
--- a/seqrush_amd/csrc/sr_host.cpp
+++ b/seqrush_amd/csrc/sr_host.cpp
@@ -22,6 +22,7 @@
 #include "sr_base_cone.h"
 #include "sr_mirror_rule.h"
 #include "sr_prio_rule.h"
+#include "sr_chain_rule.h"
 
 static thread_local std::string g_err;
 static int fail(int code, const std::string &msg) { g_err = msg; return code; }
@@ -52,6 +53,8 @@
     {"SR_TAIL", "on", "0 = no tail launch: a tied secondary is always aligned by its primary's workgroup (A/B runs); all = every such secondary is deferred to the tail launch (tests)"},
     {"SR_TAIL_THREADS", "widest instance wider than the main launch", "threads per workgroup of the tail launch among the existing instances: 256 | 512 | 1024 (tests)"},
     {"SR_TILE_PRIO", "1", "0 = no rotating tile priority among the workgroups of a CU: all tile code at priority 0, no clock read (A/B runs, tests)"},
+    {"SR_LDS_CHAIN", "1", "0 = no chain cache: every gap chain-source row of a ring search is loaded from the ring (A/B runs, tests)"},
+    {"SR_LDS_CHAIN_BYTES", "what the workgroups per CU leave of the LDS", "cap on the chain cache's bytes per workgroup (A/B runs, tests)"},
     {"SR_TAIL_ROUNDS", "8", "a batch defers only when its alignments are at most this many times the launch's workgroups"},
     {"SR_FORCE_INT32", "off", "tests: 32-bit offsets (and the 16-bit ring of 32-bit searches) whatever the sequence length"},
     {"SR_TEST_BASE_LEVELS", "off", "tests: cap on the levels a base case is given at first (forces the re-queue path)"},
@@ -247,6 +250,7 @@
     uint64_t dp_cells = 0;
     int off16 = 1, nwg = 0, nthreads = 256, symbits = 2;
     size_t lds_bytes = 0;
+    unsigned lds_chain_bytes = 0, tail_lds_chain_bytes = 0;
     SrAlignArgs aa{};
     SrUniteArgs ua{};
     std::vector<void *> dev_allocs;
@@ -869,6 +873,35 @@
     return tail_shape(impl, kblock, wave_wg, off16, ring_u16, symbits, two, main_threads, max_words, forced);
 }
 
+#define SR_LDS_GRANULE 1280
+static unsigned chain_cache_bytes(int impl, int kblock, int wave_wg, int ring_cell_bytes, int nthreads, int wg_per_cu, size_t seq_lds_bytes,
+                                  int e1, int e2, int two, long long cap) {
+    if (impl != 2 || kblock != 10 || ring_cell_bytes != 2) return 0;
+    const int resident = std::max(1, wave_wg ? wg_per_cu : std::min(wg_per_cu, std::max(1, 1024 / std::max(64, nthreads))));
+    const long long budget = (long long)((160 * 1024 / resident) / SR_LDS_GRANULE) * SR_LDS_GRANULE;
+    long long left = budget - (long long)align_static_lds(wave_wg != 0, impl, nthreads) - (long long)seq_lds_bytes;
+    left = std::min<long long>(left, SR_CHAIN_MAX_BYTES);
+    left = left > 0 ? (left / SR_LDS_GRANULE) * SR_LDS_GRANULE : 0;
+    if (cap >= 0) left = std::min(left, cap & ~7LL);
+    const int words = sr_chain_words(std::min(e1, kblock), std::min(e2, kblock), two);
+    return left >= (long long)sr_chain_min_bytes(words) ? (unsigned)left : 0u;
+}
+static long long chain_cap_knob() { const char *e = knob("SR_LDS_CHAIN_BYTES"); return e ? std::max(0LL, atoll(e)) : -1LL; }
+extern "C" unsigned sr_chain_cache_bytes(int impl, int kblock, int wave_wg, int ring_cell_bytes, int nthreads, int wg_per_cu, uint64_t seq_lds_bytes,
+                                         int e1, int e2, int two, long long cap) {
+    return chain_cache_bytes(impl, kblock, wave_wg, ring_cell_bytes, nthreads, wg_per_cu, (size_t)seq_lds_bytes, e1, e2, two, cap);
+}
+extern "C" int sr_chain_slice(uint32_t cap, int naligners, int words, int idx, int shift, int32_t *out) {
+    const int n = sr_chain_slice_groups(cap, naligners, words);
+    out[0] = n; out[1] = sr_chain_slice_first(n, shift); out[2] = (int32_t)sr_chain_slice_off(n, idx, words);
+    return n;
+}
+extern "C" int sr_chain_served_host(int first, int n, int g) { return sr_chain_served(first, n, g) ? 1 : 0; }
+extern "C" uint32_t sr_chain_word_off_host(uint32_t slice_off, int first, int n, int g, int row) { return sr_chain_word_off(slice_off, first, n, g, row); }
+extern "C" uint32_t sr_chain_min_bytes_host(int words) { return sr_chain_min_bytes(words); }
+extern "C" int sr_chain_words_host(int n1, int n2, int two) { return sr_chain_words(n1, n2, two); }
+extern "C" int sr_chain_tile_own(void) { return SR_CHAIN_TILE_OWN; }
+
 static int plan_kernel(sr_ctx *c, const PackedSeqs &pk, const SrPen &pen, const SrPen &ori, uint64_t maxlen, uint32_t np, Plan &pl) {
     hipDeviceProp_t prop;
     HIPCHK(hipGetDeviceProperties(&prop, c->device));
@@ -916,6 +949,10 @@
     const char *tl = knob("SR_TAIL"), *tt = knob("SR_TAIL_THREADS");
     pl.tail_threads = (tl && !strcmp(tl, "0")) ? 0
                       : tail_shape(impl, kblock, pl.wave_wg, c->off16, pl.ring_u16, bits, pen.two, c->nthreads, pl.max_words, tt ? std::max(1, atoi(tt)) : 0);
+    const char *lc = knob("SR_LDS_CHAIN");
+    c->lds_chain_bytes = ((lc && atoi(lc) == 0) || !srk_align_blk_chain_build() || bits != 2 || pl.wave_wg) ? 0u
+                         : chain_cache_bytes(impl, kblock, pl.wave_wg, (int)pl.rsz, c->nthreads, pl.wg_per_cu, c->lds_bytes, pen.e1, pen.e2, pen.two, chain_cap_knob());
+    c->tail_lds_chain_bytes = 0;
     return SR_OK;
 }
 
@@ -1073,6 +1110,9 @@
     if (c->tail_threads) {
         c->tail_wg_per_cu = (int)std::max<size_t>(1, std::min<size_t>((size_t)1024 / c->tail_threads,
                                                                       (160 * 1024) / (c->lds_bytes + align_static_lds(false, 2, c->tail_threads))));
+        const char *lc = knob("SR_LDS_CHAIN");
+        c->tail_lds_chain_bytes = ((lc && atoi(lc) == 0) || !srk_align_blk_chain_build() || pk.sm.bits != 2) ? 0u
+                                  : chain_cache_bytes(impl, pl.kblock, 0, (int)rsz, c->tail_threads, c->tail_wg_per_cu, c->lds_bytes, pen.e1, pen.e2, pen.two, chain_cap_knob());
         const char *tl = knob("SR_TAIL"), *tr = knob("SR_TAIL_ROUNDS");
         c->tail_all = tl && !strcmp(tl, "all");
         c->tail_rounds = tr ? std::max(0, atoi(tr)) : SR_TAIL_ROUNDS_DEFAULT;
@@ -1093,6 +1133,7 @@
         const char *tp = knob("SR_TILE_PRIO");
         a.prio_wg = std::max(1, std::min(pl.wg_per_cu, 1024 / std::max(64, c->nthreads)));
         a.tile_prio = (a.prio_wg > 1 && !(tp && atoi(tp) == 0)) ? 1 : 0;
+        a.lds_chain_bytes = c->lds_chain_bytes;
         const char *trk = knob("SR_TAIL_ROUNDS");
         c->prio_rounds = trk ? std::max(0, atoi(trk)) : SR_TAIL_ROUNDS_DEFAULT;
     }
@@ -1209,7 +1250,7 @@
              "\"base_history_bytes_per_workgroup\": %llu, \"workspace_bytes\": %llu, \"cigar_arena_bytes\": %llu, "
              "\"orientation_ring_bytes\": %llu, \"union_find_bytes\": %llu, \"device_free_bytes_at_load\": %zu, \"kernel_build\": \"%s\", "
              "\"ring_depth_m\": %d, \"ring_depth_id\": %d, \"fused_unite\": %d, \"wave_build\": %d, \"level_kernel_wide\": %d, "
-             "\"profile_ticks\": %d, \"orientation_route\": \"%s\", \"source_digest\": \"%s\", \"mirror_partners\": %llu, \"tail_threads\": %d, \"mirror_replay\": %d, \"replay_record_bytes\": %llu, \"tile_prio\": %d, \"prio_epoch_shift\": %d, \"prio_workgroups_per_cu\": %d, \"knobs\": ",
+             "\"profile_ticks\": %d, \"orientation_route\": \"%s\", \"source_digest\": \"%s\", \"mirror_partners\": %llu, \"tail_threads\": %d, \"mirror_replay\": %d, \"replay_record_bytes\": %llu, \"tile_prio\": %d, \"prio_epoch_shift\": %d, \"prio_workgroups_per_cu\": %d, \"lds_chain_bytes\": %u, \"tail_lds_chain_bytes\": %u, \"knobs\": ",
              np, pl.nbatch, pk.sm.bits, pl.osz, pl.impl == 2 ? pl.rsz : pl.osz, pl.impl, pl.impl == 2 ? pl.kblock : 1, pen.two ? 1 : 0, pl.lazy_id,
              pl.nwg, c->nthreads, pl.wg_per_cu, c->lds_bytes,
              (unsigned long long)(pl.bring_wg * pl.rsz), (unsigned long long)(pl.bhist_wg * pl.osz),
@@ -1217,7 +1258,7 @@
              (unsigned long long)(3ULL * c->uf_size * 8), pl.free_b, srk_align_blk_build_tag(), pl.kdepth, pl.kdepth2, c->fuse_unite ? 1 : 0,
              pl.wave_wg ? 1 : 0, (pl.impl == 1 && pl.ring_scope + 1 > 32) ? 1 : 0, c->aa.profile_ticks, oroute, srk_source_digest(),
              (unsigned long long)c->mirror_partners, c->tail_threads, pl.brec_bytes ? 1 : 0, (unsigned long long)pl.brec_bytes,
-             c->aa.tile_prio, SR_PRIO_EPOCH_SHIFT, c->aa.prio_wg);
+             c->aa.tile_prio, SR_PRIO_EPOCH_SHIFT, c->aa.prio_wg, c->lds_chain_bytes, c->tail_lds_chain_bytes);
     c->workspace_report = std::string(buf) + knobs_json() + "}";
 }
 
@@ -1341,13 +1382,14 @@
     HIPCHK(hipEventRecord(*e0, c->stream));
     if (a.npairs > 0) {
         if (a.cu_arrivals) HIPCHK(hipMemsetAsync(a.cu_arrivals, 0, SR_PRIO_TABLE * sizeof(uint32_t), c->stream));
-        r = srk_align(&a, main_wg, c->lds_bytes, c->off16, c->nthreads, c->stream);
+        r = srk_align(&a, main_wg, c->lds_bytes + a.lds_chain_bytes, c->off16, c->nthreads, c->stream);
         if (r) return fail(SR_ERR_HIP, std::string("align kernel launch failed: ") + hipGetErrorString((hipError_t)r));
         if (defer) {
             const int grid = (int)std::min<uint64_t>({(uint64_t)c->tail_cus * (uint64_t)c->tail_wg_per_cu, (uint64_t)c->nwg, (uint64_t)partners});
             a.tail_mode = SR_TAIL_RUN; a.timeline = nullptr;
             a.cu_arrivals = nullptr; a.prio_timeline = nullptr; a.tile_prio = 0;
-            r = srk_align(&a, grid, c->lds_bytes, c->off16, c->tail_threads, c->stream);
+            a.lds_chain_bytes = c->tail_lds_chain_bytes;
+            r = srk_align(&a, grid, c->lds_bytes + a.lds_chain_bytes, c->off16, c->tail_threads, c->stream);
             if (r) return fail(SR_ERR_HIP, std::string("align kernel tail launch failed: ") + hipGetErrorString((hipError_t)r));
         }
     }
diff --git a/seqrush_amd/csrc/sr_internal.h b/seqrush_amd/csrc/sr_internal.h
--- a/seqrush_amd/csrc/sr_internal.h
+++ b/seqrush_amd/csrc/sr_internal.h
@@ -98,6 +98,7 @@
     int prio_wg;
     int tile_prio;
     unsigned long long *prio_timeline;
+    unsigned lds_chain_bytes;
     uint8_t *is_reverse;
     int32_t *score;
     int32_t *ori_fwd, *ori_rev;
@@ -177,6 +178,7 @@
                      uint32_t *counts, int *error_flag, void *stream);
 int srk_scan_u32(const uint32_t *in, uint64_t n, uint32_t *out, uint32_t *tile_sum, uint32_t *grand, void *stream);
 const char *srk_source_digest(void);
+int srk_align_blk_chain_build(void);
 const char *srk_align_blk_build_tag(void);
 int srk_align_blk_max_levels(void);
 int srk_align_blk_supports(const SrPen *pen, const SrPen *ori);
```

Result: slower. 103,000 (-4.3%).
